# RabbitBio/RabbitKSSD

Measured on AMD Instinct MI355X. Metric: genome-pairs/sec alldist (10k bacteria, L3K10), higher is better.
Workload: dtype bit-sliced counters of 32 x 32 tiles in registers, 16 planes (exact), u32 counts after extraction / f64 jaccard + distance; 1 GPU; alldist over 10000 synthetic bacterial sketches (sketch-level clade generator, seed 20261003, L3K10: 28-bit hashes, ~1220 per genome, clades of 10), -D 0.05, distance kernel only from an HBM-resident index (BASELINE configs[2]: precomputed .sketch/.dict); genomes=10000, pairs=49995000, hits=45000, kernel=rk_tile_kernel<512u, true>

## Files before the change

rabbitkssd_amd/csrc/rk_core.hip:

```cpp
#include <algorithm>
#include <cstdlib>
#include <cstring>

#include "rk_internal.h"

int rk_fail(rk_ctx *ctx, int code, const char *fmt, ...)
{
    char buf[512];
    va_list ap;
    va_start(ap, fmt);
    vsnprintf(buf, sizeof(buf), fmt, ap);
    va_end(ap);
    if (ctx) ctx->err = buf;
    return code;
}

static size_t pool_round(size_t bytes)
{
    if (bytes <= (1u << 16)) return (bytes + 511) & ~(size_t)511;
    if (bytes <= (1u << 24)) return (bytes + 65535) & ~(size_t)65535;
    return (bytes + ((1u << 21) - 1)) & ~(size_t)((1u << 21) - 1);
}

static void pool_put_locked(rk_ctx *ctx, void *p)
// ... 113 lines not shown
    } else {
        RK_HIP(ctx, hipMemcpyAsync(dst, src_dev, bytes, hipMemcpyDeviceToHost, stream));
        RK_HIP(ctx, hipStreamSynchronize(stream));
    }
    return RK_OK;
}

int rk_occupancy(rk_ctx *ctx, const void *kernel, int threads, size_t lds_bytes)
{
    const auto key = std::make_tuple(kernel, threads, lds_bytes);
    {
        std::lock_guard<std::mutex> lk(ctx->mu);
        auto it = ctx->occupancy.find(key);
        if (it != ctx->occupancy.end()) return it->second;
    }
    int per_cu = 0;
    if (hipOccupancyMaxActiveBlocksPerMultiprocessor(&per_cu, kernel, threads, lds_bytes) != hipSuccess) {
        (void)hipGetLastError();
        per_cu = 1;
    }
    std::lock_guard<std::mutex> lk(ctx->mu);
    ctx->occupancy[key] = per_cu;
    return per_cu;
}

template <class V> __global__ void k_calib_read(const V *p, size_t n, unsigned long long *sink)
{
    unsigned long long acc = 0;
    for (size_t i = (size_t)blockIdx.x * blockDim.x + threadIdx.x; i < n; i += (size_t)gridDim.x * blockDim.x) {
        const V v = p[i];
        const unsigned char *b = reinterpret_cast<const unsigned char *>(&v);
        acc += b[0] + b[sizeof(V) - 1];
    }
    if (acc == 0x1234567ULL) *sink = acc;
}
extern "C" int rk_debug_calib_read(rk_ctx *ctx, uint64_t bytes, int width)
{
    if (!ctx || (width != 4 && width != 8 && width != 16)) return RK_ERR_ARG;
    RK_HIP(ctx, hipSetDevice(ctx->device));
    DevBuf<char> buf(ctx);
    DevBuf<unsigned long long> sink(ctx);
    RK_HIP(ctx, buf.alloc(bytes));
    RK_HIP(ctx, sink.alloc(1));
    RK_HIP(ctx, hipMemsetAsync(buf.p, 1, bytes, ctx->stream));
    const unsigned grid = (unsigned)ctx->num_cu * 8;
    if (width == 4) hipLaunchKernelGGL(k_calib_read<uint32_t>, dim3(grid), dim3(256), 0, ctx->stream, (const uint32_t *)buf.p, bytes / 4, sink.p);
    else if (width == 8) hipLaunchKernelGGL(k_calib_read<uint2>, dim3(grid), dim3(256), 0, ctx->stream, (const uint2 *)buf.p, bytes / 8, sink.p);
    else hipLaunchKernelGGL(k_calib_read<uint4>, dim3(grid), dim3(256), 0, ctx->stream, (const uint4 *)buf.p, bytes / 16, sink.p);
    RK_HIP(ctx, hipGetLastError());
    RK_HIP(ctx, hipStreamSynchronize(ctx->stream));
    return RK_OK;
}

extern "C" int rk_debug_stream_read_gbs(rk_ctx *ctx, uint64_t bytes, int reps, double *gbs)
{
    if (!ctx || !gbs || reps < 1 || bytes < (1u << 20)) return RK_ERR_ARG;
    *gbs = 0.0;
    RK_HIP(ctx, hipSetDevice(ctx->device));
    DevBuf<char> buf(ctx);
    DevBuf<unsigned long long> sink(ctx);
    RK_HIP(ctx, buf.alloc(bytes));
    RK_HIP(ctx, sink.alloc(1));
    RK_HIP(ctx, hipMemsetAsync(buf.p, 1, bytes, ctx->stream));
    const unsigned grid = (unsigned)ctx->num_cu * 8;
    hipEvent_t e0, e1;
    RK_HIP(ctx, hipEventCreate(&e0));
    RK_HIP(ctx, hipEventCreate(&e1));
    hipLaunchKernelGGL(k_calib_read<uint4>, dim3(grid), dim3(256), 0, ctx->stream, (const uint4 *)buf.p, bytes / 16, sink.p);
    (void)hipEventRecord(e0, ctx->stream);
    for (int r = 0; r < reps; r++)
        hipLaunchKernelGGL(k_calib_read<uint4>, dim3(grid), dim3(256), 0, ctx->stream, (const uint4 *)buf.p, bytes / 16, sink.p);
    (void)hipEventRecord(e1, ctx->stream);
    hipError_t e = hipStreamSynchronize(ctx->stream);
    float ms = 0.f;
    if (e == hipSuccess) e = hipEventElapsedTime(&ms, e0, e1);
    (void)hipEventDestroy(e0);
    (void)hipEventDestroy(e1);
    RK_HIP(ctx, e);
    if (ms > 0.f) *gbs = (double)bytes * reps / (ms * 1e-3) / 1e9;
    return RK_OK;
}

extern "C" {

const char *rk_version(void) { return "rabbitkssd-amd 0.1.0 (gfx950)"; }

int rk_device_count(void)
{
    int n = 0;
    if (hipGetDeviceCount(&n) != hipSuccess) return 0;
    return n;
}

static uint32_t env_u32(const char *name, uint32_t dflt)
{
    const char *v = getenv(name);
    return v && atoi(v) > 0 ? (uint32_t)atoi(v) : dflt;
}

int rk_ctx_create(int device, rk_ctx **out)
{
    if (!out) return RK_ERR_ARG;
    *out = nullptr;
    int n = 0;
    if (hipGetDeviceCount(&n) != hipSuccess || n <= 0) return RK_ERR_NO_DEVICE;
    if (device < 0 || device >= n) return RK_ERR_NO_DEVICE;
    if (hipSetDevice(device) != hipSuccess) return RK_ERR_HIP;
    rk_ctx *ctx = new (std::nothrow) rk_ctx;
    if (!ctx) return RK_ERR_NOMEM;
    ctx->device = device;
    int v = 0;
    if (hipDeviceGetAttribute(&v, hipDeviceAttributeMultiprocessorCount, device) != hipSuccess || v <= 0) {
        delete ctx;
        return RK_ERR_HIP;
    }
    ctx->num_cu = v;
    ctx->max_lds = 64 * 1024;
    if (hipDeviceGetAttribute(&v, hipDeviceAttributeMaxSharedMemoryPerBlock, device) == hipSuccess && v > 0)
        ctx->max_lds = (size_t)v;
    if (hipDeviceGetAttribute(&v, hipDeviceAttributeSharedMemPerBlockOptin, device) == hipSuccess &&
        (size_t)v > ctx->max_lds)
        ctx->max_lds = (size_t)v;
    if (hipStreamCreateWithFlags(&ctx->stream, hipStreamNonBlocking) != hipSuccess || !rk_pinned_scratch(ctx, kPinnedBytes)) {
        rk_ctx_destroy(ctx);
        return RK_ERR_HIP;
    }
    ctx->cache_limit = (size_t)env_u32("RK_POOL_LIMIT_MB", 32768) << 20;
    ctx->sw_dist_threads = env_u32("RK_DIST_THREADS", 0);
    ctx->sw_dist_rows = env_u32("RK_DIST_ROWS", 0);
    ctx->sw_dist_pair = env_u32("RK_DIST_PAIR", 1);
    ctx->sw_dist_pair_minwg = env_u32("RK_DIST_PAIR_MINWG", 3);
    ctx->sw_dist_persist = env_u32("RK_DIST_PERSIST", 1);
    ctx->sw_dist_cand_cap = env_u32("RK_DIST_CAND_CAP", 0);
    ctx->sw_dist_stage_hits = env_u32("RK_DIST_STAGE_HITS", 0);
    ctx->sw_dist_xcd_rows = env_u32("RK_DIST_XCD_ROWS", 0);
    ctx->sw_dist_bands = getenv("RK_DIST_BANDS") ? atoi(getenv("RK_DIST_BANDS")) != 0 : 1;
    if (getenv("RK_DIST_BAND_MIN_ROWS")) ctx->sw_dist_band_min_rows = std::max(1, atoi(getenv("RK_DIST_BAND_MIN_ROWS")));
    ctx->sw_dist_near = getenv("RK_DIST_NEAR") ? atoi(getenv("RK_DIST_NEAR")) != 0 : 1;
    if (getenv("RK_DIST_TILES")) ctx->sw_dist_tiles = atoi(getenv("RK_DIST_TILES"));
    if (getenv("RK_DIST_TILES_MIN_GENOMES")) ctx->sw_dist_tiles_min_genomes = atoi(getenv("RK_DIST_TILES_MIN_GENOMES"));
    if (getenv("RK_DIST_TILES_MIN_SHARD_ROWS")) ctx->sw_dist_tiles_min_shard_rows = atoi(getenv("RK_DIST_TILES_MIN_SHARD_ROWS"));
    if (getenv("RK_DIST_NEAR_UW")) ctx->sw_dist_near_uw = atoi(getenv("RK_DIST_NEAR_UW"));
    if (getenv("RK_DIST_NEAR_MIN")) ctx->sw_dist_near_min = std::max(1, atoi(getenv("RK_DIST_NEAR_MIN")));
    if (getenv("RK_DIST_FB_SKIP")) ctx->sw_dist_fb_skip = atoi(getenv("RK_DIST_FB_SKIP")) != 0;
    ctx->sw_dist_debug = getenv("RK_DIST_DEBUG") ? atoi(getenv("RK_DIST_DEBUG")) : 0;
    if (getenv("RK_DIST_LDS_KB")) ctx->sw_dist_lds_kb = std::max(0, atoi(getenv("RK_DIST_LDS_KB")));
    ctx->sw_sketch_img = getenv("RK_SKETCH_IMG") ? std::min(2, std::max(0, atoi(getenv("RK_SKETCH_IMG")))) : 2;
    ctx->sw_index_fast = getenv("RK_INDEX_FAST") ? atoi(getenv("RK_INDEX_FAST")) != 0 : 1;
    ctx->sw_index_relabel = getenv("RK_INDEX_RELABEL") ? atoi(getenv("RK_INDEX_RELABEL")) != 0 : 1;
    ctx->sw_index_no_self = getenv("RK_INDEX_NO_SELF") ? atoi(getenv("RK_INDEX_NO_SELF")) != 0 : 0;
    if (getenv("RK_INDEX_TILES")) ctx->sw_index_tiles = atoi(getenv("RK_INDEX_TILES"));
    if (getenv("RK_INDEX_NO_HEAVY")) ctx->sw_index_heavy = atoi(getenv("RK_INDEX_NO_HEAVY")) == 0;
    if (getenv("RK_TILE_REC_CAP")) ctx->sw_tile_rec_cap = strtoull(getenv("RK_TILE_REC_CAP"), nullptr, 10);
    ctx->sw_topn = getenv("RK_DIST_TOPN") ? atoi(getenv("RK_DIST_TOPN")) != 0 : 1;
    if (getenv("RK_TOPN_BATCH_BYTES")) ctx->sw_topn_batch_bytes = std::max(1ULL, strtoull(getenv("RK_TOPN_BATCH_BYTES"), nullptr, 10));
    if (getenv("RK_TOPN_CAND_CAP")) ctx->sw_topn_cand_cap = strtoull(getenv("RK_TOPN_CAND_CAP"), nullptr, 10);
    *out = ctx;
    return RK_OK;
}

void rk_ctx_set_single_shot(rk_ctx *ctx, int on)
{
    if (ctx) ctx->single_shot = on != 0;
}

void rk_ctx_set_timing(rk_ctx *ctx, int on)
{
    if (!ctx) return;
    (void)hipSetDevice(ctx->device);
    if (on && !ctx->ev[0] && (hipEventCreate(&ctx->ev[0]) != hipSuccess || hipEventCreate(&ctx->ev[1]) != hipSuccess)) return;
    ctx->timing = on != 0;
}

void rk_ctx_pool_stats(rk_ctx *ctx, uint64_t out[4])
{
    if (!ctx || !out) return;
    std::lock_guard<std::mutex> lk(ctx->mu);
    out[0] = ctx->pool_bytes;
    out[1] = ctx->cached_bytes;
    out[2] = ctx->driver_allocs;
    out[3] = ctx->driver_frees;
}

double rk_ctx_last_ms(const rk_ctx *ctx, int which) { return ctx && which >= 0 && which < 15 ? ctx->last_ms[which] : 0.0; }

void rk_ctx_trim(rk_ctx *ctx)
{
    if (!ctx) return;
    std::lock_guard<std::mutex> lk(ctx->mu);
    (void)hipSetDevice(ctx->device);
    if (!ctx->deferred.empty()) pool_collect_locked(ctx, true);
    for (auto &b : ctx->free_blocks) {
        ctx->live.erase(b.second);
        ctx->pool_bytes -= b.first;
        ctx->driver_frees++;
        (void)hipFree(b.second);
    }
    ctx->free_blocks.clear();
    ctx->cached_bytes = 0;
}

void rk_ctx_destroy(rk_ctx *ctx)
{
    if (!ctx) return;
    (void)hipSetDevice(ctx->device);
    if (ctx->stream) {
        (void)hipStreamSynchronize(ctx->stream);
        (void)hipStreamDestroy(ctx->stream);
        if (ctx->stream2) (void)hipStreamDestroy(ctx->stream2);
        if (ctx->ev_fork) (void)hipEventDestroy(ctx->ev_fork);
        if (ctx->ev_join) (void)hipEventDestroy(ctx->ev_join);
        if (ctx->ev_inv) (void)hipEventDestroy(ctx->ev_inv);
    }
    rk_ctx_trim(ctx);
    for (hipEvent_t e : ctx->spare_events) (void)hipEventDestroy(e);
    for (auto &b : ctx->live) (void)hipFree(b.first);
    if (ctx->pinned) (void)hipHostFree(ctx->pinned);
    for (hipEvent_t e : ctx->ev)
        if (e) (void)hipEventDestroy(e);
    delete ctx;
}

const char *rk_last_error(const rk_ctx *ctx) { return ctx ? ctx->err.c_str() : "no context"; }

void rk_free_host(void *p) { free(p); }

int rk_pinned_alloc(rk_ctx *ctx, uint64_t bytes, void **out)
{
    if (!ctx || !out) return RK_ERR_ARG;
    *out = nullptr;
    RK_HIP(ctx, hipSetDevice(ctx->device));
    if (hipHostMalloc(out, bytes ? bytes : 1, hipHostMallocDefault) != hipSuccess) {
        *out = nullptr;
        return rk_fail(ctx, RK_ERR_NOMEM, "cannot pin %llu bytes of host memory", (unsigned long long)bytes);
    }
    return RK_OK;
}
void rk_pinned_free(void *p) { if (p) (void)hipHostFree(p); }

int rk_dev_alloc(rk_ctx *ctx, uint64_t bytes, void **out)
{
    if (!ctx || !out) return RK_ERR_ARG;
    *out = nullptr;
    RK_HIP(ctx, hipSetDevice(ctx->device));
    if (hipMalloc(out, bytes ? bytes : 1) != hipSuccess) {
        *out = nullptr;
        return rk_fail(ctx, RK_ERR_NOMEM, "cannot allocate %llu bytes on the device", (unsigned long long)bytes);
    }
    return RK_OK;
}
void rk_dev_free(void *p) { if (p) (void)hipFree(p); }

int rk_stream_create(rk_ctx *ctx, void **out)
{
    if (!ctx || !out) return RK_ERR_ARG;
    *out = nullptr;
    RK_HIP(ctx, hipSetDevice(ctx->device));
    hipStream_t st = nullptr;
    RK_HIP(ctx, hipStreamCreateWithFlags(&st, hipStreamNonBlocking));
    *out = (void *)st;
    return RK_OK;
}
void rk_stream_destroy(void *stream) { if (stream) (void)hipStreamDestroy((hipStream_t)stream); }

int rk_stream_sync(rk_ctx *ctx, void *stream)
{
    if (!ctx) return RK_ERR_ARG;
    RK_HIP(ctx, hipSetDevice(ctx->device));
    RK_HIP(ctx, hipStreamSynchronize((hipStream_t)stream));
    return RK_OK;
}

int rk_upload_async(rk_ctx *ctx, void *dst_dev, const void *src_host, uint64_t bytes, void *stream)
{
    if (!ctx || (bytes && (!dst_dev || !src_host))) return RK_ERR_ARG;
    RK_HIP(ctx, hipSetDevice(ctx->device));
    if (bytes) RK_HIP(ctx, hipMemcpyAsync(dst_dev, src_host, bytes, hipMemcpyHostToDevice, (hipStream_t)stream));
    return RK_OK;
}

int rk_dev_copy_async(rk_ctx *ctx, void *dst_dev, const void *src_dev, uint64_t bytes, void *stream)
{
    if (!ctx || (bytes && (!dst_dev || !src_dev))) return RK_ERR_ARG;
    RK_HIP(ctx, hipSetDevice(ctx->device));
    if (bytes) RK_HIP(ctx, hipMemcpyAsync(dst_dev, src_dev, bytes, hipMemcpyDeviceToDevice, (hipStream_t)stream));
    return RK_OK;
}

int rk_params_init(int half_k, int half_subk, int drlevel, rk_params *p)
{
    if (!p) return RK_ERR_ARG;
    if (half_subk - drlevel < 3) return RK_ERR_ARG;
    if (half_k < half_subk || half_subk >= 8 || half_subk < 1) return RK_ERR_ARG;
    if (half_k > 16 || drlevel < 0) return RK_ERR_ARG;
    memset(p, 0, sizeof(*p));
    const int out = half_k - half_subk;
    p->half_k = half_k;
    p->half_subk = half_subk;
    p->drlevel = drlevel;
    p->half_outctx_len = out;
    p->rev_add_move = 4 * half_k - 2;
    p->kmer_size = 2u * (uint32_t)half_k;
    p->dim_start = 0;
    p->dim_end = 1 << (4 * (half_subk - drlevel));
    const uint64_t tupmask = ~0ULL >> (64 - 4 * half_k);
    const uint64_t domask = (tupmask >> (4 * out)) << (2 * out);
// ... 95 lines not shown
```

rabbitkssd_amd/csrc/rk_dist.hip:

```cpp
#include <algorithm>
#include <chrono>
#include <cmath>
#include <cstdio>
#include <cstdlib>
#include <cstring>
#include <thread>
#include <tuple>
#include <vector>


#include "rk_internal.h"
#include "rk_dist_common.h"
#include "rk_dist_plan.h"

namespace {

__global__ void k_hit_keys(const rk_hit *hits, unsigned long long n, unsigned long long *keys)
{
    const unsigned long long i = (unsigned long long)blockIdx.x * blockDim.x + threadIdx.x;
    if (i < n) keys[i] = ((unsigned long long)hits[i].row << 32) | hits[i].col;
}

constexpr int kGroup = 8;
constexpr uint32_t kRowsPerXcdChunk = 16;
// ... 928 lines not shown
    else if (idx->tiles_ready) {
        const uint32_t step = o->row_step > 1 ? o->row_step : 1;
        const bool small_shard = step > 2 && idx->n_ref / step < (uint32_t)ctx->sw_dist_tiles_min_shard_rows;
        tiles = !(small_shard && idx->d_selfrange);
    } else if (floor(sp->min_jorc * (double)idx->min_ref_size) < (double)ctx->sw_dist_near_min) {
        tiles = true;
    } else {
        int rc = near_window_too_narrow(ctx, idx, stream, &tiles);
        if (rc) return rc;
    }
    if (tiles) {
        sp->kind = SelfPlan::kTiles;
        sp->need_tiles = !idx->tiles_ready;
        if (!sp->need_tiles) sp->tile = tile_launch_shape(idx, o, sp->min_jorc);
        return RK_OK;
    }
    if (!idx->d_selfrange) {
        if (!can_rows)
            return rk_fail(ctx, RK_ERR_UNSUPPORTED, "this index has no slice records (2^31 postings or more): only sparse self joins (a threshold "
                                                    "below distance 1.0) over set sketches run on it%s", idx->tiles_unusable ? ", and its tile records "
                                                    "exceed the memory budget (lists scattered over thousands of genomes)" : "");
        sp->need_slices = true;
    }
    const bool slices_coming = sp->need_slices && idx->d_src_off && idx->wide == (idx->d_uhash64 != nullptr);
    sp->near = slices_coming || idx->d_self_split ? plan_near(ctx, idx, o, dense_mode, sp->min_jorc) : NearPlan();
    sp->kind = sp->near.use ? SelfPlan::kNear : SelfPlan::kBands;
    return sp->near.use ? RK_OK : plan_bands(ctx, idx, o, dense_mode, &sp->bands);
}

int ensure_fallback(rk_ctx *ctx, rk_index *idx, hipStream_t stream)
{
    std::lock_guard<std::mutex> lk(idx->lazy_mu);
    if (idx->d_fb) return RK_OK;
    DevBuf<uint32_t> fb(ctx);
    if (fb.alloc((size_t)idx->n_ref + 8) != hipSuccess) return rk_fail(ctx, RK_ERR_NOMEM, "cannot allocate the fallback list");
    RK_HIP(ctx, hipMemsetAsync(fb.p, 0, 16, stream));
    RK_HIP(ctx, hipStreamSynchronize(stream));
    if (hipHostMalloc((void **)&idx->h_fb_seen, 64, hipHostMallocCoherent) == hipSuccess) *idx->h_fb_seen = 0xFFFFFFFFu;
    else { (void)hipGetLastError(); idx->h_fb_seen = nullptr; }
    idx->d_fb = fb.release();
    return RK_OK;
}

int launch_near(rk_ctx *ctx, const rk_index *idx, const rk_dist_opts *o, const NearPlan &np, rk_hit *hits_dev, uint64_t cap,
                unsigned long long *n_hits_dev, hipStream_t stream)
{
    NearArgs a;
    a.ranges = idx->d_selfrange;
    a.range_off = idx->d_self_off;
    a.range_split = idx->d_self_split;
    a.size_off = idx->d_src_off;
    a.postings = idx->d_postings;
    a.ref_sizes = idx->d_sizes;
    a.orig = idx->relabeled ? idx->d_orig : nullptr;
    a.n_ref = idx->n_ref;
    a.row_first = np.rows.row_first;
    a.row_step = np.rows.row_step;
    a.row_block = np.rows.row_block;
    a.units_per_block = np.units_per_block;
    a.n_units = np.n_units;
    a.metric = o->metric != 0;
    a.kmer_size = o->kmer_size;
    a.max_dist = o->max_dist;
    a.min_jorc = np.min_jorc;
    a.min_ref_size = (uint32_t)std::min<uint64_t>(idx->min_ref_size, 0xFFFFFFFFu);
    a.hits = hits_dev;
    a.cap = cap;
    a.n_hits = n_hits_dev;
    a.fb_count = idx->d_fb;
    a.fb_rows = idx->d_fb + 4;
    a.stage_hits = kNearStage;
    a.debug = getenv("RK_NEAR_DEBUG") ? atoi(getenv("RK_NEAR_DEBUG")) : 0;
#define RK_NEAR(P, U) hipLaunchKernelGGL((rk_near_kernel<P, U>), dim3(np.grid), dim3(kNearThreads), 0, stream, a)
    if (np.pair) { if (np.uw == 1) RK_NEAR(true, 1); else if (np.uw == 2) RK_NEAR(true, 2); else RK_NEAR(true, 4); }
    else { if (np.uw == 1) RK_NEAR(false, 1); else if (np.uw == 2) RK_NEAR(false, 2); else RK_NEAR(false, 4); }
#undef RK_NEAR
    RK_HIP(ctx, hipGetLastError());
    return RK_OK;
}

struct FbGate { unsigned char key[sizeof(rk_index::fb_key)] = {0}; bool skip = false, arm = false; };
FbGate fb_gate_begin(rk_ctx *ctx, rk_index *mut, const rk_dist_opts *o, bool dense_mode)
{
    FbGate g;
    static_assert(sizeof(rk_dist_opts) + 1 <= sizeof g.key, "key holds the options and the report mode");
    memcpy(g.key, o, sizeof(rk_dist_opts));
    g.key[sizeof(rk_dist_opts)] = dense_mode ? 1 : 0;
    if (ctx->sw_dist_fb_skip && mut->h_fb_seen) {
        std::lock_guard<std::mutex> lk(mut->lazy_mu);
        if (memcmp(g.key, mut->fb_key, sizeof g.key) != 0) {
            memcpy(mut->fb_key, g.key, sizeof g.key);
            mut->fb_state = 0;
        }
        if (mut->fb_state == 1) {
            const hipError_t qe = hipEventQuery((hipEvent_t)mut->fb_event);
            if (qe == hipSuccess) mut->fb_state = *(volatile uint32_t *)mut->h_fb_seen == 0 ? 2 : 3;
            else (void)hipGetLastError();
        }
        g.skip = mut->fb_state == 2;
        if (mut->fb_state == 0) {
            if (!mut->fb_event) {
                hipEvent_t ev;
                if (hipEventCreateWithFlags(&ev, hipEventDisableTiming | hipEventReleaseToSystem) == hipSuccess) mut->fb_event = ev;
                else (void)hipGetLastError();
            }
            g.arm = mut->fb_event != nullptr;
        }
    }
    return g;
}
void fb_gate_armed(rk_index *mut, const FbGate &g, hipStream_t stream)
{
    std::lock_guard<std::mutex> lk(mut->lazy_mu);
    if (mut->fb_state == 0 && memcmp(g.key, mut->fb_key, sizeof g.key) == 0 &&
        hipEventRecord((hipEvent_t)mut->fb_event, stream) == hipSuccess) mut->fb_state = 1;
}

int launch_near_and_fallback(rk_ctx *ctx, rk_index *mut, const rk_dist_opts *o, bool dense_mode, const NearPlan &np, rk_hit *hits_dev,
                             uint64_t cap, unsigned long long *n_hits_dev, hipStream_t stream)
{
    int rc = ensure_fallback(ctx, mut, stream);
    if (!rc && np.n_units) rc = launch_near(ctx, mut, o, np, hits_dev, cap, n_hits_dev, stream);
    if (rc) return rc;
    const FbGate gate = fb_gate_begin(ctx, mut, o, dense_mode);
    if (gate.skip) return RK_OK;
    Plan fp;
    rk_dist_opts all = *o;
    all.row_first = 0;
    all.row_step = 1;
    rc = make_plan(ctx, mut, mut->n_ref, mut->max_src_size, &all, false, true, mut->n_ref, &fp, false);
    if (rc) return rc;
    rc = launch_dist(ctx, mut, mut->d_selfrange, mut->d_self_off, mut->d_src_off, mut->n_ref, o, fp, hits_dev, cap, n_hits_dev,
                     nullptr, stream, mut->d_fb);
    if (!rc && gate.arm) fb_gate_armed(mut, gate, stream);
    return rc;
}

int launch_self(rk_ctx *ctx, const rk_index *idx, const rk_dist_opts *o, bool dense_mode, rk_hit *hits_dev, uint64_t cap,
                unsigned long long *n_hits_dev, hipStream_t stream)
{
    rk_index *mut = const_cast<rk_index *>(idx);
    SelfPlan sp;
    int rc = plan_self(ctx, idx, o, dense_mode, stream, &sp);
    if (!rc && sp.need_tiles) {
        rc = rk_tiles_build(ctx, mut, stream);
        if (!rc && !idx->tiles_unusable) sp.tile = tile_launch_shape(idx, o, sp.min_jorc);
        else if (!rc) rc = plan_self(ctx, idx, o, dense_mode, stream, &sp);
    }
    if (!rc && sp.need_slices) {
        rc = rk_index_ensure_slices(ctx, mut, stream);
        if (!rc) rc = plan_self(ctx, idx, o, dense_mode, stream, &sp);
    }
    if (rc) return rc;
    if (sp.kind == SelfPlan::kTiles) return launch_tiles(ctx, idx, o, sp.min_jorc, sp.tile, hits_dev, cap, n_hits_dev, stream);
    if (sp.kind == SelfPlan::kNear) return launch_near_and_fallback(ctx, mut, o, dense_mode, sp.near, hits_dev, cap, n_hits_dev, stream);
    if (ctx->sw_dist_debug) print_bands(sp.bands);
    for (size_t b = 0; !rc && b < sp.bands.size(); b++)
        rc = launch_dist(ctx, idx, idx->d_selfrange, idx->d_self_off, idx->d_src_off, idx->n_ref, o, sp.bands[b], hits_dev, cap,
                         n_hits_dev, nullptr, stream);
    return rc;
}

uint64_t host_exact_distances(rk_hit *h, uint64_t n, const rk_dist_opts *o)
{
    const int metric = o->metric != 0;
    auto fix = [&](uint64_t lo, uint64_t hi) {
        for (uint64_t i = lo; i < hi; i++) {
            const JorcDist jd = rk_distance(h[i].common, h[i].size0, h[i].size1, metric, o->kmer_size);
            h[i].jorc = jd.jorc;
            h[i].dist = jd.dist;
        }
    };
    const uint64_t kChunk = 8192;
    if (n < 2 * kChunk) fix(0, n);
    else {
        const unsigned nt = (unsigned)std::min<uint64_t>(std::max(1u, std::thread::hardware_concurrency()), std::min<uint64_t>(16, n / kChunk));
        std::vector<std::thread> pool;
        for (unsigned t = 0; t < nt; t++) pool.emplace_back(fix, n * t / nt, n * (t + 1) / nt);
        for (auto &th : pool) th.join();
    }
    uint64_t w = 0;
    for (uint64_t i = 0; i < n; i++) {
        const bool keep = o->triangle ? (h[i].dist < o->max_dist) : (h[i].dist <= o->max_dist);
        if (keep) {
            if (w != i) h[w] = h[i];
            w++;
        }
    }
    return w;
}

int download_hits_in_order(rk_ctx *ctx, const rk_hit *hits_dev, unsigned long long n, uint32_t n_query, hipStream_t stream, rk_hit **out_p)
{
    rk_hit *out = (rk_hit *)malloc((n ? n : 1) * sizeof(rk_hit));
    if (!out) return rk_fail(ctx, RK_ERR_NOMEM, "host allocation of %llu hits failed", n);
    const rk_hit *src = hits_dev;
    DevBuf<rk_hit> ordered(ctx);
    bool on_device = false;
    if (n > (ctx->single_shot ? (1ULL << 18) : 2048ULL)) {
        DevBuf<unsigned long long> keys(ctx), keys_out(ctx);
        int bits = 33;
        while (bits < 64 && (1ULL << (bits - 32)) < n_query) bits++;
        if (keys.alloc(n) == hipSuccess && keys_out.alloc(n) == hipSuccess && ordered.alloc(n) == hipSuccess) {
            hipLaunchKernelGGL(k_hit_keys, dim3((unsigned)((n + 255) / 256)), dim3(256), 0, stream, hits_dev, n, keys.p);
            on_device = rk_prim_sort_hits(ctx, keys.p, keys_out.p, hits_dev, ordered.p, n, (unsigned)bits, stream) == RK_OK;
        }
        if (on_device) src = ordered.p;
        else (void)hipGetLastError();
    }
    if (n) {
        hipError_t e = hipMemcpyAsync(out, src, n * sizeof(rk_hit), hipMemcpyDeviceToHost, stream);
        if (e == hipSuccess) e = hipStreamSynchronize(stream);
        if (e != hipSuccess) {
            free(out);
            return rk_fail(ctx, RK_ERR_HIP, "hit download failed: %s", hipGetErrorString(e));
        }
    }
    if (!on_device)
        std::sort(out, out + n, [](const rk_hit &x, const rk_hit &y) {
            return x.row != y.row ? x.row < y.row : x.col < y.col;
        });
    *out_p = out;
    return RK_OK;
}

}

uint64_t rk_host_exact_distances(rk_hit *h, uint64_t n, const rk_dist_opts *o) { return host_exact_distances(h, n, o); }

#ifdef RK_DIST_PROFILE
extern "C" int rk_debug_dist_prof_raw(unsigned long long *out, unsigned long long n_waves)
{
    if (n_waves > (unsigned long long)kProfWaves) return -1;
    return hipMemcpyFromSymbol(out, HIP_SYMBOL(g_prof), n_waves * 16 * 8) == hipSuccess ? 0 : -1;
}
extern "C" int rk_debug_dist_prof(unsigned long long *out16, int reset)
{
    std::vector<unsigned long long> all((size_t)kProfWaves * 16);
    if (hipMemcpyFromSymbol(all.data(), HIP_SYMBOL(g_prof), sizeof(g_prof)) != hipSuccess) return -1;
    for (int i = 0; i < 16; i++) out16[i] = 0;
    for (size_t w = 0; w < (size_t)kProfWaves; w++)
        for (int i = 0; i < 16; i++) out16[i] += all[w * 16 + i];
    if (reset) {
        std::fill(all.begin(), all.end(), 0ULL);
        if (hipMemcpyToSymbol(HIP_SYMBOL(g_prof), all.data(), sizeof(g_prof)) != hipSuccess) return -1;
    }
    return 0;
}
#endif

extern "C" {

int rk_dist_kernel_name(rk_ctx *ctx, const rk_index *idx, const rk_sketches *queries, const rk_dist_opts *opts, char *buf,
                        size_t cap)
{
    if (!ctx || !idx || !opts || !buf || !cap) return RK_ERR_ARG;
    if (queries) return rk_distq_kernel_name(ctx, idx, queries, buf, cap);
    SelfPlan sp;
    int rc = plan_self(ctx, idx, opts, rk_dense_mode(opts), ctx->stream, &sp);
    if (rc) return rc;
    if (sp.kind == SelfPlan::kTiles && sp.need_tiles)
        snprintf(buf, cap, "rk_tile_kernel");
    else if (sp.kind == SelfPlan::kTiles)
        snprintf(buf, cap, "rk_tile_kernel<%du, %s>", sp.tile.threads, sp.tile.srow ? "true" : "false");
    else if (sp.kind == SelfPlan::kNear)
        snprintf(buf, cap, "rk_near_kernel<%s, %d>", sp.near.pair ? "true" : "false", sp.near.uw);
    else {
        if (ctx->sw_dist_debug) print_bands(sp.bands);
        const Plan &p = sp.bands[0];
        if (sp.bands.size() > 1)
            snprintf(buf, cap, "rk_dist_kernel<%s, %d, %u> [%u bands]", p.u16 ? "true" : "false", p.mode, p.threads, (unsigned)sp.bands.size());
        else
            snprintf(buf, cap, "rk_dist_kernel<%s, %d, %u>", p.u16 ? "true" : "false", p.mode, p.threads);
    }
    return RK_OK;
}

int rk_index_tile_stats(const rk_index *idx, const rk_dist_opts *opts, uint64_t out[4])
{
    if (!idx || !out) return RK_ERR_ARG;
    out[0] = out[1] = out[2] = out[3] = 0;
    if (!idx->tiles_ready) return RK_OK;
    out[0] = idx->n_tiles;
    out[2] = idx->n_tile_records;
    out[3] = idx->n_tile_slots;
    if (opts && opts->kmer_size > 0 && opts->max_dist > 0.0) out[1] = tile_launch_shape(idx, opts, rk_min_jorc(opts)).grid;
    return RK_OK;
}

int rk_dist_rows_dev(rk_ctx *ctx, const rk_index *idx, const rk_sketches *queries,
                     const rk_dist_opts *opts, rk_hit *hits_dev, uint64_t hits_cap,
                     uint64_t *n_hits_dev, void *stream)
{
    if (!ctx || !idx || !opts || !n_hits_dev || (!hits_dev && hits_cap)) return RK_ERR_ARG;
    RK_HIP(ctx, hipSetDevice(ctx->device));
    if (queries) {
        if (opts->triangle && queries->n != idx->n_ref)
            return rk_fail(ctx, RK_ERR_ARG, "triangle mode needs the indexed sketches as queries (%u vs %u)",
                           queries->n, idx->n_ref);
        return rk_distq_launch(ctx, idx, queries, opts, rk_dense_mode(opts), hits_dev, hits_cap, (unsigned long long *)n_hits_dev,
                               nullptr, (hipStream_t)stream);
    }
    if (int rc = rk_self_join_args(ctx, idx, opts)) return rc;
    return launch_self(ctx, idx, opts, rk_dense_mode(opts), hits_dev, hits_cap, (unsigned long long *)n_hits_dev, (hipStream_t)stream);
}

int rk_dist_rows(rk_ctx *ctx, const rk_index *idx, const rk_sketches *queries,
// ... 70 lines not shown
```

rabbitkssd_amd/csrc/rk_dist_tile.inc:

```

struct TileArgs {
    const unsigned long long *tile_key;
    const unsigned long long *tile_start;
    const uint32_t *blk_min;
    const uint64_t *size_off;
    const uint32_t *orig;
    const uint32_t *order;
    const uint4 *dir;
    unsigned long long n_tiles;
    uint32_t n_ref;
    uint32_t row_first, row_step, row_block;
    int metric, kmer_size;
    double max_dist, min_jorc;
    rk_hit *hits;
    unsigned long long cap;
    unsigned long long *n_hits;
    int debug;
};

constexpr unsigned long long kTileSrowPerTile = 2000ULL;
constexpr int kTilePlanes = 11;

__device__ inline uint32_t csa(uint32_t &a, uint32_t b, uint32_t c)
{
    const uint32_t carry = __builtin_amdgcn_bitop3_b32(a, b, c, 0xE8);
    a = __builtin_amdgcn_bitop3_b32(a, b, c, 0x96);
    return carry;
}
__device__ inline uint32_t ripple(uint32_t &p, uint32_t carry)
{
    const uint32_t c2 = p & carry;
    p ^= carry;
    return c2;
}

template <uint32_t kTileThreads, bool SROW>
__global__ __launch_bounds__(kTileThreads, kTileThreads == 256 ? 6 : 4) void rk_tile_kernel(TileArgs a, const uint2 *__restrict__ contrib, const uint32_t *__restrict__ rows, const uint32_t *__restrict__ cols)
{
    constexpr uint32_t kTileWaves = kTileThreads / 64;
    constexpr uint32_t kTileStage = (uint32_t)(8 * kTileThreads * sizeof(uint2) / sizeof(rk_hit));
    static_assert(kTileStage >= kTileThreads + 64, "a round of cells fits the stage");
    __shared__ uint32_t cnt[32 * 32];
    __shared__ __attribute__((aligned(16))) uint2 recs[8 * kTileThreads];
    rk_hit *stage = reinterpret_cast<rk_hit *>(recs);
    __shared__ uint32_t s_cursor;
    __shared__ unsigned long long s_base;
    __shared__ uint32_t rsize[32], csize[32];
    const uint32_t tid = threadIdx.x, lane = tid & 63, wave = tid >> 6;
    const uint32_t half = lane >> 5, row = lane & 31;

    const uint4 d0 = a.dir[2 * (size_t)blockIdx.x], d1 = a.dir[2 * (size_t)blockIdx.x + 1];
    const uint32_t b = d0.x, w = d0.y;
    const unsigned long long s0 = (unsigned long long)d0.z | ((unsigned long long)d0.w << 32), s1 = s0 + d1.x;
    {
        const uint32_t lb = d1.y;
        bool take = (double)(s1 - s0) >= a.min_jorc * (double)lb;
        if (take && a.row_step > 1) {
            bool mine = false;
            const uint32_t r0 = b * 32, r1 = min(a.n_ref, r0 + 32);
            for (uint32_t blk = r0 / a.row_block; blk <= (r1 - 1) / a.row_block; blk++) mine |= blk % a.row_step == a.row_first;
            take = mine;
        }
        if (!take || (a.debug & 4) || ((a.debug & 32) && blockIdx.x >= 512) || ((a.debug & 64) && blockIdx.x >= 256)) return;
    }
    for (uint32_t i = tid; i < 32 * 32; i += kTileThreads) cnt[i] = 0;
    if (tid == 0) s_cursor = 0;
    __syncthreads();

    auto flush_stage = [&]() {
        __syncthreads();
        const uint32_t n_st = min(s_cursor, kTileStage);
        if (n_st) {
            if (tid == 0) s_base = (a.debug & 4096) ? (unsigned long long)blockIdx.x * 128ULL : atomicAdd(a.n_hits, (unsigned long long)n_st);
            __syncthreads();
            const unsigned long long at0 = s_base;
            const unsigned long long *src = reinterpret_cast<const unsigned long long *>(stage);
            unsigned long long *dst = reinterpret_cast<unsigned long long *>(a.hits);
            constexpr uint32_t kW = sizeof(rk_hit) / 8;
            for (uint32_t i = tid; i < n_st * kW; i += kTileThreads)
                if (at0 + i / kW < a.cap) dst[at0 * kW + i] = src[i];
        }
        __syncthreads();
        if (tid == 0) s_cursor = 0;
        __syncthreads();
    };

    {
        if (tid < 64) {
            const uint32_t g = (tid < 32 ? b : w) * 32 + (tid & 31);
            const uint32_t sz = g < a.n_ref ? (uint32_t)(a.size_off[g + 1] - a.size_off[g]) : 0u;
            if (tid < 32) rsize[tid] = sz; else csize[tid - 32] = sz;
        }
        uint32_t p[kTilePlanes + 1];
#pragma unroll
        for (int k = 0; k <= kTilePlanes; k++) p[k] = 0;
        uint32_t steps = 0;
        auto to_lds = [&]() {
            uint32_t carry = 0;
#pragma unroll
            for (int k = 0; k < kTilePlanes; k++) {
                const uint32_t o = (uint32_t)__shfl_xor((int)p[k], 32);
                const uint32_t u = p[k] ^ o;
                const uint32_t c2 = (p[k] & o) | (u & carry);
                p[k] = u ^ carry;
                carry = c2;
            }
            p[kTilePlanes] = carry;
            uint32_t any = 0;
#pragma unroll
            for (int k = 0; k <= kTilePlanes; k++) any |= p[k];
            const uint32_t occupied = wave_or(any);
            uint32_t occ2 = (occupied | (occupied >> 16)) & 0xFFFFu;
            while (occ2) {
                const int c = __builtin_ctz(occ2) + 16 * (int)half;
                occ2 &= occ2 - 1;
                uint32_t v = 0;
#pragma unroll
                for (int k = 0; k <= kTilePlanes; k++) v |= ((p[k] >> c) & 1u) << k;
                if (v) atomicAdd(&cnt[c * 32 + row], v);
            }
#pragma unroll
            for (int k = 0; k <= kTilePlanes; k++) p[k] = 0;
            steps = 0;
        };
        auto add8 = [&](const uint32_t (&m)[8]) {
            const uint32_t t2a = csa(p[0], m[0], m[1]);
            const uint32_t t2b = csa(p[0], m[2], m[3]);
            const uint32_t t4a = csa(p[1], t2a, t2b);
            const uint32_t t2c = csa(p[0], m[4], m[5]);
            const uint32_t t2d = csa(p[0], m[6], m[7]);
            const uint32_t t4b = csa(p[1], t2c, t2d);
            uint32_t carry = csa(p[2], t4a, t4b);
#pragma unroll
            for (int k = 3; k < kTilePlanes; k++) carry = ripple(p[k], carry);
            steps += 8;
            if (steps >= 1984) to_lds();
        };
        auto carry16 = [&](const uint32_t (&ma)[8], const uint32_t (&mb)[8]) -> uint32_t {
            const uint32_t a2a = csa(p[0], ma[0], ma[1]);
            const uint32_t a2b = csa(p[0], ma[2], ma[3]);
            const uint32_t a4a = csa(p[1], a2a, a2b);
            const uint32_t a2c = csa(p[0], ma[4], ma[5]);
            const uint32_t a2d = csa(p[0], ma[6], ma[7]);
            const uint32_t a4b = csa(p[1], a2c, a2d);
            const uint32_t c8a = csa(p[2], a4a, a4b);
            const uint32_t b2a = csa(p[0], mb[0], mb[1]);
            const uint32_t b2b = csa(p[0], mb[2], mb[3]);
            const uint32_t b4a = csa(p[1], b2a, b2b);
            const uint32_t b2c = csa(p[0], mb[4], mb[5]);
            const uint32_t b2d = csa(p[0], mb[6], mb[7]);
            const uint32_t b4b = csa(p[1], b2c, b2d);
            const uint32_t c8b = csa(p[2], b4a, b4b);
            return csa(p[3], c8a, c8b);
        };
        auto add16 = [&](const uint32_t (&ma)[8], const uint32_t (&mb)[8]) {
            uint32_t carry = carry16(ma, mb);
#pragma unroll
            for (int k = 4; k < kTilePlanes; k++) carry = ripple(p[k], carry);
            steps += 16;
            if (steps >= 1984) to_lds();
        };
        if (!(a.debug & 1)) {
            if constexpr (SROW) {
                constexpr int kDepth = 3;
                const unsigned long long slot0 = (unsigned long long)d1.z | ((unsigned long long)d1.w << 32);
                const unsigned long long *__restrict__ tile_rows = reinterpret_cast<const unsigned long long *>(rows + slot0);
                const uint32_t n_rec = d1.x;
                const uint32_t wave_u = (uint32_t)__builtin_amdgcn_readfirstlane((int)wave);
                const uint32_t per = ((n_rec + kTileWaves - 1) / kTileWaves + 127u) & ~127u;
                const uint32_t w0 = min(n_rec, wave_u * per), w1 = min(n_rec, w0 + per);
                const uint32_t n_sub = (w1 - w0 + 127u) / 128u;
                const uint32_t *__restrict__ tile_cols = cols + slot0;
                uint32_t *mine = reinterpret_cast<uint32_t *>(recs + wave * 512);
                uint32_t in0[kDepth], in1[kDepth];
                auto request = [&](uint32_t sub, int slot) {
                    const uint32_t at = w0 + sub * 128u + lane;
                    in0[slot] = tile_cols[at];
                    in1[slot] = tile_cols[at + 64u];
                };
                const uint32_t put0 = (lane & 1u) * 64u + (lane >> 1), put1 = put0 + 32u;
    #pragma unroll
                for (int d = 0; d < kDepth; d++)
                    if ((uint32_t)d < n_sub) request((uint32_t)d, d);
                for (uint32_t sub0 = 0; sub0 < n_sub; sub0 += kDepth) {
    #pragma unroll
                    for (int d = 0; d < kDepth; d++) {
                        const uint32_t sub = sub0 + d;
                        if (sub >= n_sub) break;
                        const uint32_t at = w0 + sub * 128u + lane;
                        uint32_t *slot = mine + (sub & 3u) * 128;
                        slot[put0] = at < w1 ? in0[d] : 0u;
                        slot[put1] = at + 64u < w1 ? in1[d] : 0u;
                        if (sub + kDepth < n_sub) request(sub + kDepth, d);
                        __builtin_amdgcn_fence(__ATOMIC_RELEASE, "wavefront");
                        __builtin_amdgcn_wave_barrier();
                        const uint32_t n_here = min(128u, w1 - (w0 + sub * 128u));
                        const uint4 *rd = reinterpret_cast<const uint4 *>(slot + 64 * half);
                        const unsigned long long *pairs = tile_rows + ((w0 + sub * 128u) >> 1);
                        const uint32_t n_groups = min(8u, (n_here + 15) / 16);
                        auto masks_sel = [&](uint32_t g, const unsigned long long *sel, uint32_t (&m)[8]) {
                            const uint4 r0 = rd[2 * g], r1 = rd[2 * g + 1];
                            const uint32_t y[8] = {r0.x, r0.y, r0.z, r0.w, r1.x, r1.y, r1.z, r1.w};
    #pragma unroll
                            for (int j = 0; j < 8; j++)
                                asm("v_cndmask_b32_e64 %0, 0, %1, %2" : "=v"(m[j]) : "v"(y[j]), "s"(sel[j]));
                        };
                        auto masks = [&](uint32_t g, uint32_t (&m)[8]) {
                            unsigned long long sel[8];
    #pragma unroll
                            for (int j = 0; j < 8; j++) sel[j] = pairs[8 * g + j];
                            const uint4 r0 = rd[2 * g], r1 = rd[2 * g + 1];
                            const uint32_t y[8] = {r0.x, r0.y, r0.z, r0.w, r1.x, r1.y, r1.z, r1.w};
    #pragma unroll
                            for (int j = 0; j < 8; j++)
                                asm("v_cndmask_b32_e64 %0, 0, %1, %2" : "=v"(m[j]) : "v"(y[j]), "s"(sel[j]));
                        };
                        uint32_t g = 0;
                        auto carry32 = [&](uint32_t g0) -> uint32_t {
                            unsigned long long sel[32];
    #pragma unroll
                            for (int j = 0; j < 32; j++) sel[j] = pairs[8 * g0 + j];
                            uint32_t ma[8], mb[8];
                            masks_sel(g0, sel, ma);
                            masks_sel(g0 + 1, sel + 8, mb);
                            const uint32_t c16a = carry16(ma, mb);
                            masks_sel(g0 + 2, sel + 16, ma);
                            masks_sel(g0 + 3, sel + 24, mb);
                            const uint32_t c16b = carry16(ma, mb);
                            return csa(p[4], c16a, c16b);
                        };
                        if (n_groups == 8 && !(a.debug & (256 | 512 | 1024))) {
                            const uint32_t c32a = carry32(0);
                            const uint32_t c32b = carry32(4);
                            uint32_t carry = csa(p[5], c32a, c32b);
    #pragma unroll
                            for (int k = 6; k < kTilePlanes; k++) carry = ripple(p[k], carry);
                            steps += 64;
                            if (steps >= 1984) to_lds();
                            g = 8;
                        }
                        for (; g + 3 < n_groups && !(a.debug & (256 | 512)); g += 4) {
                            uint32_t carry = carry32(g);
    #pragma unroll
                            for (int k = 5; k < kTilePlanes; k++) carry = ripple(p[k], carry);
                            steps += 32;
                            if (steps >= 1984) to_lds();
                        }
                        for (; g + 1 < n_groups && !(a.debug & 256); g += 2) {
                            uint32_t ma[8], mb[8];
                            masks(g, ma);
                            masks(g + 1, mb);
                            if (a.debug & 8) { p[0] |= ma[0] | ma[1] | ma[2] | ma[3] | ma[4] | ma[5] | ma[6] | ma[7] | mb[0] | mb[7]; continue; }
                            add16(ma, mb);
                        }
                        for (; g < n_groups; g++) {
                            uint32_t m[8];
                            masks(g, m);
                            if (a.debug & 8) { p[0] |= m[0] | m[1] | m[2] | m[3] | m[4] | m[5] | m[6] | m[7]; continue; }
                            add8(m);
                        }
                        __builtin_amdgcn_wave_barrier();
                    }
                }
            } else {
                constexpr int kDepth = 3;
                const uint2 *__restrict__ tile = contrib + s0;
                const uint32_t n_rec = d1.x;
                const uint32_t per = ((n_rec + kTileWaves - 1) / kTileWaves + 127u) & ~127u;
                const uint32_t w0 = min(n_rec, wave * per), w1 = min(n_rec, w0 + per);
                const uint32_t n_sub = (w1 - w0 + 127u) / 128u;
                uint2 *mine = recs + wave * 512;
                uint2 in0[kDepth], in1[kDepth];
                auto request = [&](uint32_t sub, int slot) {
                    const uint32_t at = w0 + sub * 128u + lane;
                    in0[slot] = tile[min(at, n_rec - 1u)];
                    in1[slot] = tile[min(at + 64u, n_rec - 1u)];
                };
    #pragma unroll
                for (int d = 0; d < kDepth; d++)
                    if ((uint32_t)d < n_sub) request((uint32_t)d, d);
                for (uint32_t sub0 = 0; sub0 < n_sub; sub0 += kDepth) {
    #pragma unroll
                    for (int d = 0; d < kDepth; d++) {
                        const uint32_t sub = sub0 + d;
                        if (sub >= n_sub) break;
                        const uint32_t at = w0 + sub * 128u + lane;
                        uint2 *slot = mine + (sub & 3u) * 128;
                        slot[lane] = at < w1 ? in0[d] : make_uint2(0, 0);
                        slot[64 + lane] = at + 64u < w1 ? in1[d] : make_uint2(0, 0);
                        if (sub + kDepth < n_sub) request(sub + kDepth, d);
                        __builtin_amdgcn_fence(__ATOMIC_RELEASE, "wavefront");
                        __builtin_amdgcn_wave_barrier();
                        const uint32_t n_here = min(128u, w1 - (w0 + sub * 128u));
                        const uint4 *rd = reinterpret_cast<const uint4 *>(slot + 64 * half);
                        const uint32_t n_groups = min(8u, (n_here + 7) / 8);
                        auto masks = [&](uint32_t g, uint32_t (&m)[8]) {
    #pragma unroll
                            for (int j = 0; j < 4; j++) {
                                const uint4 r = rd[4 * g + j];
                                m[2 * j] = (uint32_t)__builtin_amdgcn_sbfe((int)r.x, row, 1) & r.y;
                                m[2 * j + 1] = (uint32_t)__builtin_amdgcn_sbfe((int)r.z, row, 1) & r.w;
                            }
                        };
                        uint32_t g = 0;
                        auto carry32 = [&](uint32_t g0) -> uint32_t {
                            uint32_t ma[8], mb[8];
                            masks(g0, ma);
                            masks(g0 + 1, mb);
                            const uint32_t c16a = carry16(ma, mb);
                            masks(g0 + 2, ma);
                            masks(g0 + 3, mb);
                            const uint32_t c16b = carry16(ma, mb);
                            return csa(p[4], c16a, c16b);
                        };
                        if (n_groups == 8 && !(a.debug & (256 | 512 | 1024))) {
                            const uint32_t c32a = carry32(0);
                            const uint32_t c32b = carry32(4);
                            uint32_t carry = csa(p[5], c32a, c32b);
    #pragma unroll
                            for (int k = 6; k < kTilePlanes; k++) carry = ripple(p[k], carry);
                            steps += 64;
                            if (steps >= 1984) to_lds();
                            g = 8;
                        }
                        for (; g + 3 < n_groups && !(a.debug & (256 | 512)); g += 4) {
                            uint32_t carry = carry32(g);
    #pragma unroll
                            for (int k = 5; k < kTilePlanes; k++) carry = ripple(p[k], carry);
                            steps += 32;
                            if (steps >= 1984) to_lds();
                        }
                        for (; g + 1 < n_groups && !(a.debug & 256); g += 2) {
                            uint32_t ma[8], mb[8];
                            masks(g, ma);
                            masks(g + 1, mb);
                            if (a.debug & 8) { p[0] |= ma[0] | ma[1] | ma[2] | ma[3] | ma[4] | ma[5] | ma[6] | ma[7] | mb[0] | mb[7]; continue; }
                            add16(ma, mb);
                        }
                        for (; g < n_groups; g++) {
                            uint32_t m[8];
                            masks(g, m);
                            if (a.debug & 8) { p[0] |= m[0] | m[1] | m[2] | m[3] | m[4] | m[5] | m[6] | m[7]; continue; }
                            add8(m);
                        }
                        __builtin_amdgcn_wave_barrier();
                    }
                }
            }
        }
        if (!(a.debug & 16)) {
            constexpr int kAll = 16;
            uint32_t q[kAll];
            {
                uint32_t carry = 0;
#pragma unroll
                for (int k = 0; k < kTilePlanes; k++) {
                    const uint32_t o = (uint32_t)__shfl_xor((int)p[k], 32);
                    const uint32_t u = p[k] ^ o;
                    q[k] = u ^ carry;
                    carry = (p[k] & o) | (u & carry);
                }
                q[kTilePlanes] = carry;
#pragma unroll
                for (int k = kTilePlanes + 1; k < kAll; k++) q[k] = 0;
            }
            uint32_t *all_planes = reinterpret_cast<uint32_t *>(recs);
            uint32_t *my_planes = all_planes + wave * 1024;
            auto publish = [&]() {
                if (lane < 32) {
#pragma unroll
                    for (int k = 0; k < kAll; k++) my_planes[k * 32 + row] = q[k];
                }
            };
            if (kTileWaves > 1) publish();
            __syncthreads();
#pragma unroll
            for (uint32_t stride = 1; stride < kTileWaves; stride <<= 1) {
                if ((wave & (2 * stride - 1)) == 0) {
                    const uint32_t *theirs = all_planes + (wave + stride) * 1024;
                    uint32_t carry = 0;
#pragma unroll
                    for (int k = 0; k < kAll; k++) {
                        const uint32_t o = theirs[k * 32 + row];
                        const uint32_t u = q[k] ^ o;
                        const uint32_t c2 = (q[k] & o) | (u & carry);
                        q[k] = u ^ carry;
                        carry = c2;
                    }
                    publish();
                }
                __syncthreads();
            }
            if (kTileWaves > 1) {
#pragma unroll
                for (int k = 0; k < kAll; k++) q[k] = all_planes[k * 32 + row];
            }
            constexpr uint32_t kColsPerHalf = 16 / kTileWaves;
#pragma unroll
            for (uint32_t i = 0; i < kColsPerHalf; i++) {
                const uint32_t c = wave * (32 / kTileWaves) + half * kColsPerHalf + i;
                uint32_t v = 0;
#pragma unroll
                for (int k = 0; k < kAll; k++) v |= ((q[k] >> c) & 1u) << k;
                if (v) cnt[c * 32 + row] += v;
            }
        }
        __syncthreads();
        for (uint32_t round = 0; round < 1024 / kTileThreads; round++) {
            if (s_cursor + kTileThreads > kTileStage) flush_stage();
            const uint32_t ci = round * kTileThreads + tid;
            const uint32_t col = ci >> 5, r = ci & 31;
            const uint32_t common = cnt[ci];
            cnt[ci] = 0;
            const uint32_t grow = b * 32 + r, gcol = w * 32 + col;
            bool ok = common != 0 && gcol > grow && gcol < a.n_ref && !(a.debug & 2);
            if (ok && a.row_step > 1) ok = (grow / a.row_block) % a.row_step == a.row_first;
            if (ok) {
                const int size0 = (int)rsize[r], size1 = (int)csize[col];
                const int denom = a.metric ? min(size0, size1) : size0 + size1 - (int)common;
                if ((double)common >= a.min_jorc * (double)denom) {
                    const JorcDist jd = rk_distance((int)common, size0, size1, a.metric, a.kmer_size);
                    if (jd.dist < a.max_dist) {
                        uint32_t out_row = grow, out_col = gcol;
                        if (a.orig) {
                            out_row = a.orig[grow];
                            out_col = a.orig[gcol];
                        }
                        const bool flip = out_row > out_col;
                        rk_hit hrec;
                        hrec.row = flip ? out_col : out_row;
                        hrec.col = flip ? out_row : out_col;
                        hrec.common = (int)common;
                        hrec.size0 = flip ? size1 : size0;
                        hrec.size1 = flip ? size0 : size1;
                        hrec.pad_ = 0;
                        hrec.jorc = jd.jorc;
                        hrec.dist = jd.dist;
                        stage[atomicAdd(&s_cursor, 1u)] = hrec;
                    }
                }
            }
            __syncthreads();
        }
        flush_stage();
    }
}

struct TileShape { unsigned long long grid = 0; int threads = 256; bool srow = false; };
TileShape tile_launch_shape(const rk_index *idx, const rk_dist_opts *o, double min_jorc)
{
    const int metric = o->metric != 0;
    unsigned long long grid = idx->n_tiles;
    if (min_jorc > 0.0) {
        const double kk = ceil(-8.0 * log2(min_jorc));
        if (kk < (double)kTileTable) grid = idx->tile_prefix[metric][kk < 0.0 ? 0 : (int)kk];
    }
    if (getenv("RK_TILE_ALL")) grid = idx->n_tiles;
    const uint32_t row_step = o->row_step ? o->row_step : 1;
    int threads = grid / row_step < 1500 ? 512 : 256;
    if (grid / row_step < 150) threads = 1024;
    if (getenv("RK_TILE_THREADS")) threads = atoi(getenv("RK_TILE_THREADS"));
    if (threads != 512 && threads != 1024) threads = 256;
    bool srow = threads >= 512 && grid && idx->n_tile_records >= kTileSrowPerTile * grid && idx->d_tile_rows;
    if (getenv("RK_TILE_SROW")) srow = atoi(getenv("RK_TILE_SROW")) != 0 && idx->d_tile_rows;
    return TileShape{grid, threads, srow};
}

int launch_tiles(rk_ctx *ctx, const rk_index *idx, const rk_dist_opts *o, double min_jorc, const TileShape &shape, rk_hit *hits_dev, uint64_t cap,
                 unsigned long long *n_hits_dev, hipStream_t stream)
{
    if (!idx->n_tiles) return RK_OK;
    TileArgs a;
    a.tile_key = idx->d_tile_key;
    a.tile_start = idx->d_tile_start;
    a.blk_min = idx->d_blk_min;
    a.size_off = idx->d_src_off;
    a.orig = idx->relabeled ? idx->d_orig : nullptr;
    a.n_tiles = idx->n_tiles;
    a.n_ref = idx->n_ref;
    a.order = idx->d_tile_order[o->metric != 0];
    a.dir = idx->d_tile_dir[o->metric != 0];
    const RowShard rows(o, idx->n_ref, 0);
    a.row_step = rows.row_step;
    a.row_first = rows.row_first;
    a.row_block = rows.row_block;
    a.metric = o->metric != 0;
    a.kmer_size = o->kmer_size;
    a.max_dist = o->max_dist;
    a.min_jorc = min_jorc;
    a.hits = hits_dev;
    a.cap = cap;
    a.n_hits = n_hits_dev;
    a.debug = getenv("RK_TILE_DEBUG") ? atoi(getenv("RK_TILE_DEBUG")) : 0;
    if (!shape.grid) return RK_OK;
    if (shape.grid > 0x7FFFFFFFULL) return rk_fail(ctx, RK_ERR_UNSUPPORTED, "too many tiles for one launch (%llu)", (unsigned long long)idx->n_tiles);
#define RK_TILE_LAUNCH(T)                                                                                                              \
    do {                                                                                                                               \
        if (shape.srow) hipLaunchKernelGGL((rk_tile_kernel<T, true>), dim3((unsigned)shape.grid), dim3(T), 0, stream, a, (const uint2 *)idx->d_tile_contrib, (const uint32_t *)idx->d_tile_rows, (const uint32_t *)idx->d_tile_cols); \
        else hipLaunchKernelGGL((rk_tile_kernel<T, false>), dim3((unsigned)shape.grid), dim3(T), 0, stream, a, (const uint2 *)idx->d_tile_contrib, (const uint32_t *)idx->d_tile_rows, (const uint32_t *)idx->d_tile_cols); \
    } while (0)
    if (shape.threads == 512)
        RK_TILE_LAUNCH(512);
    else if (shape.threads == 1024)
        RK_TILE_LAUNCH(1024);
    else
        RK_TILE_LAUNCH(256);
#undef RK_TILE_LAUNCH
    RK_HIP(ctx, hipGetLastError());
    return RK_OK;
}
```

rabbitkssd_amd/csrc/rk_index.hip:

```cpp
#include <cstring>

#include <algorithm>
#include <chrono>
#include <cstdlib>
#include <thread>

#include "rk_internal.h"

namespace {

struct BuildResult {
    unsigned long long U, n_self, dups, flags;
    unsigned long long flagged;
};

template <class Acc, class L, class W> __device__ inline Acc block_scan_sweeps(uint32_t n, L load, W store)
{
    __shared__ Acc scan_part[1024 / 64];
    constexpr uint32_t R = 16;
    const uint32_t tid = threadIdx.x, lane = tid & 63, wave = tid >> 6, nw = blockDim.x >> 6;
    const uint32_t rows = (n + 63) / 64;
    Acc carry = 0;
    for (uint32_t base = 0; base < rows; base += nw * R) {
        const uint32_t r0 = base + wave * R;
// ... 321 lines not shown
        uint32_t votes = 0;
#pragma unroll
        for (uint32_t j = 0; j < kMinK; j++) votes += r[j] == r[i];
        if (votes >= 2 && r[i] < best) best = r[i];
    }
    parent[g] = best;
}

__global__ void k_cluster_keys(const uint32_t *parent, uint32_t n_genomes, int id_bits, unsigned long long *keys)
{
    const uint32_t g = blockIdx.x * blockDim.x + threadIdx.x;
    if (g >= n_genomes) return;
    uint32_t p = parent[g];
    for (uint32_t hop = 0; hop < n_genomes; hop++) {
        const uint32_t q = parent[p];
        if (q == p) break;
        p = q;
    }
    keys[g] = ((unsigned long long)p << id_bits) | g;
}

__global__ void k_order_from_keys(const unsigned long long *keys, uint32_t n_genomes, int id_bits, const uint64_t *off,
                                  const uint32_t *sizes_in, uint32_t *orig, uint32_t *sizes)
{
    const uint32_t i = blockIdx.x * blockDim.x + threadIdx.x;
    if (i >= n_genomes) return;
    const uint32_t g = (uint32_t)(keys[i] & ((1ULL << id_bits) - 1ULL));
    orig[i] = g;
    sizes[i] = sizes_in ? sizes_in[g] : (uint32_t)(off[g + 1] - off[g]);
}

__global__ void k_offsets_scan(const uint32_t *sizes, uint32_t n_genomes, uint64_t *off_new)
{
    const unsigned long long all = block_scan_sweeps<unsigned long long>(
        n_genomes, [&](uint32_t g) { return (unsigned long long)sizes[g]; },
        [&](uint32_t g, unsigned long long before) { off_new[g] = before; });
    if (threadIdx.x == 0) off_new[n_genomes] = all;
}

constexpr uint32_t kRankThreads = 256, kRankPer = 4, kRankQ = kRankThreads * kRankPer, kRankStretch = 256, kRankMaxN = 32768;
__global__ void k_cluster_keys32(const uint32_t *parent, uint32_t n_genomes, int id_bits, uint32_t *keys, uint32_t *rank)
{
    const uint32_t g = blockIdx.x * blockDim.x + threadIdx.x;
    if (g >= n_genomes) return;
    rank[g] = 0;
    uint32_t p = parent[g];
    for (uint32_t hop = 0; hop < n_genomes; hop++) {
        const uint32_t q = parent[p];
        if (q == p) break;
        p = q;
    }
    keys[g] = (p << id_bits) | g;
}
__global__ __launch_bounds__(kRankThreads) void k_rank_keys(const uint32_t *__restrict__ keys, uint32_t n, uint32_t *rank)
{
    __shared__ __attribute__((aligned(16))) uint32_t others[kRankStretch];
    const uint32_t j0 = blockIdx.y * kRankStretch;
    for (uint32_t j = threadIdx.x; j < kRankStretch; j += kRankThreads) others[j] = j0 + j < n ? keys[j0 + j] : 0xFFFFFFFFu;
    uint32_t mine[kRankPer], below[kRankPer];
#pragma unroll
    for (uint32_t i = 0; i < kRankPer; i++) {
        const uint32_t q = blockIdx.x * kRankQ + i * kRankThreads + threadIdx.x;
        mine[i] = q < n ? keys[q] : 0u;
        below[i] = 0;
    }
    __syncthreads();
    const uint4 *o4 = reinterpret_cast<const uint4 *>(others);
#pragma unroll 4
    for (uint32_t j = 0; j < kRankStretch / 4; j++) {
        const uint4 v = o4[j];
#pragma unroll
        for (uint32_t i = 0; i < kRankPer; i++) below[i] += (v.x < mine[i]) + (v.y < mine[i]) + (v.z < mine[i]) + (v.w < mine[i]);
    }
#pragma unroll
    for (uint32_t i = 0; i < kRankPer; i++) {
        const uint32_t q = blockIdx.x * kRankQ + i * kRankThreads + threadIdx.x;
        if (q < n && below[i]) atomicAdd(&rank[q], below[i]);
    }
}
__global__ void k_order_from_rank(const uint32_t *rank, uint32_t n_genomes, const uint64_t *off, const uint32_t *sizes_in, uint32_t *orig, uint32_t *sizes)
{
    const uint32_t g = blockIdx.x * blockDim.x + threadIdx.x;
    if (g >= n_genomes) return;
    const uint32_t i = rank[g];
    orig[i] = g;
    sizes[i] = sizes_in ? sizes_in[g] : (uint32_t)(off[g + 1] - off[g]);
}

template <class K>
__global__ void k_gather_sketches(const K *hashes, const uint64_t *off, const uint32_t *orig, const uint64_t *off_new,
                                  uint32_t n_genomes, K *out)
{
    const uint32_t i = blockIdx.x * (blockDim.x >> 6) + (threadIdx.x >> 6);
    if (i >= n_genomes) return;
    const uint64_t src = off[orig[i]], dst = off_new[i], n = off_new[i + 1] - dst;
    for (uint64_t k = threadIdx.x & 63; k < n; k += 64) out[dst + k] = hashes[src + k];
}

__global__ void k_emit_table(const uint32_t *inv, const uint64_t *off_new, uint32_t n, uint2 *tab)
{
    const uint32_t g = blockIdx.x * blockDim.x + threadIdx.x;
    if (g < n) tab[g] = make_uint2(inv[g], (uint32_t)off_new[inv[g]]);
}

__global__ void k_invert_order(const uint32_t *orig, uint32_t n, uint32_t *inv)
{
    const uint32_t i = blockIdx.x * blockDim.x + threadIdx.x;
    if (i < n) inv[orig[i]] = i;
}

__global__ void k_iota(uint32_t n, uint32_t *out)
{
    const uint32_t i = blockIdx.x * blockDim.x + threadIdx.x;
    if (i < n) out[i] = i;
}

#include "rk_index_fast.inc"
#include "rk_index_tiles.inc"
#include "rk_index_keys.inc"

struct BuildSource {
    uint32_t n = 0;
    uint64_t total = 0;
    bool wide = false, is_set = false;
    uint64_t max_size = 0, min_size = 0;
    const uint64_t *d_off = nullptr;
    const uint32_t *d_sizes = nullptr;
    const uint32_t *d_sig = nullptr;
    const rk_sketches *s = nullptr;
    const unsigned long long *keys = nullptr;
    uint64_t n_keys = 0;
};
inline BuildSource source_of(const rk_sketches *s)
{
    BuildSource src;
    src.n = s->n;
    src.total = s->total;
    src.wide = s->wide;
    src.is_set = s->is_set;
    src.max_size = s->max_size;
    for (uint32_t g = 0; g < s->n; g++) {
        const uint64_t sz = s->h_off[g + 1] - s->h_off[g];
        if (sz && (!src.min_size || sz < src.min_size)) src.min_size = sz;
    }
    src.d_off = s->d_off;
    src.s = s;
    return src;
}

#include "rk_index_plan.h"

struct TileSortBufs {
    DevBuf<uint3> brec;
    DevBuf<uint32_t> tb, bins, t_rows, t_cols;
    DevBuf<uint4> proto, t_dir_j, t_dir_c;
    DevBuf<unsigned long long> level_start;
    DevBuf<uint2> t_contrib;
    explicit TileSortBufs(rk_ctx *c) : brec(c), tb(c), bins(c), t_rows(c), t_cols(c), proto(c), t_dir_j(c), t_dir_c(c), level_start(c), t_contrib(c) {}
    int alloc(rk_ctx *ctx, uint32_t n_blocks, uint64_t n_records, uint64_t tile_cap)
    {
        const uint64_t slot_cap = n_records + tile_cap;
        RK_HIP(ctx, brec.alloc(n_records));
        RK_HIP(ctx, tb.alloc(3 * (size_t)n_blocks));
        RK_HIP(ctx, bins.alloc((size_t)n_blocks + 1));
        RK_HIP(ctx, proto.alloc(2 * tile_cap));
        RK_HIP(ctx, level_start.alloc(2 * (kTileTable + 1)));
        RK_HIP(ctx, t_contrib.alloc(slot_cap + 256));
        if (rowsort_stage(n_blocks)) {
            RK_HIP(ctx, t_rows.alloc(slot_cap + 256));
            RK_HIP(ctx, t_cols.alloc(slot_cap + 256));
        }
        RK_HIP(ctx, t_dir_j.alloc(2 * tile_cap));
        RK_HIP(ctx, t_dir_c.alloc(2 * tile_cap));
        return RK_OK;
    }
    TileSortArgs args(const uint3 *rec, uint32_t region_cap, uint32_t n_blocks, const uint32_t *blk_min, const ZeroedLayout &z) const
    {
        TileSortArgs ta;
        memset(&ta, 0, sizeof ta);
        ta.rec = rec;
        ta.cur = z.tile_cursors();
        ta.region_cap = region_cap;
        ta.n_blocks = n_blocks;
        ta.bin_count = z.bin_count();
        ta.bin_cursor = z.bin_cursor();
        ta.bin_start = bins.p;
        ta.brec = brec.p;
        ta.blk_min = blk_min;
        ta.contrib = t_contrib.p;
        ta.rows = t_rows.p;
        ta.cols = t_cols.p;
        ta.tb_base = tb.p;
        ta.tb_cnt = tb.p + n_blocks;
        ta.order = tb.p + 2 * (size_t)n_blocks;
        ta.proto = proto.p;
        ta.level_start = level_start.p;
        ta.dir[0] = t_dir_j.p;
        ta.dir[1] = t_dir_c.p;
        ta.tres = z.tile_res();
        return ta;
    }
    void hand_over(rk_index *idx, const TileResult &tr)
    {
        idx->d_tile_contrib = t_contrib.release();
        idx->d_tile_rows = t_rows.release();
        idx->d_tile_cols = t_cols.release();
        idx->d_tile_dir[0] = t_dir_j.release();
        idx->d_tile_dir[1] = t_dir_c.release();
        idx->n_tile_slots = tr.n_slots;
        idx->n_tiles = tr.n_tiles;
        idx->n_tile_records = tr.n_records;
        idx->tile_max_records = tr.max_records;
        for (int m = 0; m < 2; m++)
            for (int k = 0; k < kTileTable; k++) idx->tile_prefix[m][k] = tr.level_count[m][k];
        idx->tiles_ready = true;
        idx->tiles_from_build = true;
    }
};

struct BuildCtx {
    rk_ctx *ctx;
    const BuildSource &src;
    const BuildPlan &p;
    const BuildKnobs &k;
    rk_index *idx;
    hipStream_t st;
};

int alloc_index_arrays(rk_ctx *ctx, rk_index *idx, const BuildPlan &p)
{
    RK_TRY(pool_array(ctx, &idx->d_sizes, (size_t)p.N + 1));
    RK_TRY(pool_array(ctx, &idx->d_src_off, (size_t)p.N + 1));
    RK_TRY(pool_array(ctx, &idx->d_postings, p.H_el + 8));
    if (idx->wide) RK_TRY(pool_array(ctx, &idx->d_uhash64, p.Ucap + 1));
    else RK_TRY(pool_array(ctx, &idx->d_uhash, p.Ucap + 1));
    RK_TRY(pool_array(ctx, &idx->d_upos, p.Ucap + 2));
    RK_TRY(pool_array(ctx, &idx->d_orig, (size_t)p.N + 1));
    if (p.tiles_mode) RK_TRY(pool_array(ctx, &idx->d_blk_min, (size_t)p.n_blocks));
    return RK_OK;
}
int alloc_slices(rk_ctx *ctx, rk_index *idx, const BuildPlan &p)
{
    if (p.no_self || idx->d_selfrange) return RK_OK;
    RK_TRY(pool_array(ctx, &idx->d_selfrange, p.H + 1));
    RK_TRY(pool_array(ctx, &idx->d_self_off, (size_t)p.N + 1));
    RK_TRY(pool_array(ctx, &idx->d_self_split, (size_t)p.N + 1));
    return RK_OK;
}
void drop_blk_min(rk_ctx *ctx, rk_index *idx)
{
    rk_pool_free(ctx, idx->d_blk_min);
    idx->d_blk_min = nullptr;
}

int ensure_stream2(rk_ctx *ctx, bool high_priority)
{
    if (ctx->stream2) return RK_OK;
    int prio_lo = 0, prio_hi = 0;
    if (high_priority && hipDeviceGetStreamPriorityRange(&prio_lo, &prio_hi) == hipSuccess && prio_hi != prio_lo)
        RK_HIP(ctx, hipStreamCreateWithPriority(&ctx->stream2, hipStreamNonBlocking, prio_hi));
    else
        RK_HIP(ctx, hipStreamCreateWithFlags(&ctx->stream2, hipStreamNonBlocking));
    RK_HIP(ctx, hipEventCreateWithFlags(&ctx->ev_fork, hipEventDisableTiming));
    RK_HIP(ctx, hipEventCreateWithFlags(&ctx->ev_join, hipEventDisableTiming));
    RK_HIP(ctx, hipEventCreateWithFlags(&ctx->ev_inv, hipEventDisableTiming));
    return RK_OK;
}

struct Renumbering {
    const BuildCtx &b;
    DevBuf<unsigned long long> rl_table, rl_keys, rl_keys_sorted;
    DevBuf<uint32_t> rl_parent, rl_keys32, rl_rank, rl_inv;
    DevBuf<uint2> rl_tab;
    DevBuf<char> rl_tmp;
    const uint32_t *inv = nullptr;
    bool forked = false, joined = true;
    bool inv_recorded = false;
    bool enqueued = false;
    explicit Renumbering(const BuildCtx &bc)
        : b(bc), rl_table(bc.ctx), rl_keys(bc.ctx), rl_keys_sorted(bc.ctx), rl_parent(bc.ctx), rl_keys32(bc.ctx), rl_rank(bc.ctx), rl_inv(bc.ctx),
          rl_tab(bc.ctx), rl_tmp(bc.ctx) {}

    int mark_fork()
    {
        if (!b.p.two_streams) return RK_OK;
        RK_TRY(ensure_stream2(b.ctx, b.k.stream2_high));
        RK_HIP(b.ctx, hipEventRecord(b.ctx->ev_fork, b.st));
        return RK_OK;
    }
    int join()
    {
        if (!joined) {
            RK_HIP(b.ctx, hipStreamWaitEvent(b.st, b.ctx->ev_join, 0));
            joined = true;
        }
        return RK_OK;
    }
    int wait_inv()
    {
        if (inv_recorded && !joined) RK_HIP(b.ctx, hipStreamWaitEvent(b.st, b.ctx->ev_inv, 0));
        else RK_TRY(join());
        return RK_OK;
    }
    int ensure_table()
    {
        if (!inv || rl_tab.p) return RK_OK;
        RK_HIP(b.ctx, rl_tab.alloc(b.p.N));
        hipLaunchKernelGGL(k_emit_table, dim3(blocks_for(b.p.N)), dim3(kThreads), 0, b.st, inv, b.idx->d_src_off, b.p.N, rl_tab.p);
        return RK_OK;
    }
    int branch_heads(hipStream_t *sh)
    {
        RK_HIP(b.ctx, hipEventRecord(b.ctx->ev_fork, b.st));
        RK_HIP(b.ctx, hipStreamWaitEvent(b.ctx->stream2, b.ctx->ev_fork, 0));
        *sh = b.ctx->stream2;
        return RK_OK;
    }
    int heads_branched()
    {
        RK_HIP(b.ctx, hipEventRecord(b.ctx->ev_join, b.ctx->stream2));
        joined = false;
        return RK_OK;
    }
    int enqueue(bool want_tab);
    int enqueue_identity();
};

int Renumbering::enqueue(bool want_tab)
{
    if (enqueued) return RK_OK;
    enqueued = true;
    if (!b.p.relabel) return enqueue_identity();
    rk_ctx *ctx = b.ctx;
    rk_index *idx = b.idx;
    const BuildSource &src = b.src;
    const uint32_t N = b.p.N;
    hipStream_t s2 = b.st;
    if (b.p.two_streams) {
        s2 = ctx->stream2;
        RK_HIP(ctx, hipStreamWaitEvent(s2, ctx->ev_fork, 0));
        forked = true;
    }
    const int id_bits = b.p.gb;
    uint32_t slots = 1024;
    const unsigned long long want_slots = b.k.table_x * N * kMinK;
    while (slots < want_slots && slots < (1u << 30)) slots <<= 1;
    RK_HIP(ctx, rl_table.alloc(slots));
    RK_HIP(ctx, rl_parent.alloc(N));
    RK_HIP(ctx, hipMemsetAsync(rl_table.p, 0xFF, (size_t)slots * 8, s2));
    const unsigned nb_ins = (unsigned)(((uint64_t)N * kMinK + kInsertThreads - 1) / kInsertThreads), nb_n = blocks_for(N);
    auto insert_and_vote = [&](auto rs) {
        using R = decltype(rs);
        hipLaunchKernelGGL(k_minhash_insert<R>, dim3(nb_ins), dim3(kInsertThreads), 0, s2, rs, N, rl_table.p, slots - 1);
        hipLaunchKernelGGL(k_minhash_vote<R>, dim3(nb_n), dim3(kThreads), 0, s2, rs, N, rl_table.p, slots - 1, rl_parent.p);
    };
    if (src.d_sig) insert_and_vote(SigMinK{src.d_sig});
    else if (idx->wide) insert_and_vote(CsrMinK<uint64_t>{src.s->d_hashes64, src.s->d_off});
    else insert_and_vote(CsrMinK<uint32_t>{src.s->d_hashes, src.s->d_off});
    if (N <= kRankMaxN) {
// ... 541 lines not shown
            break;
        case AttemptOutcome::FallBackToSlices:
            rs.tiles_mode = false;
            drop_blk_min(ctx, idx);
            rep[RK_REPORT_FELL_BACK] = 1;
            break;
        default: again = false;
        }
    }
    rep[RK_REPORT_FLAGS] = o.flags;
    rep[RK_REPORT_HEAVY] = o.heavy;
    rep[RK_REPORT_PASSES] = o.passes;
    const bool built = o.what == AttemptOutcome::Built;
    if (!built && p.from_keys && (o.flags & kFastBadHash))
        return rk_fail(ctx, RK_ERR_ARG, "rk_index_build_shard_keys: a key outside the wire format (hash bits beyond the shard's range, or a genome id >= %u)", p.N);
    if (!built && n_shards > 1)
        return rk_fail(ctx, RK_ERR_UNSUPPORTED, "rk_index_build_shard: the bucket sort refused this collection (flags %s: a bucket or a pass beyond its "
                                                "buffer, a hash outside the hash space, or tile records beyond their capacity)", o.tr.overflow ? "tile overflow" : "bucket / key overflow");
    if (!built) {
        if (idx->d_blk_min) drop_blk_min(ctx, idx);
        RK_TRY(alloc_slices(ctx, idx, p));
    }

    RK_TRY(rn.enqueue(false));
    RK_TRY(rn.join());
    BuildResult r = built ? o.r : BuildResult{0, 0, 0, 0, 0};
    if (!built && p.H) {
        RK_TRY(build_general(b, res.p, &r));
        rep[RK_REPORT_GENERAL] = 1;
    } else if (!p.H) RK_TRY(build_empty(b));
    idx->U = r.U;
    idx->n_self = r.n_self;
    idx->slices_refused = p.no_self;
    idx->ref_sets = src.is_set || r.dups == 0;
    idx->built_fast = built;
    if (built) {
        idx->spread = r.flagged * 8 > r.n_self;
        idx->spread_known = 1;
    }
    set_dir_shape(idx);
    guard.p = nullptr;
    *out = idx;
    return RK_OK;
}

}

__global__ void k_slices_from_lists(const uint32_t *postings, const uint32_t *upos, uint64_t U, uint2 *raw, uint32_t *pos)
{
    const uint64_t u = (uint64_t)blockIdx.x * blockDim.x + threadIdx.x;
    if (u >= U) return;
    const uint32_t s = upos[u], e = upos[u + 1];
    const uint32_t last = e > s ? postings[e - 1] : 0u;
    uint32_t prev = 0xFFFFFFFFu;
    for (uint32_t k = s; k < e; k++) {
        const uint32_t g = postings[k];
        uint2 rec = make_uint2(0, 0);
        if (k + 1 < e) {
            const uint32_t first = postings[k + 1];
            const bool covered = (g & 1u) && prev == g - 1;
            if (last - first <= 31u) {
                uint32_t mask = 0;
                for (uint32_t m = k + 1; m < e; m++) mask |= 1u << (postings[m] - first);
                rec = make_uint2(0x80000000u | first, covered ? mask & ~1u : mask);
            } else {
                rec = make_uint2((k + 1) | (covered ? 0x40000000u : 0u), e | (first - g <= 32u ? 0x80000000u : 0u));
            }
        }
        raw[k] = rec;
        pos[k] = k;
        prev = g;
    }
}
__global__ void k_gather_slices(const uint2 *raw, const uint32_t *sorted_pos, uint64_t H, uint2 *out)
{
    const uint64_t e = (uint64_t)blockIdx.x * blockDim.x + threadIdx.x;
    if (e < H) out[e] = raw[sorted_pos[e]];
}

int rk_index_ensure_slices(rk_ctx *ctx, rk_index *idx, hipStream_t st)
{
    std::lock_guard<std::mutex> lk(idx->lazy_mu);
    if (idx->d_selfrange) return RK_OK;
    if (idx->slices_refused || idx->H >= (1ULL << 30) || !idx->ref_sets || !idx->d_src_off || idx->wide != (idx->d_uhash64 != nullptr))
        return rk_fail(ctx, RK_ERR_UNSUPPORTED, "this index has no slice records (2^31 postings or more, or RK_INDEX_NO_SELF): only sparse self "
                                                "joins (a threshold below distance 1.0) run on it");
    const auto t_begin = std::chrono::steady_clock::now();
    const uint64_t H = idx->H, U = idx->U;
    const uint32_t N = idx->n_ref;
    DevBuf<uint2> raw(ctx), self_raw(ctx), out(ctx);
    DevBuf<uint32_t> pos(ctx), keys_sorted(ctx), pos_sorted(ctx), n_open(ctx), n_cov(ctx);
    DevBuf<uint64_t> self_off(ctx), self_split(ctx);
    DevBuf<BuildResult> res(ctx);
    RK_HIP(ctx, raw.alloc(H));
    RK_HIP(ctx, self_raw.alloc(H));
    RK_HIP(ctx, out.alloc(H + 1));
    RK_HIP(ctx, pos.alloc(H));
    RK_HIP(ctx, keys_sorted.alloc(H));
    RK_HIP(ctx, pos_sorted.alloc(H));
    RK_HIP(ctx, n_open.alloc((size_t)N + 1));
    RK_HIP(ctx, n_cov.alloc((size_t)N + 1));
    RK_HIP(ctx, self_off.alloc((size_t)N + 1));
    RK_HIP(ctx, self_split.alloc((size_t)N + 1));
    RK_HIP(ctx, res.alloc(1));
    RK_HIP(ctx, hipMemsetAsync(res.p, 0, sizeof(BuildResult), st));
    BuildResult r{0, 0, 0, 0, 0};
    if (H) {
        hipLaunchKernelGGL(k_slices_from_lists, dim3(blocks_for(U)), dim3(kThreads), 0, st, idx->d_postings, idx->d_upos, U, raw.p, pos.p);
        RK_HIP(ctx, hipGetLastError());
        int gbits = 1;
        while ((1ULL << gbits) < N) gbits++;
        RK_TRY(rk_prim_sort_pairs_u32_u32(ctx, idx->d_postings, keys_sorted.p, pos.p, pos_sorted.p, H, (unsigned)gbits, st));
        hipLaunchKernelGGL(k_gather_slices, dim3(blocks_for(H)), dim3(kThreads), 0, st, raw.p, pos_sorted.p, H, self_raw.p);
        const unsigned wave_blocks = (N + 3) / 4;
        hipLaunchKernelGGL(k_row_counts2, dim3(wave_blocks), dim3(kThreads), 0, st, idx->d_src_off, N, self_raw.p, n_open.p, n_cov.p);
        hipLaunchKernelGGL(k_row_scan, dim3(1), dim3(1024), 0, st, n_open.p, n_cov.p, N, self_off.p, self_split.p, res.p);
        hipLaunchKernelGGL(k_row_place2, dim3(wave_blocks), dim3(kThreads), 0, st, idx->d_src_off, N, self_raw.p, self_off.p, self_split.p, out.p);
        RK_HIP(ctx, hipGetLastError());
        RK_TRY(rk_read_back(ctx, &r, res.p, sizeof(r), st));
    } else {
        RK_HIP(ctx, hipMemsetAsync(self_off.p, 0, ((size_t)N + 1) * 8, st));
        RK_HIP(ctx, hipMemsetAsync(self_split.p, 0, ((size_t)N + 1) * 8, st));
        RK_HIP(ctx, hipStreamSynchronize(st));
    }
    idx->n_self = r.n_self;
    idx->d_self_off = self_off.release();
    idx->d_self_split = self_split.release();
    idx->d_selfrange = out.release();
    if (ctx->sw_dist_debug)
        fprintf(stderr, "[rk] slice records built on first use: %llu records in %.3f ms\n", (unsigned long long)r.n_self,
                std::chrono::duration<double, std::milli>(std::chrono::steady_clock::now() - t_begin).count());
    return RK_OK;
}

int rk_index_ensure_dir(rk_ctx *ctx, rk_index *idx, hipStream_t st)
{
    std::lock_guard<std::mutex> lk(idx->lazy_mu);
    if (idx->d_dir) return RK_OK;
    const uint32_t nb = 1u << idx->dir_bits;
    DevBuf<uint32_t> dir(ctx);
    RK_HIP(ctx, dir.alloc((size_t)nb + 1));
    if (idx->wide)
        hipLaunchKernelGGL(k_dir<uint64_t>, dim3(blocks_for((uint64_t)nb + 1)), dim3(kThreads), 0, st,
                           idx->d_uhash64, idx->U, idx->dir_shift, nb, dir.p);
    else
        hipLaunchKernelGGL(k_dir<uint32_t>, dim3(blocks_for((uint64_t)nb + 1)), dim3(kThreads), 0, st,
                           idx->d_uhash, idx->U, idx->dir_shift, nb, dir.p);
    RK_HIP(ctx, hipGetLastError());
    RK_HIP(ctx, hipStreamSynchronize(st));
    idx->d_dir = dir.release();
    return RK_OK;
}

extern "C" {

void rk_index_free(rk_index *idx)
{
    if (!idx) return;
    rk_ctx *ctx = idx->ctx;
    rk_pool_free(ctx, idx->d_postings);
    rk_pool_free(ctx, idx->d_uhash);
    rk_pool_free(ctx, idx->d_uhash64);
    rk_pool_free(ctx, idx->d_upos);
    rk_pool_free(ctx, idx->d_dir);
    rk_pool_free(ctx, idx->d_rankbm);
    rk_pool_free(ctx, idx->d_rankbase);
    rk_pool_free(ctx, idx->d_urec);
    rk_pool_free(ctx, idx->d_sizes);
    rk_pool_free(ctx, idx->d_selfrange);
    rk_pool_free(ctx, idx->d_shard_rec);
    rk_pool_free(ctx, idx->d_self_off);
    rk_pool_free(ctx, idx->d_self_split);
    rk_pool_free(ctx, idx->d_src_off);
    rk_pool_free(ctx, idx->d_orig);
    rk_pool_free(ctx, idx->d_fb);
    rk_pool_free(ctx, idx->d_tile_contrib);
    rk_pool_free(ctx, idx->d_tile_rows);
    rk_pool_free(ctx, idx->d_tile_cols);
    rk_pool_free(ctx, idx->d_tile_key);
    rk_pool_free(ctx, idx->d_tile_start);
    rk_pool_free(ctx, idx->d_blk_min);
    rk_pool_free(ctx, idx->d_tile_dir[0]);
    rk_pool_free(ctx, idx->d_tile_dir[1]);
    rk_pool_free(ctx, idx->d_tile_order[0]);
    rk_pool_free(ctx, idx->d_tile_order[1]);
    if (idx->h_fb_seen) (void)hipHostFree(idx->h_fb_seen);
    if (idx->fb_event) (void)hipEventDestroy((hipEvent_t)idx->fb_event);
    delete idx;
}

int rk_index_order(const rk_index *idx, uint32_t *orig_out)
{
    if (!idx || (!orig_out && idx->n_ref)) return RK_ERR_ARG;
    rk_ctx *ctx = idx->ctx;
    if (!idx->relabeled || !idx->d_orig) {
        for (uint32_t i = 0; i < idx->n_ref; i++) orig_out[i] = i;
        return RK_OK;
    }
    RK_HIP(ctx, hipSetDevice(ctx->device));
    RK_HIP(ctx, hipMemcpyAsync(orig_out, idx->d_orig, (size_t)idx->n_ref * 4, hipMemcpyDeviceToHost, ctx->stream));
    RK_HIP(ctx, hipStreamSynchronize(ctx->stream));
    return RK_OK;
}

uint64_t rk_index_total(const rk_index *idx) { return idx ? idx->H : 0; }
uint64_t rk_index_distinct(const rk_index *idx) { return idx ? idx->U : 0; }
uint32_t rk_index_genomes(const rk_index *idx) { return idx ? idx->n_ref : 0; }
int rk_index_hash_bits(const rk_index *idx) { return idx ? idx->hash_bits : 0; }
int rk_index_built_fast(const rk_index *idx) { return idx && idx->built_fast ? 1 : 0; }
int rk_index_build_report(const rk_index *idx, uint64_t out[8])
{
    if (!idx || !out) return RK_ERR_ARG;
    for (int i = 0; i < RK_REPORT_WORDS; i++) out[i] = idx->build_report[i];
    return RK_OK;
}
int rk_index_products(const rk_index *idx)
{
    if (!idx) return 0;
    return (idx->d_selfrange ? 1 : 0) | (idx->tiles_ready ? 2 : 0) | (idx->tiles_ready && idx->tiles_from_build ? 4 : 0);
}

uint64_t rk_index_sum_sq(const rk_index *cidx)
{
    if (!cidx) return 0;
    rk_index *idx = const_cast<rk_index *>(cidx);
    std::lock_guard<std::mutex> lk(idx->lazy_mu);
    if (idx->sum_sq_known) return idx->sum_sq;
    rk_ctx *ctx = idx->ctx;
    if (hipSetDevice(ctx->device) != hipSuccess) return 0;
    DevBuf<unsigned long long> acc(ctx);
    if (acc.alloc(1) != hipSuccess || hipMemsetAsync(acc.p, 0, 8, ctx->stream) != hipSuccess) return 0;
    if (idx->U)
        hipLaunchKernelGGL(k_sum_sq, dim3(blocks_for(idx->U)), dim3(kThreads), 0, ctx->stream, idx->d_upos, idx->U, acc.p);
    unsigned long long ss = 0;
    if (rk_read_back(ctx, &ss, acc.p, 8, ctx->stream) != RK_OK) return 0;
    idx->sum_sq = ss;
    idx->sum_sq_known = true;
    return ss;
}

int rk_index_self_stats(const rk_index *cidx, uint64_t out[4])
{
    if (!cidx || !out) return RK_ERR_ARG;
    rk_index *idx = const_cast<rk_index *>(cidx);
    std::lock_guard<std::mutex> lk(idx->lazy_mu);
    rk_ctx *ctx = idx->ctx;
    if (!idx->self_stats_known && idx->d_selfrange && idx->n_ref) {
        RK_HIP(ctx, hipSetDevice(ctx->device));
        DevBuf<unsigned long long> acc(ctx);
        RK_HIP(ctx, acc.alloc(2));
        RK_HIP(ctx, hipMemsetAsync(acc.p, 0, 16, ctx->stream));
        hipLaunchKernelGGL(k_self_stats, dim3((idx->n_ref + 3) / 4), dim3(kThreads), 0, ctx->stream, idx->d_selfrange, idx->d_self_off,
                           idx->d_self_split, idx->n_ref, acc.p);
        RK_HIP(ctx, hipGetLastError());
        unsigned long long v[2] = {0, 0};
        RK_TRY(rk_read_back(ctx, v, acc.p, 16, ctx->stream));
        idx->self_stats[0] = idx->n_self;
        idx->self_stats[1] = v[0];
        idx->self_stats[2] = v[1];
        idx->self_stats_known = true;
    }
    idx->self_stats[3] = idx->tiles_ready ? idx->n_tile_records : 0;
    for (int i = 0; i < 4; i++) out[i] = idx->self_stats[i];
    return RK_OK;
}


static int settle_streams(rk_ctx *ctx, int rc)
{
    if (rc && ctx) {
        if (ctx->stream2) (void)hipStreamSynchronize(ctx->stream2);
        if (ctx->stream) (void)hipStreamSynchronize(ctx->stream);
        (void)hipGetLastError();
    }
    return rc;
}

int rk_index_build(rk_ctx *ctx, const rk_sketches *s, int hash_bits, rk_index **out)
{
    if (!ctx || !s || !out) return RK_ERR_ARG;
    return settle_streams(ctx, index_build_impl(ctx, source_of(s), hash_bits, 0, 1, out));
}

int rk_index_build_plan(rk_ctx *ctx, const rk_sketches *s, int hash_bits, uint32_t shard, uint32_t n_shards, int64_t out[])
{
    if (!ctx) return RK_ERR_ARG;
    if (!n_shards || n_shards > kRecRegions || (n_shards & (n_shards - 1)) || shard >= n_shards)
        return rk_fail(ctx, RK_ERR_ARG, "rk_index_build_plan: %u shards (a power of two up to %u), shard %u", n_shards, kRecRegions, shard);
    if (!s || !out) return RK_ERR_ARG;
    const BuildKnobs k = read_knobs();
    BuildPlan p;
    RK_TRY(plan_build(ctx, source_of(s), hash_bits, shard, n_shards, k, &p));
    AttemptPlan a;
    RK_TRY(plan_attempt(ctx, p, k, RetryState{p.tiles_mode}, &a));
    out[RK_PLAN_FAST_OK] = p.fast_ok();
    out[RK_PLAN_TILES_MODE] = p.tiles_mode;
    out[RK_PLAN_SLICES_OK] = p.slices_ok;
    out[RK_PLAN_TILES_OK] = p.tiles_ok;
    out[RK_PLAN_B] = p.B;
    out[RK_PLAN_LOW_BITS] = p.low_bits;
    out[RK_PLAN_GB] = p.gb;
    out[RK_PLAN_RB] = p.rb;
    out[RK_PLAN_N_PASS] = p.n_pass;
    out[RK_PLAN_RANGE_BITS] = p.range_bits;
    out[RK_PLAN_PART2] = a.part2;
    out[RK_PLAN_USE_FILTER] = a.use_filter;
    out[RK_PLAN_SMALL_WGS] = a.small_wgs;
    out[RK_PLAN_NARROW] = a.narrow;
    out[RK_PLAN_BIG_OK] = a.big_ok;
    out[RK_PLAN_RELABEL] = p.relabel;
    out[RK_PLAN_TWO_STREAMS] = p.two_streams;
    out[RK_PLAN_EMIT_T] = with_emit_shape(k.emit_t, a.narrow, [](auto threads, auto) -> int { return decltype(threads)::value; });
    out[RK_PLAN_KEYS_CAP] = (int64_t)a.keys_cap;
    out[RK_PLAN_REC_CAP] = (int64_t)a.rec_cap;
    return RK_OK;
}

int rk_index_build_shard(rk_ctx *ctx, const rk_sketches *s, int hash_bits, uint32_t shard, uint32_t n_shards, rk_index **out)
{
    if (!ctx) return RK_ERR_ARG;
    if (!n_shards || n_shards > kRecRegions || (n_shards & (n_shards - 1)) || shard >= n_shards)
        return rk_fail(ctx, RK_ERR_ARG, "rk_index_build_shard: %u shards (a power of two up to %u), shard %u", n_shards, kRecRegions, shard);
    if (!s || !out) return RK_ERR_ARG;
    return settle_streams(ctx, index_build_impl(ctx, source_of(s), hash_bits, shard, n_shards, out));
}


namespace {
struct PackArgs {
    unsigned long long dst[kRecRegions];
    unsigned long long cnt[kRecRegions];
// ... 361 lines not shown
```

rabbitkssd_amd/csrc/rk_index_tiles.inc:

```

constexpr uint32_t kRecRegions = 64;
constexpr uint32_t kRecParts = 8;
constexpr uint32_t kCrowdedSub = 768;
constexpr uint32_t kTileMaxBlocks = 16384;

struct TileResult {
    unsigned long long overflow;
    unsigned long long n_records, n_slots, n_tiles, max_records;
    unsigned long long level_count[2][kTileTable + 1];
    unsigned long long rec_count[kRecRegions];
};
struct TileCursors {
    unsigned long long final_at, tile_at;
    unsigned long long ticket;
    unsigned long long level_at[2][kTileTable + 1];
};

struct TileEmitArgs {
    const unsigned long long *keys;
    const uint32_t *bstart;
    const uint32_t *inv;
    int low_bits, gb, rb;
    uint32_t nb;
    uint32_t *postings;
    uint32_t *tmp_uhash, *tmp_upos;
    unsigned long long *tmp_uhash64;
    uint32_t *ucount;
    uint3 *rec;
    uint32_t region_cap;
    const unsigned long long *pass_base;
    unsigned long long hash_base;
    uint32_t n_dest;
    const BuildResult *stop;
    int big_ok;
    BuildResult *stop_rw;
    uint32_t *big_list, *n_big;
    TileResult *tres;
    int xcd_map;
    int debug;
};

__device__ inline uint32_t tile_level(uint32_t n, uint32_t lb)
{
    const float ratio = (float)n / (float)lb;
    if (!(ratio > 0.0f)) return kTileTable;
    auto theta = [](int k) { return exp2f(-(float)k / 8.0f) * (1.0f - 1e-4f); };
    const float kf = ceilf(-8.0f * log2f(ratio));
    int k = kf < 0.0f ? 0 : (kf > (float)kTileTable ? kTileTable : (int)kf);
    while (k > 0 && ratio >= theta(k - 1)) k--;
    while (k < kTileTable && !(ratio >= theta(k))) k++;
    return (uint32_t)k;
}

template <int T, class K>
__device__ inline uint32_t emit_sorted_bucket(const TileEmitArgs &a, const K *S, uint16_t *hd, uint16_t *rpos, uint32_t *wave_part, uint32_t *s_cnt,
                                              uint32_t *s_cur, unsigned long long *s_dbase, uint32_t n, uint32_t b, uint32_t post_base, uint32_t head_base,
                                              unsigned long long hash_hi, bool write_ucount, uint32_t *rmask)
{
    constexpr uint32_t NW = T / 64, EPT = kBucketCap / T;
    const uint32_t tid = threadIdx.x, lane = tid & 63, wave = tid >> 6;
    const uint32_t gmask = (1u << a.gb) - 1u;
    const uint32_t per = (n + T - 1) / T;
    const uint32_t k0 = min(n, tid * per), k1 = min(n, k0 + per);
    auto genome = [&](uint32_t k) { return (uint32_t)S[k] & gmask; };
    uint32_t head_bits = 0, run_bits = 0;
    {
        K prev = k0 ? S[k0 - 1] : (K)0;
#pragma unroll
        for (uint32_t i = 0; i < EPT; i++) {
            const uint32_t k = k0 + i;
            if (i < per && k < k1) {
                const K cur = S[k];
                const bool head = k == 0 || (cur >> a.gb) != (prev >> a.gb);
                const bool run = head || (((uint32_t)cur & gmask) >> 5) != (((uint32_t)prev & gmask) >> 5);
                head_bits |= (head ? 1u : 0u) << i;
                run_bits |= (run ? 1u : 0u) << i;
                prev = cur;
            }
        }
    }
    const uint32_t mine = (uint32_t)__popc(head_bits) + ((uint32_t)__popc(run_bits) << 16);
    uint32_t incl = mine;
    for (int o = 1; o < 64; o <<= 1) {
        const uint32_t t = __shfl_up(incl, o);
        if ((int)lane >= o) incl += t;
    }
    if (lane == 63) wave_part[wave] = incl;
    __syncthreads();
    uint32_t before = incl - mine, all = 0;
    for (uint32_t w = 0; w < NW; w++) {
        if (w < wave) before += wave_part[w];
        all += wave_part[w];
    }
    const uint32_t U = all & 0xFFFFu, R = all >> 16;
    {
        uint32_t at_h = before & 0xFFFFu, at_r = before >> 16;
#pragma unroll
        for (uint32_t i = 0; i < EPT; i++) {
            if (i >= per) break;
            const uint32_t k = k0 + i;
            const bool head = (head_bits >> i) & 1u;
            if (head) hd[at_h++] = (uint16_t)k;
            if ((run_bits >> i) & 1u) rpos[at_r++] = (uint16_t)(k | (head ? 0x8000u : 0u));
        }
        if (tid == 0) {
            hd[U] = (uint16_t)n;
            rpos[R] = (uint16_t)(n | 0x8000u);
        }
    }
    __syncthreads();
    if (tid == 0 && write_ucount) a.ucount[b] = U;
    if (a.debug & 4) return U;

    auto run_at = [&](uint32_t r) { return (uint32_t)rpos[r] & 0x7FFFu; };
    auto walk_mask = [&](uint32_t r) {
        uint32_t m = 0;
        for (uint32_t k = run_at(r), e = run_at(r + 1); k < e; k++) m |= 1u << (genome(k) & 31u);
        return m;
    };
    if (rmask) {
        for (uint32_t r = tid; r < R; r += T) rmask[r] = walk_mask(r);
        __syncthreads();
    }
    auto run_mask = [&](uint32_t r) { return rmask ? rmask[r] : walk_mask(r); };
    const uint32_t n_dest = a.n_dest, n_sub_regions = kRecRegions / n_dest;
    auto dest_of = [&](uint32_t row_block) { return n_dest > 1 ? row_block % n_dest : 0u; };
    bool outputs_done = false;
    auto outputs = [&]() {
        if (a.debug & 2) return;
        for (uint32_t k = tid; k < n; k += T) a.postings[post_base + k] = genome(k);
        for (uint32_t gi = tid; gi < U; gi += T) {
            const uint32_t k = hd[gi];
            const unsigned long long hh = hash_hi | (unsigned long long)(S[k] >> a.gb);
            if (a.tmp_uhash64) a.tmp_uhash64[head_base + gi] = hh;
            else a.tmp_uhash[head_base + gi] = (uint32_t)hh;
            a.tmp_upos[head_base + gi] = post_base + k;
        }
    };
    auto count_run = [&](uint32_t j, bool add, uint32_t &earlier, bool &self) {
        earlier = 0;
        for (uint32_t i = j; !(rpos[i] & 0x8000u); i--) {
            earlier++;
            if (add) atomicAdd(&s_cnt[dest_of(genome(run_at(i - 1)) >> 5)], 1u);
        }
        self = run_at(j + 1) - run_at(j) >= 2;
        if (self && add) atomicAdd(&s_cnt[dest_of(genome(run_at(j)) >> 5)], 1u);
    };
    auto place_run = [&](uint32_t j, uint32_t earlier, bool self) {
        const uint32_t mask_j = run_mask(j), wj = genome(run_at(j)) >> 5;
        for (uint32_t i = j; i > j - earlier; i--) {
            const uint32_t bi = genome(run_at(i - 1)) >> 5, d = dest_of(bi);
            const unsigned long long base = s_dbase[d];
            const uint32_t at = atomicAdd(&s_cur[d], 1u);
            if (base != ~0ULL) a.rec[base + at] = make_uint3((bi << 16) | wj, run_mask(i - 1), mask_j);
        }
        if (self) {
            const uint32_t d = dest_of(wj);
            const unsigned long long base = s_dbase[d];
            const uint32_t at = atomicAdd(&s_cur[d], 1u);
            if (base != ~0ULL) a.rec[base + at] = make_uint3((wj << 16) | wj, mask_j, mask_j);
        }
    };
    auto reserve = [&]() {
        uint32_t want = 0;
        unsigned long long got = 0;
        uint32_t region = 0;
        if (tid < n_dest) {
// ... 294 lines not shown
                const bool take = k < n && hl >= hl_lo && hl < hl_hi;
                const unsigned long long m = __ballot(take);
                if (!m) continue;
                uint32_t at = 0;
                if (lane == 0) at = atomicAdd(&s_fill, (uint32_t)__popcll(m));
                at = (uint32_t)__shfl((int)at, 0);
                if (take) S[at + (uint32_t)__popcll(m & ((1ULL << lane) - 1ULL))] = (hl << a.gb) | gi_of(full);
            }
            __syncthreads();
            if (!(a.debug & 64)) bitonic_sort_lds<T>(S, p2);
            const uint32_t U = emit_sorted_bucket<T, K>(a, S, hd, rpos, wave_part, s_cnt, s_cur, s_dbase, tot, b, pb + s0 + post_off, pb + s0 + heads_done,
                                                        hash_hi, false, bitmap);
            __syncthreads();
            heads_done += U;
        };
        auto heavy_list = [&](uint32_t hl, uint32_t post_off) {
            for (uint32_t w = tid; w < h.n_blocks; w += T) bitmap[w] = 0;
            __syncthreads();
            for (uint32_t k = tid; k < n; k += T) {
                const unsigned long long full = keys[k];
                if (hl_of(full) == hl) {
                    const uint32_t g = gi_of(full);
                    atomicOr(&bitmap[g >> 5], 1u << (g & 31u));
                }
            }
            __syncthreads();
            const uint32_t wpt = (h.n_blocks + T - 1) / T, w0 = min(h.n_blocks, tid * wpt), w1 = min(h.n_blocks, w0 + wpt);
            unsigned long long mine = 0;
            for (uint32_t w = w0; w < w1; w++) {
                const uint32_t m = bitmap[w];
                mine += (unsigned long long)__popc(m) + (m ? (1ULL << 32) : 0ULL);
            }
            unsigned long long incl = mine;
            for (int o = 1; o < 64; o <<= 1) {
                const unsigned long long t = (unsigned long long)__shfl_up((long long)incl, o);
                if ((int)lane >= o) incl += t;
            }
            if (lane == 63) wave_part64[wave] = incl;
            __syncthreads();
            unsigned long long before = incl - mine, all = 0;
            for (uint32_t w = 0; w < NW; w++) {
                if (w < wave) before += wave_part64[w];
                all += wave_part64[w];
            }
            const uint32_t R = (uint32_t)(all >> 32);
            {
                uint32_t at_p = (uint32_t)before, at_r = (uint32_t)(before >> 32);
                for (uint32_t w = w0; w < w1; w++) {
                    uint32_t m = bitmap[w];
                    if (m) nz[at_r++] = (uint16_t)w;
                    while (m) {
                        const int bit = __builtin_ctz(m);
                        m &= m - 1;
                        a.postings[pb + s0 + post_off + at_p++] = (w << 5) + (uint32_t)bit;
                    }
                }
            }
            if (tid == 0) {
                const unsigned long long hh = hash_hi | hl;
                if (a.tmp_uhash64) a.tmp_uhash64[pb + s0 + heads_done] = hh;
                else a.tmp_uhash[pb + s0 + heads_done] = (uint32_t)hh;
                a.tmp_upos[pb + s0 + heads_done] = pb + s0 + post_off;
            }
            __syncthreads();
            for (uint32_t i = tid; i < R; i += T) {
                const uint32_t w = nz[i];
                atomicAdd(&s_cnt[dest_of(w)], (R - 1 - i) + (__popc(bitmap[w]) >= 2 ? 1u : 0u));
            }
            __syncthreads();
            if (tid < n_dest) {
                const uint32_t want = s_cnt[tid];
                s_cnt[tid] = 0;
                s_cur[tid] = 0;
                const uint32_t region = tid * n_sub_regions + b % n_sub_regions;
                unsigned long long base = ~0ULL;
                if (want) {
                    const unsigned long long got = atomicAdd(&a.tres->rec_count[region], (unsigned long long)want);
                    if (got + want <= a.region_cap) base = (unsigned long long)region * a.region_cap + got;
                    else a.tres->overflow = 1;
                }
                s_dbase[tid] = base;
            }
            __syncthreads();
            for (uint32_t i = wave; i < R && !(a.debug & 1); i += NW) {
                const uint32_t wi = nz[i], mi = bitmap[wi], d = dest_of(wi);
                const bool self = __popc(mi) >= 2;
                const uint32_t cnt = (R - 1 - i) + (self ? 1u : 0u);
                uint32_t at = 0;
                if (lane == 0 && cnt) at = atomicAdd(&s_cur[d], cnt);
                at = (uint32_t)__shfl((int)at, 0);
                const unsigned long long base = s_dbase[d];
                if (base == ~0ULL) continue;
                for (uint32_t j = i + 1 + lane; j < R; j += 64) {
                    const uint32_t wj = nz[j];
                    a.rec[base + at + (j - i - 1)] = make_uint3((wi << 16) | wj, mi, bitmap[wj]);
                }
                if (self && lane == 0) a.rec[base + at + (R - 1 - i)] = make_uint3((wi << 16) | wi, mi, mi);
            }
            __syncthreads();
            heads_done += 1;
        };

        uint32_t sidx = 0;
        while (sidx < n_sub) {
            const uint32_t base = sbo[sidx];
            uint32_t lo = sidx, hi = n_sub;
            while (lo < hi) {
                const uint32_t mid = (lo + hi + 1) >> 1;
                if (sbo[mid] - base <= kBucketCap) lo = mid; else hi = mid - 1;
            }
            if (lo > sidx) {
                const uint32_t tot = sbo[lo] - base;
                if (tot) light_slab(sidx << rest_bits, lo << rest_bits, tot, base);
                sidx = lo;
                continue;
            }
            if (rest_bits == 0) {
                heavy_list(sidx, sbo[sidx]);
            } else if (rest_bits > 6) {
                if (tid == 0) atomicOr((unsigned long long *)&a.stop_rw->flags, (unsigned long long)kFastOverflow);
            } else {
                const uint32_t n_val = 1u << rest_bits;
                if (tid < 64) hist2[tid] = 0;
                __syncthreads();
                for (uint32_t k = tid; k < n; k += T) {
                    const uint32_t hl = hl_of(keys[k]);
                    if ((hl >> rest_bits) == sidx) atomicAdd(&hist2[hl & (n_val - 1u)], 1u);
                }
                __syncthreads();
                uint32_t off2 = sbo[sidx], v = 0;
                while (v < n_val) {
                    const uint32_t c2 = hist2[v];
                    if (!c2) { v++; continue; }
                    if (c2 <= kBucketCap) {
                        uint32_t e2 = v, tot = 0;
                        while (e2 < n_val && tot + hist2[e2] <= kBucketCap) tot += hist2[e2++];
                        light_slab((sidx << rest_bits) + v, (sidx << rest_bits) + e2, tot, off2);
                        off2 += tot;
                        v = e2;
                    } else {
                        heavy_list((sidx << rest_bits) + v, off2);
                        off2 += c2;
                        v++;
                    }
                }
            }
            sidx++;
        }
        if (tid == 0) a.ucount[b] = heads_done;
        __syncthreads();
    }
}

struct TileSortArgs {
    const uint3 *rec;
    TileCursors *cur;
    uint32_t region_cap;
    uint32_t n_blocks;
    uint32_t *bin_count;
    uint32_t *bin_start;
    uint32_t *bin_cursor;
    uint3 *brec;
    const uint32_t *blk_min;
    uint2 *contrib;
    uint32_t *rows, *cols;
    uint32_t *tb_base, *tb_cnt;
    uint32_t *order;
    uint4 *proto;
    unsigned long long *level_start;
    uint4 *dir[2];
    TileResult *tres;
    uint32_t stage_slots;
    int debug;
};

__device__ inline void trec_share(const TileSortArgs &a, unsigned long long *lo, unsigned long long *hi)
{
    const unsigned long long cnt = min(a.tres->rec_count[blockIdx.x], (unsigned long long)a.region_cap);
    const unsigned long long share = (cnt + gridDim.y - 1) / gridDim.y;
    const unsigned long long base = (unsigned long long)blockIdx.x * a.region_cap;
    *lo = base + min(cnt, (unsigned long long)blockIdx.y * share);
    *hi = base + min(cnt, ((unsigned long long)blockIdx.y + 1) * share);
}

__device__ inline void trec_histogram(const TileSortArgs &a, unsigned long long lo, unsigned long long hi, uint32_t *h)
{
    constexpr int D = 8;
    for (unsigned long long i0 = lo + threadIdx.x; i0 < hi; i0 += (unsigned long long)D * blockDim.x) {
        uint32_t k[D];
#pragma unroll
        for (int d = 0; d < D; d++) {
            const unsigned long long i = i0 + (unsigned long long)d * blockDim.x;
            k[d] = i < hi ? a.rec[i].x : 0xFFFFFFFFu;
        }
#pragma unroll
        for (int d = 0; d < D; d++)
            if (k[d] != 0xFFFFFFFFu) atomicAdd(&h[k[d] >> 16], 1u);
    }
}

__global__ __launch_bounds__(512) void k_trec_count(TileSortArgs a)
{
    extern __shared__ uint32_t trec_lds[];
    if (a.tres->overflow) return;
    for (uint32_t i = threadIdx.x; i < a.n_blocks; i += blockDim.x) trec_lds[i] = 0;
    __syncthreads();
    unsigned long long lo, hi;
    trec_share(a, &lo, &hi);
    trec_histogram(a, lo, hi, trec_lds);
    __syncthreads();
    for (uint32_t i = threadIdx.x; i < a.n_blocks; i += blockDim.x)
        if (trec_lds[i]) atomicAdd(&a.bin_count[i], trec_lds[i]);
}

__global__ void k_trec_starts(TileSortArgs a)
{
    if (a.tres->overflow) return;
    const uint32_t all = block_scan_sweeps<uint32_t>(a.n_blocks, [&](uint32_t i) { return a.bin_count[i]; },
                                                     [&](uint32_t i, uint32_t before) { a.bin_start[i] = before; });
    if (threadIdx.x == 0) {
        a.bin_start[a.n_blocks] = all;
        a.tres->n_records = all;
    }
    __shared__ uint32_t n_first, n_rest;
    if (threadIdx.x == 0) n_first = n_rest = 0;
    __syncthreads();
    const uint32_t big = max(16384u, 8u * (all / a.n_blocks));
    const uint32_t lane = threadIdx.x & 63;
    for (int round = 0; round < 2; round++) {
        for (uint32_t i0 = threadIdx.x - lane; i0 < a.n_blocks; i0 += blockDim.x) {
            const uint32_t i = i0 + lane;
            const bool mine = i < a.n_blocks && (a.bin_count[i] > big) == (round == 0);
            const unsigned long long m = __ballot(mine);
            if (!m) continue;
            uint32_t at = 0;
            if (lane == 0) at = atomicAdd(round ? &n_rest : &n_first, (uint32_t)__popcll(m));
            at = (uint32_t)__shfl((int)at, 0) + (round ? n_first : 0u);
            if (mine) a.order[at + (uint32_t)__popcll(m & ((1ULL << lane) - 1ULL))] = i;
        }
        __syncthreads();
    }
}

__global__ __launch_bounds__(512) void k_trec_scatter(TileSortArgs a)
{
    extern __shared__ uint32_t trec_lds[];
    if (a.tres->overflow) return;
    for (uint32_t i = threadIdx.x; i < a.n_blocks; i += blockDim.x) trec_lds[i] = 0;
    __syncthreads();
    unsigned long long lo, hi;
    trec_share(a, &lo, &hi);
    trec_histogram(a, lo, hi, trec_lds);
    __syncthreads();
    for (uint32_t i = threadIdx.x; i < a.n_blocks; i += blockDim.x) {
        const uint32_t c = trec_lds[i];
        if (c) trec_lds[i] = a.bin_start[i] + atomicAdd(&a.bin_cursor[i], c);
    }
    __syncthreads();
    constexpr int D = 8;
    for (unsigned long long i0 = lo + threadIdx.x; i0 < hi; i0 += (unsigned long long)D * blockDim.x) {
        uint3 r[D];
#pragma unroll
        for (int d = 0; d < D; d++) {
            const unsigned long long i = i0 + (unsigned long long)d * blockDim.x;
            r[d] = i < hi ? a.rec[i] : make_uint3(0xFFFFFFFFu, 0, 0);
        }
#pragma unroll
        for (int d = 0; d < D; d++)
            if (r[d].x != 0xFFFFFFFFu) a.brec[atomicAdd(&trec_lds[r[d].x >> 16], 1u)] = r[d];
    }
}

constexpr uint32_t kRowStage = 6144;
inline uint32_t rowsort_stage(uint32_t n_blocks) { return n_blocks <= 8192 ? kRowStage : 0; }
inline size_t rowsort_lds(uint32_t n_blocks) { return (size_t)n_blocks * 4 + 8 + (size_t)rowsort_stage(n_blocks) * 8; }
template <uint32_t T> __global__ __launch_bounds__(T) void k_trec_rowsort(TileSortArgs a)
{
    extern __shared__ __attribute__((aligned(16))) uint32_t trec_lds[];
    __shared__ unsigned long long scan_part[T / 64];
    __shared__ unsigned long long s_slot0, s_tile0;
    __shared__ uint32_t lv[2][kTileTable + 1];
    __shared__ uint32_t s_ticket;
    if (a.tres->overflow) return;
    const uint32_t tid = threadIdx.x, lane = tid & 63, wave = tid >> 6, nb = a.n_blocks;
    uint32_t *cur = trec_lds;
    uint2 *stage = reinterpret_cast<uint2 *>(trec_lds + ((nb + 1) & ~1u));
    constexpr int D = T >= 1024 ? 16 : 8;
    for (;;) {
        __syncthreads();
        if (tid == 0) s_ticket = (uint32_t)atomicAdd(&a.cur->ticket, 1ULL);
        __syncthreads();
        const uint32_t it = s_ticket;
        if (it >= nb) break;
        const uint32_t b = a.order[it];
        const uint32_t r0 = a.bin_start[b], r1 = a.bin_start[b + 1];
        if (r0 == r1) {
            if (tid == 0) a.tb_cnt[it] = 0;
            continue;
        }
        for (uint32_t i = tid; i < nb; i += T) cur[i] = 0;
        for (uint32_t i = tid; i < 2 * (kTileTable + 1); i += T) (&lv[0][0])[i] = 0;
        __syncthreads();
        for (uint32_t i0 = r0 + tid; i0 < r1; i0 += D * T) {
            uint32_t k[D];
#pragma unroll
            for (int d = 0; d < D; d++) k[d] = i0 + d * T < r1 ? a.brec[i0 + d * T].x : 0xFFFFFFFFu;
#pragma unroll
            for (int d = 0; d < D; d++)
                if (k[d] != 0xFFFFFFFFu && !(a.debug & 4)) atomicAdd(&cur[k[d] & 0xFFFFu], 1u);
        }
        __syncthreads();
        const uint32_t per = ((nb + T - 1) / T) | 1u;
        const uint32_t w0 = min(nb, tid * per), w1 = min(nb, w0 + per);
        unsigned long long mine = 0;
        uint32_t biggest = 0;
        for (uint32_t w = w0; w < w1; w++) {
            const uint32_t c = cur[w];
            mine += (unsigned long long)((c + 1u) & ~1u) + (c ? (1ULL << 40) : 0ULL);
            biggest = max(biggest, c);
        }
        unsigned long long incl = mine;
        for (int o = 1; o < 64; o <<= 1) {
            const unsigned long long t = (unsigned long long)__shfl_up((long long)incl, o);
            if ((int)lane >= o) incl += t;
        }
        for (int o = 32; o > 0; o >>= 1) biggest = max(biggest, (uint32_t)__shfl_xor((int)biggest, o));
        if (lane == 63) scan_part[wave] = incl;
        __syncthreads();
        unsigned long long before = incl - mine, all = 0;
        for (uint32_t w = 0; w < T / 64; w++) {
            if (w < wave) before += scan_part[w];
            all += scan_part[w];
        }
        const unsigned long long n_slots = all & ((1ULL << 40) - 1ULL), n_tiles = all >> 40;
        const bool staged = n_slots <= a.stage_slots;
        if (tid == 0) {
            s_slot0 = atomicAdd(&a.cur->final_at, n_slots);
            s_tile0 = atomicAdd(&a.cur->tile_at, n_tiles);
            a.tb_base[it] = (uint32_t)s_tile0;
            a.tb_cnt[it] = (uint32_t)n_tiles;
        }
        if (lane == 0 && biggest) atomicMax(&a.tres->max_records, (unsigned long long)biggest);
        if (staged)
            for (uint32_t i = tid; i < (uint32_t)n_slots; i += T) stage[i] = make_uint2(0, 0);
        __syncthreads();
        const unsigned long long slot0 = s_slot0, tile0 = s_tile0;
        {
            uint32_t at = (uint32_t)(before & ((1ULL << 40) - 1ULL));
            unsigned long long t = tile0 + (before >> 40);
            const uint32_t mb = a.blk_min[b];
            for (uint32_t w = w0; w < w1; w++) {
                const uint32_t c = cur[w];
                cur[w] = at;
                if (c) {
                    const unsigned long long first = slot0 + at;
                    const uint32_t mw = a.blk_min[w];
                    const uint32_t lb_j = max(mb, mw), lb_c = min(mb, mw);
                    const uint32_t lj = tile_level(c, lb_j), lc = tile_level(c, lb_c);
                    a.proto[2 * t] = make_uint4(b, w, (uint32_t)first, (uint32_t)(first >> 32));
                    a.proto[2 * t + 1] = make_uint4(c, lb_j, lb_c, lj | (lc << 16));
                    atomicAdd(&lv[0][lj], 1u);
                    atomicAdd(&lv[1][lc], 1u);
                    t++;
                }
                at += (c + 1u) & ~1u;
            }
        }
        __syncthreads();
        if (staged) {
            for (uint32_t i0 = r0 + tid; i0 < r1; i0 += D * T) {
                uint3 r[D];
#pragma unroll
                for (int d = 0; d < D; d++) r[d] = i0 + d * T < r1 ? a.brec[i0 + d * T] : make_uint3(0xFFFFFFFFu, 0, 0);
#pragma unroll
                for (int d = 0; d < D; d++)
                    if (r[d].x != 0xFFFFFFFFu) stage[atomicAdd(&cur[r[d].x & 0xFFFFu], 1u)] = make_uint2(r[d].y, r[d].z);
            }
            __syncthreads();
            for (uint32_t i = tid; i < (uint32_t)n_slots; i += T) {
                const uint2 v = stage[i];
                a.contrib[slot0 + i] = v;
                a.rows[slot0 + i] = v.x;
                a.cols[slot0 + i] = v.y;
            }
        } else {
            for (uint32_t i0 = r0 + tid; i0 < r1; i0 += D * T) {
                uint3 r[D];
#pragma unroll
                for (int d = 0; d < D; d++) r[d] = i0 + d * T < r1 ? a.brec[i0 + d * T] : make_uint3(0xFFFFFFFFu, 0, 0);
#pragma unroll
                for (int d = 0; d < D; d++)
                    if (r[d].x != 0xFFFFFFFFu && !(a.debug & 1)) a.contrib[slot0 + atomicAdd(&cur[r[d].x & 0xFFFFu], 1u)] = make_uint2(r[d].y, r[d].z);
            }
            __syncthreads();
            for (unsigned long long i0 = tid; i0 < n_slots && a.rows && !(a.debug & 2); i0 += (unsigned long long)D * T) {
                uint2 v[D];
#pragma unroll
                for (int d = 0; d < D; d++) v[d] = i0 + (unsigned long long)d * T < n_slots ? a.contrib[slot0 + i0 + (unsigned long long)d * T] : make_uint2(0, 0);
#pragma unroll
                for (int d = 0; d < D; d++)
                    if (i0 + (unsigned long long)d * T < n_slots) {
                        a.rows[slot0 + i0 + (unsigned long long)d * T] = v[d].x;
                        a.cols[slot0 + i0 + (unsigned long long)d * T] = v[d].y;
                    }
            }
        }
        __syncthreads();
        for (uint32_t i = tid; i < 2 * (kTileTable + 1); i += T) {
            const uint32_t c = (&lv[0][0])[i];
            if (c) atomicAdd(&a.tres->level_count[0][0] + i, (unsigned long long)c);
        }
    }
}

__global__ void k_tdir_scan(TileSortArgs a)
{
    if (a.tres->overflow) return;
    const uint32_t m = threadIdx.x >> 9, l = threadIdx.x & 511;
    __shared__ unsigned long long part[2][512 / 64];
    const unsigned long long c = l <= (uint32_t)kTileTable ? a.tres->level_count[m][l] : 0ULL;
    unsigned long long incl = c;
    const uint32_t lane = threadIdx.x & 63, wv = l >> 6;
    for (int o = 1; o < 64; o <<= 1) {
        const unsigned long long t = (unsigned long long)__shfl_up((long long)incl, o);
        if ((int)lane >= o) incl += t;
    }
    if (lane == 63) part[m][wv] = incl;
    __syncthreads();
    for (uint32_t w = 0; w < wv; w++) incl += part[m][w];
    if (l <= (uint32_t)kTileTable) {
        a.level_start[m * (kTileTable + 1) + l] = incl - c;
        a.tres->level_count[m][l] = incl;
    }
    if (threadIdx.x == 0) {
        a.tres->n_tiles = a.cur->tile_at;
        a.tres->n_slots = a.cur->final_at;
    }
}

constexpr uint32_t kDirItems = 8;
__global__ __launch_bounds__(256) void k_tdir_place(TileSortArgs a)
{
    constexpr uint32_t T = 256;
    __shared__ unsigned long long at[2][kTileTable + 1];
    __shared__ uint32_t cnt[2][kTileTable + 1];
    if (a.tres->overflow) return;
    const uint32_t n_items = a.n_blocks, tid = threadIdx.x;
    const uint32_t it0 = blockIdx.x * kDirItems, it1 = min(n_items, it0 + kDirItems);
    if (it0 >= it1) return;
    for (uint32_t i = tid; i < 2 * (kTileTable + 1); i += T) (&cnt[0][0])[i] = 0;
    __syncthreads();
    for (uint32_t it = it0; it < it1; it++) {
        const uint32_t n = a.tb_cnt[it];
        const uint4 *mine = a.proto + 2 * (size_t)a.tb_base[it];
        for (uint32_t t = tid; t < n; t += T) {
            const uint32_t lv = mine[2 * t + 1].w;
            atomicAdd(&cnt[0][lv & 0xFFFFu], 1u);
            atomicAdd(&cnt[1][lv >> 16], 1u);
        }
    }
    __syncthreads();
    for (uint32_t i = tid; i < 2 * (kTileTable + 1); i += T) {
        const uint32_t c = (&cnt[0][0])[i];
        if (c) (&at[0][0])[i] = a.level_start[i] + atomicAdd(&a.cur->level_at[0][0] + i, (unsigned long long)c);
    }
    __syncthreads();
    for (uint32_t it = it0; it < it1; it++) {
        const uint32_t n = a.tb_cnt[it];
        const uint4 *mine = a.proto + 2 * (size_t)a.tb_base[it];
        for (uint32_t t = tid; t < n; t += T) {
            const uint4 e0 = mine[2 * t], e1 = mine[2 * t + 1];
#pragma unroll
            for (int m = 0; m < 2; m++) {
                const uint32_t lv = m ? (e1.w >> 16) : (e1.w & 0xFFFFu);
                const unsigned long long p = atomicAdd(&at[m][lv], 1ULL);
                a.dir[m][2 * p] = e0;
                a.dir[m][2 * p + 1] = make_uint4(e1.x, m ? e1.z : e1.y, e0.z, e0.w);
            }
        }
    }
}

__global__ void k_blk_min_sizes(const uint32_t *sizes, uint32_t n_ref, uint32_t n_blocks, uint32_t *blk_min)
{
    const uint32_t b = blockIdx.x * blockDim.x + threadIdx.x;
    if (b >= n_blocks) return;
    uint32_t m = 0xFFFFFFFFu;
    for (uint32_t g = b * 32; g < min(n_ref, b * 32 + 32); g++) {
        const uint32_t s = sizes[g];
        if (s && s < m) m = s;
    }
    blk_min[b] = m;
}

template <class F> int launch_tile_sort(rk_ctx *ctx, TileSortArgs ta, hipStream_t st, F before_rowsort)
{
    const size_t hist_lds = (size_t)ta.n_blocks * 4;
    ta.stage_slots = rowsort_stage(ta.n_blocks);
    ta.debug = getenv("RK_ROWSORT_DEBUG") ? atoi(getenv("RK_ROWSORT_DEBUG")) : 0;
    if (hist_lds > 48 * 1024) {
        RK_HIP(ctx, hipFuncSetAttribute((const void *)k_trec_count, hipFuncAttributeMaxDynamicSharedMemorySize, (int)hist_lds));
        RK_HIP(ctx, hipFuncSetAttribute((const void *)k_trec_scatter, hipFuncAttributeMaxDynamicSharedMemorySize, (int)hist_lds));
    }
    hipLaunchKernelGGL(k_trec_count, dim3(kRecRegions, kRecParts), dim3(512), hist_lds, st, ta);
    hipLaunchKernelGGL(k_trec_starts, dim3(1), dim3(1024), 0, st, ta);
    hipLaunchKernelGGL(k_trec_scatter, dim3(kRecRegions, kRecParts), dim3(512), hist_lds, st, ta);
    int rc = before_rowsort();
    if (rc) return rc;
    if (ta.stage_slots) {
        RK_HIP(ctx, hipFuncSetAttribute((const void *)k_trec_rowsort<512>, hipFuncAttributeMaxDynamicSharedMemorySize, (int)rowsort_lds(ta.n_blocks)));
        hipLaunchKernelGGL(k_trec_rowsort<512>, dim3(std::min(ta.n_blocks, 4096u)), dim3(512), rowsort_lds(ta.n_blocks), st, ta);
    } else {
        RK_HIP(ctx, hipFuncSetAttribute((const void *)k_trec_rowsort<1024>, hipFuncAttributeMaxDynamicSharedMemorySize, (int)rowsort_lds(ta.n_blocks)));
        hipLaunchKernelGGL(k_trec_rowsort<1024>, dim3(std::min(ta.n_blocks, 1024u)), dim3(1024), rowsort_lds(ta.n_blocks), st, ta);
    }
    hipLaunchKernelGGL(k_tdir_scan, dim3(1), dim3(1024), 0, st, ta);
    hipLaunchKernelGGL(k_tdir_place, dim3((ta.n_blocks + kDirItems - 1) / kDirItems), dim3(256), 0, st, ta);
    RK_HIP(ctx, hipGetLastError());
    return RK_OK;
}
```

rabbitkssd_amd/csrc/rk_internal.h:

```cpp
#pragma once
#include <hip/hip_runtime.h>

#include <cstdarg>
#include <cstdint>
#include <cstdio>
#include <cstdlib>
#include <map>
#include <mutex>
#include <string>
#include <tuple>
#include <unordered_map>
#include <vector>

#include "rabbitkssd.h"

struct rk_ctx {
    int device = 0;
    int num_cu = 0;
    size_t max_lds = 0;
    std::string err;
    hipStream_t stream = nullptr;
    hipStream_t stream2 = nullptr;
    hipEvent_t ev_fork = nullptr, ev_join = nullptr, ev_inv = nullptr;
    void *pinned = nullptr;
    size_t pinned_bytes = 0;
    std::mutex mu;
    std::multimap<size_t, void *> free_blocks;
    std::unordered_map<void *, size_t> live;
    size_t pool_bytes = 0;
    size_t cached_bytes = 0;
    uint64_t driver_allocs = 0, driver_frees = 0;
    std::vector<std::pair<void *, hipEvent_t>> deferred;
    std::vector<hipEvent_t> spare_events;
    size_t cache_limit = 0;
    std::map<std::tuple<const void *, int, size_t>, int> occupancy;
    bool single_shot = false;
    bool timing = false;
    hipEvent_t ev[2] = {nullptr, nullptr};
    double last_ms[15] = {0, 0, 0, 0, 0, 0, 0, 0, 0, 0, 0, 0, 0, 0, 0};
    rk_sketch_plan sketch_plan = {};
    bool sketch_plan_set = false;
    uint32_t sw_dist_threads = 0, sw_dist_rows = 0, sw_dist_pair = 1, sw_dist_pair_minwg = 3, sw_dist_persist = 1;
    uint32_t sw_dist_cand_cap = 0, sw_dist_stage_hits = 0, sw_dist_xcd_rows = 0;
    int sw_dist_bands = 1;
    int sw_dist_band_min_rows = 3072;
    int sw_dist_near = 1;
    int sw_dist_near_uw = 0;
    int sw_dist_fb_skip = 1;
    int sw_dist_tiles = 2;
    int sw_dist_tiles_min_genomes = 4000, sw_dist_tiles_min_shard_rows = 12000;
    int sw_dist_near_min = 16;
    int sw_dist_debug = 0;
    int sw_dist_lds_kb = 0;
    int sw_sketch_img = 2;
    int sw_index_fast = 1;
    int sw_index_relabel = 1;
    int sw_index_no_self = 0;
    int sw_index_heavy = 1;
    int sw_index_tiles = 2;
    unsigned long long sw_tile_rec_cap = 0;
    int sw_topn = 1;
    unsigned long long sw_topn_batch_bytes = 1ULL << 30;
    unsigned long long sw_topn_cand_cap = 0;
};
constexpr size_t kPinnedBytes = 1 << 16;

int rk_fail(rk_ctx *ctx, int code, const char *fmt, ...);
void *rk_pool_alloc(rk_ctx *ctx, size_t bytes);
void rk_pool_free(rk_ctx *ctx, void *p);
void rk_pool_free_after(rk_ctx *ctx, void *p, hipStream_t st);
int rk_read_back(rk_ctx *ctx, void *dst, const void *src_dev, size_t bytes, hipStream_t stream);
int rk_occupancy(rk_ctx *ctx, const void *kernel, int threads, size_t lds_bytes);
void *rk_pinned_scratch(rk_ctx *ctx, size_t bytes);

#define RK_HIP(ctx, call)                                                                   \
    do {                                                                                    \
        hipError_t e__ = (call);                                                            \
        if (e__ != hipSuccess)                                                              \
            return rk_fail((ctx), RK_ERR_HIP, "%s failed: %s (%s:%d)", #call,               \
                           hipGetErrorString(e__), __FILE__, __LINE__);                     \
    } while (0)
#define RK_TRY(call) do { int rc__ = (call); if (rc__) return rc__; } while (0)

constexpr int kThreads = 256;
inline unsigned blocks_for(uint64_t n, int t = kThreads) { return (unsigned)((n + t - 1) / t); }

struct TimedSpan {
    rk_ctx *ctx;
    int which;
    void clear() const { if (ctx->timing) ctx->last_ms[which] = 0.0; }
    hipError_t begin() const { return ctx->timing ? hipEventRecord(ctx->ev[0], ctx->stream) : hipSuccess; }
    hipError_t end() const { return ctx->timing ? hipEventRecord(ctx->ev[1], ctx->stream) : hipSuccess; }
    void read() const
    {
        float ms = 0.f;
        if (ctx->timing && hipEventElapsedTime(&ms, ctx->ev[0], ctx->ev[1]) == hipSuccess) ctx->last_ms[which] = ms;
    }
};

inline bool rk_switched_off(const char *name)
{
    const char *sw = getenv(name);
    return sw && atoi(sw) == 0;
}

template <class T> struct DevBuf {
    rk_ctx *ctx;
    T *p = nullptr;
    explicit DevBuf(rk_ctx *c) : ctx(c) {}
    DevBuf(const DevBuf &) = delete;
    DevBuf &operator=(const DevBuf &) = delete;
    ~DevBuf() { reset(); }
    hipError_t alloc(size_t n) {
        reset();
        p = static_cast<T *>(rk_pool_alloc(ctx, (n ? n : 1) * sizeof(T)));
        return p ? hipSuccess : hipErrorOutOfMemory;
    }
    void reset() {
        if (p) rk_pool_free(ctx, p);
        p = nullptr;
    }
    T *release() {
        T *q = p;
        p = nullptr;
        return q;
    }
    operator T *() const { return p; }
};

template <class T> inline int pool_array(rk_ctx *ctx, T **out, size_t n)
{
    *out = static_cast<T *>(rk_pool_alloc(ctx, (n ? n : 1) * sizeof(T)));
    return *out ? RK_OK : rk_fail(ctx, RK_ERR_NOMEM, "cannot allocate %llu bytes on the device", (unsigned long long)(n * sizeof(T)));
}

template <class T, void (*Free)(T *)> struct Owned {
    T *p;
    ~Owned() { if (p) Free(p); }
};

struct rk_filter {
    rk_ctx *ctx = nullptr;
    rk_params params{};
    int32_t *d_table = nullptr;
    uint32_t *d_bitmap = nullptr;
    int bitmap_bits = 0;
    bool exact = false;
    int img = 0;
    uint32_t n_keys = 0;
};

struct rk_sketches {
    rk_ctx *ctx = nullptr;
    uint32_t n = 0;
    uint64_t total = 0;
    uint64_t windows = 0;
    bool wide = false;
    uint32_t *d_hashes = nullptr;
    uint64_t *d_hashes64 = nullptr;
    uint64_t *d_off = nullptr;
    std::vector<uint64_t> h_off;
    bool is_set = false;
    uint64_t max_size = 0;
    std::mutex lazy_mu;
    uint32_t *d_member_rec = nullptr;
    uint32_t *d_member_seg = nullptr;
};

template <class F> int with_hash_type(bool wide, F f) { return wide ? f(uint64_t()) : f(uint32_t()); }
inline uint32_t *&hashes_of(rk_sketches *s, uint32_t) { return s->d_hashes; }
inline uint64_t *&hashes_of(rk_sketches *s, uint64_t) { return s->d_hashes64; }

struct rk_index {
    rk_ctx *ctx = nullptr;
    uint32_t n_ref = 0;
    uint64_t H = 0;
    uint64_t U = 0;
    int hash_bits = 0;
    int dir_bits = 0, dir_shift = 0;
    uint64_t sum_sq = 0;
    bool sum_sq_known = false;
    uint64_t self_stats[4] = {0, 0, 0, 0};
    bool self_stats_known = false;
    uint64_t max_src_size = 0;
    uint64_t max_ref_size = 0;
    uint64_t min_ref_size = 0;
    bool ref_sets = false;
    uint2 *d_rankbm = nullptr;
    uint32_t *d_rankbase = nullptr;
    uint2 *d_urec = nullptr;
    uint32_t *d_postings = nullptr;
    bool wide = false;
    uint32_t *d_uhash = nullptr;
    uint64_t *d_uhash64 = nullptr;
    uint32_t *d_upos = nullptr;
    uint32_t *d_dir = nullptr;
    uint32_t *d_sizes = nullptr;
    uint2 *d_selfrange = nullptr;
    uint64_t *d_self_off = nullptr;
    uint64_t *d_self_split = nullptr;
    uint64_t n_self = 0;
    uint64_t *d_src_off = nullptr;
    uint32_t *d_orig = nullptr;
    bool relabeled = false;
    bool built_fast = false;
    uint64_t build_report[8] = {0, 0, 0, 0, 0, 0, 0, 0};
    uint32_t *d_fb = nullptr;
    uint32_t *h_fb_seen = nullptr;
    unsigned char fb_key[40] = {0};
    int fb_state = 0;
    void *fb_event = nullptr;
    uint2 *d_tile_contrib = nullptr;
    uint32_t *d_tile_rows = nullptr, *d_tile_cols = nullptr;
    uint64_t n_tile_slots = 0, tile_max_records = 0;
    unsigned long long *d_tile_key = nullptr;
    unsigned long long *d_tile_start = nullptr;
    uint32_t *d_blk_min = nullptr;
    uint4 *d_tile_dir[2] = {nullptr, nullptr};
    uint32_t *d_tile_order[2] = {nullptr, nullptr};
    unsigned long long tile_prefix[2][256] = {};
    uint64_t n_tiles = 0, n_tile_records = 0;
    bool tiles_ready = false;
    bool tiles_from_build = false;
    uint3 *d_shard_rec = nullptr;
    uint32_t shard_region_cap = 0, n_shards = 0, shard_id = 0;
    unsigned long long shard_rec_count[64] = {};
    bool slices_refused = false;
    bool tiles_unusable = false;
    int spread_known = 0;
    bool spread = false;
    std::mutex lazy_mu;
};

using IndexGuard = Owned<rk_index, rk_index_free>;
using SketchesGuard = Owned<rk_sketches, rk_sketches_free>;

inline void set_dir_shape(rk_index *idx)
{
    int dbits = 10;
    while (dbits < 24 && (1ULL << dbits) < 2 * idx->U) dbits++;
    if (dbits > idx->hash_bits) dbits = idx->hash_bits;
    idx->dir_bits = dbits;
    idx->dir_shift = idx->hash_bits - dbits;
}

int rk_prim_sort_keys_u64(rk_ctx *ctx, const unsigned long long *in, unsigned long long *out, uint64_t n, unsigned begin_bit, unsigned end_bit,
                          hipStream_t st, void **tmp_keep = nullptr);
int rk_prim_sort_pairs_u32_u32(rk_ctx *ctx, const uint32_t *kin, uint32_t *kout, const uint32_t *vin, uint32_t *vout, uint64_t n, unsigned end_bit,
                               hipStream_t st);
int rk_prim_sort_pairs_u64_u32(rk_ctx *ctx, const uint64_t *kin, uint64_t *kout, const uint32_t *vin, uint32_t *vout, uint64_t n, unsigned end_bit,
                               hipStream_t st);
int rk_prim_inclusive_scan_u32(rk_ctx *ctx, const uint32_t *in, uint32_t *out, uint64_t n, hipStream_t st);
int rk_prim_exclusive_scan_u32(rk_ctx *ctx, const uint32_t *in, uint32_t *out, uint64_t n, hipStream_t st);
int rk_prim_unique_u64(rk_ctx *ctx, const unsigned long long *in, unsigned long long *out, unsigned long long *n_out_dev, uint64_t n, hipStream_t st);
int rk_prim_rle_u64(rk_ctx *ctx, const unsigned long long *in, uint64_t n, unsigned long long *runs, unsigned int *counts, unsigned long long *n_runs_dev,
                    hipStream_t st);
int rk_prim_select_u64(rk_ctx *ctx, const unsigned long long *in, const unsigned char *flags, unsigned long long *out, unsigned long long *n_out_dev,
                       uint64_t n, hipStream_t st);
int rk_prim_segmented_sort_u32(rk_ctx *ctx, const uint32_t *in, uint32_t *out, unsigned n, unsigned segments, const uint64_t *off, hipStream_t st);
int rk_prim_segmented_sort_u64(rk_ctx *ctx, const uint64_t *in, uint64_t *out, unsigned n, unsigned segments, const uint64_t *off, hipStream_t st);
int rk_prim_sort_hits(rk_ctx *ctx, const unsigned long long *keys, unsigned long long *keys_out, const rk_hit *hits, rk_hit *hits_out, uint64_t n,
                      unsigned end_bit, hipStream_t st);
constexpr int kTileTable = 256;
int rk_tiles_build(rk_ctx *ctx, rk_index *idx, hipStream_t stream);
int rk_index_ensure_slices(rk_ctx *ctx, rk_index *idx, hipStream_t stream);
int rk_index_ensure_dir(rk_ctx *ctx, rk_index *idx, hipStream_t stream);
int rk_distq_launch(rk_ctx *ctx, const rk_index *idx, const rk_sketches *queries, const rk_dist_opts *opts, bool dense_mode,
                    rk_hit *hits_dev, uint64_t cap, unsigned long long *n_hits_dev, int32_t *dense_dev,
                    hipStream_t stream);
int rk_distq_counts(rk_ctx *ctx, const rk_index *idx, const rk_sketches *queries, const rk_dist_opts *opts, uint32_t slot_base,
                    uint32_t n_slots, int32_t *counts_dev, hipStream_t stream);
uint64_t rk_host_exact_distances(rk_hit *h, uint64_t n, const rk_dist_opts *opts);
int rk_distq_kernel_name(rk_ctx *ctx, const rk_index *idx, const rk_sketches *queries, char *buf, size_t cap);
inline bool rk_dense_mode(const rk_dist_opts *o) { return o->triangle ? (1.0 < o->max_dist) : (1.0 <= o->max_dist); }
inline int rk_self_join_args(rk_ctx *ctx, const rk_index *idx, const rk_dist_opts *opts)
{
    if (!opts->triangle || !idx->d_src_off) return rk_fail(ctx, RK_ERR_ARG, "queries == NULL needs triangle=1 and an index built by rk_index_build");
    if (idx->n_shards > 1) return rk_fail(ctx, RK_ERR_ARG, "a shard of a sharded build holds the lists of one hash range: join through rk_index_join_shard");
    return RK_OK;
}
int rk_sketches_classify(rk_ctx *ctx, rk_sketches *s);
```

rabbitkssd_amd/csrc/rk_tiles.hip:

```cpp
#include <algorithm>
#include <chrono>
#include <cstdio>
#include <cstdlib>
#include <cstring>
#include <mutex>

#include <rocprim/rocprim.hpp>

#include "rk_internal.h"

namespace {


__global__ void k_list_starts(const uint32_t *upos, uint64_t U, uint8_t *starts)
{
    const uint64_t u = (uint64_t)blockIdx.x * blockDim.x + threadIdx.x;
    if (u >= U) return;
    const uint32_t p = upos[u];
    if (upos[u + 1] > p) starts[p] = 1;
}

__global__ void k_run_flags(const uint32_t *postings, const uint8_t *starts, uint64_t H, uint32_t *flags, uint32_t *bm)
{
    const uint64_t p = (uint64_t)blockIdx.x * blockDim.x + threadIdx.x;
    const bool in = p < H;
    const bool ls = in && starts[p];
    const bool run = in && (ls || (postings[p] >> 5) != (postings[p - (p ? 1 : 0)] >> 5));
    if (p <= H) flags[p] = run ? 1u : 0u;
    const unsigned long long m = __ballot(ls);
    if ((threadIdx.x & 31) == 0 && (p >> 5) <= (H >> 5)) bm[p >> 5] = (uint32_t)(m >> (threadIdx.x & 32));
}

__global__ void k_run_emit(const uint32_t *postings, const uint32_t *bm, const uint32_t *rank, uint64_t H, uint32_t *run_block,
                           uint32_t *run_mask, uint32_t *run_first, uint32_t *run_records)
{
    const uint64_t p = (uint64_t)blockIdx.x * blockDim.x + threadIdx.x;
    if (p >= H) return;
    const uint32_t j = rank[p];
    if (rank[p + 1] == j) return;
    const uint32_t blk = postings[p] >> 5;
    uint32_t mask = 1u << (postings[p] & 31);
    for (uint64_t q = p + 1; q < H && rank[q + 1] == rank[q]; q++) mask |= 1u << (postings[q] & 31);
    uint64_t wd = p >> 5;
    uint32_t bits = bm[wd] & (0xFFFFFFFFu >> (31 - (p & 31)));
    while (!bits) bits = bm[--wd];
    const uint64_t ls = (wd << 5) + (31 - __builtin_clz(bits));
    const uint32_t first = rank[ls];
    run_block[j] = blk;
    run_mask[j] = mask;
    run_first[j] = first;
    run_records[j] = (j - first) + (__popc(mask) >= 2 ? 1u : 0u);
}

__global__ void k_contrib_emit(const uint32_t *run_block, const uint32_t *run_mask, const uint32_t *run_first, const unsigned long long *run_at,
                               uint64_t n_runs, int kbits, unsigned long long *keys, uint2 *vals)
{
    const uint64_t j = (uint64_t)blockIdx.x * blockDim.x + threadIdx.x;
    if (j >= n_runs) return;
    const uint32_t wj = run_block[j], mj = run_mask[j];
    unsigned long long at = run_at[j];
    for (uint32_t i = run_first[j]; i < j; i++) {
        keys[at] = ((unsigned long long)run_block[i] << kbits) | wj;
        vals[at] = make_uint2(run_mask[i], mj);
        at++;
    }
    if (__popc(mj) >= 2) {
        keys[at] = ((unsigned long long)wj << kbits) | wj;
        vals[at] = make_uint2(mj, mj);
    }
}

__global__ void k_blk_min(const uint32_t *sizes, uint32_t n_ref, uint32_t n_blocks, uint32_t *blk_min)
{
    const uint32_t b = blockIdx.x * blockDim.x + threadIdx.x;
    if (b >= n_blocks) return;
    uint32_t m = 0xFFFFFFFFu;
    for (uint32_t g = b * 32; g < min(n_ref, b * 32 + 32); g++) {
        const uint32_t s = sizes[g];
        if (s && s < m) m = s;
    }
    blk_min[b] = m;
}

__global__ void k_tile_key_expand(const unsigned long long *packed, unsigned long long n, int kbits, unsigned long long *out)
{
    const unsigned long long i = (unsigned long long)blockIdx.x * blockDim.x + threadIdx.x;
    if (i < n) out[i] = ((packed[i] >> kbits) << 32) | (packed[i] & ((1ULL << kbits) - 1ULL));
}

__global__ void k_widen_u32(const uint32_t *in, uint64_t n, unsigned long long *out)
{
    const uint64_t i = (uint64_t)blockIdx.x * blockDim.x + threadIdx.x;
    if (i < n) out[i] = in[i];
}

__global__ void k_tile_ratio_keys(const unsigned long long *tile_key, const unsigned long long *tile_start, const uint32_t *blk_min,
                                  unsigned long long n_tiles, uint32_t *key_j, uint32_t *key_c, uint32_t *ids)
{
    const unsigned long long t = (unsigned long long)blockIdx.x * blockDim.x + threadIdx.x;
    if (t >= n_tiles) return;
    const unsigned long long key = tile_key[t];
    const uint32_t mb = blk_min[(uint32_t)(key >> 32)], mw = blk_min[(uint32_t)key];
    const float n = (float)(tile_start[t + 1] - tile_start[t]);
    key_j[t] = ~__float_as_uint(n / (float)max(mb, mw));
    key_c[t] = ~__float_as_uint(n / (float)min(mb, mw));
    ids[t] = (uint32_t)t;
}

__global__ void k_tile_prefix_table(const uint32_t *keys, unsigned long long n_tiles, unsigned long long *table)
{
    const int k = threadIdx.x;
    if (k >= kTileTable) return;
    const float theta = exp2f(-(float)k / 8.0f) * (1.0f - 1e-4f);
    const uint32_t limit = ~__float_as_uint(theta);
    unsigned long long lo = 0, hi = n_tiles;
    while (lo < hi) {
        const unsigned long long mid = (lo + hi) >> 1;
        if (keys[mid] <= limit) lo = mid + 1; else hi = mid;
    }
    table[k] = lo;
}

__global__ void k_tile_dir(const uint32_t *order, const unsigned long long *tile_key, const unsigned long long *tile_start,
                           const unsigned long long *slot_start, const uint32_t *blk_min, unsigned long long n_tiles, int metric, uint4 *out)
{
    const unsigned long long i = (unsigned long long)blockIdx.x * blockDim.x + threadIdx.x;
    if (i >= n_tiles) return;
    const uint32_t t = order[i];
    const unsigned long long key = tile_key[t], s0 = tile_start[t], n = tile_start[t + 1] - s0, d0 = slot_start[t];
    const uint32_t b = (uint32_t)(key >> 32), w = (uint32_t)key;
    const uint32_t mb = blk_min[b], mw = blk_min[w];
    out[2 * i] = make_uint4(b, w, (uint32_t)s0, (uint32_t)(s0 >> 32));
    out[2 * i + 1] = make_uint4((uint32_t)min(n, 0xFFFFFFFFULL), metric ? min(mb, mw) : max(mb, mw), (uint32_t)d0, (uint32_t)(d0 >> 32));
}

__global__ void k_tile_max(const unsigned long long *tile_start, unsigned long long n_tiles, unsigned long long *out)
{
    const unsigned long long t = (unsigned long long)blockIdx.x * blockDim.x + threadIdx.x;
    unsigned long long v = t < n_tiles ? tile_start[t + 1] - tile_start[t] : 0ULL;
    for (int o = 32; o > 0; o >>= 1) v = max(v, (unsigned long long)__shfl_xor((long long)v, o));
    if ((threadIdx.x & 63) == 0 && v) atomicMax(out, v);
}
__global__ void k_tile_padded_counts(const unsigned long long *tile_start, unsigned long long n_tiles, unsigned long long *padded)
{
    const unsigned long long t = (unsigned long long)blockIdx.x * blockDim.x + threadIdx.x;
    if (t < n_tiles) padded[t] = (tile_start[t + 1] - tile_start[t] + 1ULL) & ~1ULL;
}
__global__ void k_tile_split(const uint2 *recs, const unsigned long long *tile_start, const unsigned long long *slot_start, unsigned long long n_tiles,
                             uint32_t *rows, uint32_t *cols)
{
    const unsigned long long t = (unsigned long long)blockIdx.x * (blockDim.x >> 6) + (threadIdx.x >> 6);
    if (t >= n_tiles) return;
    const uint32_t lane = threadIdx.x & 63;
    const unsigned long long s0 = tile_start[t], n = tile_start[t + 1] - s0, d0 = slot_start[t];
    for (unsigned long long i = lane; i < n; i += 64) {
        const uint2 r = recs[s0 + i];
        rows[d0 + i] = r.x;
        cols[d0 + i] = r.y;
    }
}

#define RK_TILE_TRY(call) do { int rc__ = (call); if (rc__) return rc__; } while (0)

int tile_scan_u64(rk_ctx *ctx, unsigned long long *v, uint64_t n, unsigned long long *total, hipStream_t st)
{
    *total = 0;
    if (!n) return RK_OK;
    unsigned long long last_in = 0, last_out = 0;
    RK_TILE_TRY(rk_read_back(ctx, &last_in, v + (n - 1), 8, st));
    size_t tb = 0;
    RK_HIP(ctx, rocprim::exclusive_scan(nullptr, tb, v, v, 0ULL, n, rocprim::plus<unsigned long long>(), st));
    DevBuf<char> tmp(ctx);
    RK_HIP(ctx, tmp.alloc(tb));
    RK_HIP(ctx, rocprim::exclusive_scan(tmp.p, tb, v, v, 0ULL, n, rocprim::plus<unsigned long long>(), st));
    RK_TILE_TRY(rk_read_back(ctx, &last_out, v + (n - 1), 8, st));
    *total = last_in + last_out;
    return RK_OK;
}

}

static int tiles_build_body(rk_ctx *ctx, rk_index *idx, hipStream_t st);
int rk_tiles_build(rk_ctx *ctx, rk_index *idx, hipStream_t st)
{
    const int rc = tiles_build_body(ctx, idx, st);
    if (rc) {
        (void)hipStreamSynchronize(st);
        (void)hipGetLastError();
    }
    return rc;
}
static int tiles_build_body(rk_ctx *ctx, rk_index *idx, hipStream_t st)
{
    std::lock_guard<std::mutex> lk(idx->lazy_mu);
    if (idx->tiles_ready || idx->tiles_unusable) return RK_OK;
    const auto t_begin = std::chrono::steady_clock::now();
    const uint64_t H = idx->H, U = idx->U;
    const uint32_t n_blocks = (idx->n_ref + 31) / 32;
    const unsigned tpb = 256;
    auto nb = [&](uint64_t n) { return dim3((unsigned)((n + tpb - 1) / tpb)); };
    DevBuf<uint32_t> blk_min(ctx);
    RK_HIP(ctx, blk_min.alloc(n_blocks));
    hipLaunchKernelGGL(k_blk_min, nb(n_blocks), dim3(tpb), 0, st, idx->d_sizes, idx->n_ref, n_blocks, blk_min.p);
    DevBuf<unsigned long long> keys_out(ctx), tile_key(ctx), tile_start(ctx);
    DevBuf<uint2> vals_out(ctx);
    DevBuf<uint32_t> order_j(ctx), order_c(ctx);
    DevBuf<uint4> dir_j(ctx), dir_c(ctx);
    DevBuf<uint32_t> t_rows(ctx), t_cols(ctx);
    unsigned long long n_slots = 0;
    unsigned long long n_c = 0, n_t = 0;
    if (H && U) {
        DevBuf<uint32_t> bm(ctx), rank(ctx);
        DevBuf<uint8_t> starts(ctx);
        RK_HIP(ctx, bm.alloc(H / 32 + 2));
        RK_HIP(ctx, rank.alloc(H + 1));
        RK_HIP(ctx, starts.alloc(H + 1));
        RK_HIP(ctx, hipMemsetAsync(starts.p, 0, H + 1, st));
        hipLaunchKernelGGL(k_list_starts, nb(U), dim3(tpb), 0, st, idx->d_upos, U, starts.p);
        hipLaunchKernelGGL(k_run_flags, nb(H + 1), dim3(tpb), 0, st, idx->d_postings, starts.p, H, rank.p, bm.p);
        RK_HIP(ctx, hipGetLastError());
        uint32_t n_runs32 = 0;
        {
            size_t tb = 0;
            RK_HIP(ctx, rocprim::exclusive_scan(nullptr, tb, rank.p, rank.p, 0u, H + 1, rocprim::plus<uint32_t>(), st));
            DevBuf<char> tmp(ctx);
            RK_HIP(ctx, tmp.alloc(tb));
            RK_HIP(ctx, rocprim::exclusive_scan(tmp.p, tb, rank.p, rank.p, 0u, H + 1, rocprim::plus<uint32_t>(), st));
            RK_TILE_TRY(rk_read_back(ctx, &n_runs32, rank.p + H, 4, st));
        }
        const uint64_t n_runs = n_runs32;
        DevBuf<uint32_t> run_block(ctx), run_mask(ctx), run_first(ctx), run_records(ctx);
        DevBuf<unsigned long long> run_at(ctx);
        RK_HIP(ctx, run_block.alloc(n_runs));
        RK_HIP(ctx, run_mask.alloc(n_runs));
        RK_HIP(ctx, run_first.alloc(n_runs));
        RK_HIP(ctx, run_records.alloc(n_runs));
        RK_HIP(ctx, run_at.alloc(n_runs));
        hipLaunchKernelGGL(k_run_emit, nb(H), dim3(tpb), 0, st, idx->d_postings, bm.p, rank.p, H, run_block.p, run_mask.p, run_first.p,
                           run_records.p);
        hipLaunchKernelGGL(k_widen_u32, nb(n_runs), dim3(tpb), 0, st, run_records.p, n_runs, run_at.p);
        RK_HIP(ctx, hipGetLastError());
        RK_TILE_TRY(tile_scan_u64(ctx, run_at.p, n_runs, &n_c, st));
        {
            const char *env = getenv("RK_TILE_BUDGET");
            const unsigned long long budget = env ? strtoull(env, nullptr, 10) : 4ULL * H + (1ULL << 22);
            if (n_c > budget) {
                idx->tiles_unusable = true;
                if (ctx->sw_dist_debug) fprintf(stderr, "[rk] tiles: %llu records for %llu postings exceed the budget of %llu: not built\n", n_c, (unsigned long long)H, budget);
                RK_HIP(ctx, hipStreamSynchronize(st));
                return RK_OK;
            }
        }
        if (n_c) {
            DevBuf<unsigned long long> keys(ctx);
            DevBuf<uint2> vals(ctx);
            if (keys.alloc(n_c) != hipSuccess || vals.alloc(n_c) != hipSuccess || keys_out.alloc(n_c) != hipSuccess || vals_out.alloc(n_c + 256) != hipSuccess)
                return rk_fail(ctx, RK_ERR_NOMEM, "cannot allocate %llu tile records", n_c);
            int kbits = 1;
            while (kbits < 32 && (1u << kbits) < n_blocks) kbits++;
            hipLaunchKernelGGL(k_contrib_emit, nb(n_runs), dim3(tpb), 0, st, run_block.p, run_mask.p, run_first.p, run_at.p, n_runs, kbits, keys.p, vals.p);
            RK_HIP(ctx, hipGetLastError());
            int bbits = 1;
            while (bbits < 32 && (1u << bbits) < n_blocks) bbits++;
            size_t tb = 0;
            RK_HIP(ctx, rocprim::radix_sort_pairs(nullptr, tb, keys.p, keys_out.p, vals.p, vals_out.p, (size_t)n_c, 0, 2 * bbits, st));
            DevBuf<char> tmp(ctx);
            RK_HIP(ctx, tmp.alloc(tb));
            RK_HIP(ctx, rocprim::radix_sort_pairs(tmp.p, tb, keys.p, keys_out.p, vals.p, vals_out.p, (size_t)n_c, 0, 2 * bbits, st));
            DevBuf<unsigned long long> n_runs_out(ctx);
            DevBuf<uint32_t> counts(ctx);
            RK_HIP(ctx, n_runs_out.alloc(1));
            RK_HIP(ctx, counts.alloc(n_c));
            size_t tb2 = 0;
            RK_HIP(ctx, rocprim::run_length_encode(nullptr, tb2, keys_out.p, (size_t)n_c, keys.p, counts.p, n_runs_out.p, st));
            DevBuf<char> tmp2(ctx);
            RK_HIP(ctx, tmp2.alloc(tb2));
            RK_HIP(ctx, rocprim::run_length_encode(tmp2.p, tb2, keys_out.p, (size_t)n_c, keys.p, counts.p, n_runs_out.p, st));
            RK_TILE_TRY(rk_read_back(ctx, &n_t, n_runs_out.p, 8, st));
            RK_HIP(ctx, tile_key.alloc(n_t));
            RK_HIP(ctx, tile_start.alloc(n_t + 1));
            hipLaunchKernelGGL(k_tile_key_expand, nb(n_t), dim3(tpb), 0, st, keys.p, n_t, bbits, tile_key.p);
            hipLaunchKernelGGL(k_widen_u32, nb(n_t), dim3(tpb), 0, st, counts.p, n_t, tile_start.p);
            RK_HIP(ctx, hipGetLastError());
            unsigned long long tot = 0;
            RK_TILE_TRY(tile_scan_u64(ctx, tile_start.p, n_t, &tot, st));
            RK_HIP(ctx, hipMemcpyAsync(tile_start.p + n_t, &n_c, 8, hipMemcpyHostToDevice, st));
            RK_HIP(ctx, hipStreamSynchronize(st));
            if (tot != n_c) return rk_fail(ctx, RK_ERR_HIP, "tile directory does not add up (%llu vs %llu records)", tot, n_c);
            if (n_t >= 0xFFFFFFFFULL) return rk_fail(ctx, RK_ERR_UNSUPPORTED, "more than 2^32-1 tiles");
            DevBuf<uint32_t> key_j(ctx), key_c(ctx), ids(ctx), key_out(ctx);
            DevBuf<unsigned long long> table(ctx);
            RK_HIP(ctx, key_j.alloc(n_t));
            RK_HIP(ctx, key_c.alloc(n_t));
            RK_HIP(ctx, ids.alloc(n_t));
            RK_HIP(ctx, key_out.alloc(n_t));
            RK_HIP(ctx, order_j.alloc(n_t));
            RK_HIP(ctx, order_c.alloc(n_t));
            RK_HIP(ctx, table.alloc(2 * kTileTable + 1));
            RK_HIP(ctx, hipMemsetAsync(table.p + 2 * kTileTable, 0, 8, st));
            hipLaunchKernelGGL(k_tile_max, nb(n_t), dim3(tpb), 0, st, tile_start.p, n_t, table.p + 2 * kTileTable);
            hipLaunchKernelGGL(k_tile_ratio_keys, nb(n_t), dim3(tpb), 0, st, tile_key.p, tile_start.p, blk_min.p, n_t, key_j.p, key_c.p, ids.p);
            RK_HIP(ctx, hipGetLastError());
            size_t tb3 = 0;
            RK_HIP(ctx, rocprim::radix_sort_pairs(nullptr, tb3, key_j.p, key_out.p, ids.p, order_j.p, (size_t)n_t, 0, 32, st));
            DevBuf<char> tmp3(ctx);
            RK_HIP(ctx, tmp3.alloc(tb3));
            RK_HIP(ctx, rocprim::radix_sort_pairs(tmp3.p, tb3, key_j.p, key_out.p, ids.p, order_j.p, (size_t)n_t, 0, 32, st));
            hipLaunchKernelGGL(k_tile_prefix_table, dim3(1), dim3(kTileTable), 0, st, key_out.p, n_t, table.p);
            RK_HIP(ctx, hipStreamSynchronize(st));
            RK_HIP(ctx, rocprim::radix_sort_pairs(tmp3.p, tb3, key_c.p, key_out.p, ids.p, order_c.p, (size_t)n_t, 0, 32, st));
            hipLaunchKernelGGL(k_tile_prefix_table, dim3(1), dim3(kTileTable), 0, st, key_out.p, n_t, table.p + kTileTable);
            DevBuf<unsigned long long> slot_start(ctx);
            RK_HIP(ctx, slot_start.alloc(n_t + 1));
            hipLaunchKernelGGL(k_tile_padded_counts, nb(n_t), dim3(tpb), 0, st, tile_start.p, n_t, slot_start.p);
            RK_HIP(ctx, hipGetLastError());
            RK_TILE_TRY(tile_scan_u64(ctx, slot_start.p, n_t, &n_slots, st));
            RK_HIP(ctx, t_rows.alloc(n_slots + 256));
            RK_HIP(ctx, t_cols.alloc(n_slots + 256));
            RK_HIP(ctx, hipMemsetAsync(t_rows.p, 0, (n_slots + 256) * 4, st));
            RK_HIP(ctx, hipMemsetAsync(t_cols.p, 0, (n_slots + 256) * 4, st));
            hipLaunchKernelGGL(k_tile_split, dim3((unsigned)((n_t + 3) / 4)), dim3(256), 0, st, vals_out.p, tile_start.p, slot_start.p, n_t, t_rows.p, t_cols.p);
            RK_HIP(ctx, dir_j.alloc(2 * n_t));
            RK_HIP(ctx, dir_c.alloc(2 * n_t));
            hipLaunchKernelGGL(k_tile_dir, nb(n_t), dim3(tpb), 0, st, order_j.p, tile_key.p, tile_start.p, slot_start.p, blk_min.p, n_t, 0, dir_j.p);
            hipLaunchKernelGGL(k_tile_dir, nb(n_t), dim3(tpb), 0, st, order_c.p, tile_key.p, tile_start.p, slot_start.p, blk_min.p, n_t, 1, dir_c.p);
            RK_HIP(ctx, hipGetLastError());
            RK_HIP(ctx, hipStreamSynchronize(st));
            RK_HIP(ctx, hipGetLastError());
            RK_HIP(ctx, hipMemcpyAsync(idx->tile_prefix, table.p, sizeof(idx->tile_prefix), hipMemcpyDeviceToHost, st));
            RK_HIP(ctx, hipMemcpyAsync(&idx->tile_max_records, table.p + 2 * kTileTable, 8, hipMemcpyDeviceToHost, st));
            RK_HIP(ctx, hipStreamSynchronize(st));
        }
    }
    RK_HIP(ctx, hipStreamSynchronize(st));
    idx->d_tile_contrib = vals_out.release();
    idx->d_tile_rows = t_rows.release();
    idx->d_tile_cols = t_cols.release();
    idx->n_tile_slots = n_slots;
    idx->d_tile_key = tile_key.release();
    idx->d_tile_start = tile_start.release();
    idx->d_blk_min = blk_min.release();
    idx->d_tile_dir[0] = dir_j.release();
    idx->d_tile_dir[1] = dir_c.release();
    idx->d_tile_order[0] = order_j.release();
    idx->d_tile_order[1] = order_c.release();
    idx->n_tiles = n_t;
    idx->n_tile_records = n_c;
    idx->tiles_ready = true;
    if (ctx->sw_dist_debug)
        fprintf(stderr, "[rk] tiles: %llu tiles, %llu records, biggest tile %llu (%u genomes), built in %.3f ms\n", n_t, n_c, (unsigned long long)idx->tile_max_records, idx->n_ref,
                std::chrono::duration<double, std::milli>(std::chrono::steady_clock::now() - t_begin).count());
    return RK_OK;
}
```

Baseline: 2938 billion genome-pairs/s.

## Replace bit-sliced counter path with popcount accumulation over transposed tile copy

Replaces the bit-sliced carry-save counter kernel path with a per-lane popcount accumulation. Each wave reads 64-record steps of row bitmasks and column words, plus a per-step occupancy mask that lets it skip empty quarters, and then atomically adds the 32 per-lane counters into shared memory. A new tile copy kernel histogram-sorts records and writes 64-padded transposed rows/cols arrays with occupancy words. The copy can be deferred and built lazily after repeated asks. Occupancy bounds are raised to 7 for the popcount variant, which adds register pressure and LDS atomics.

```diff
diff --git a/rabbitkssd_amd/csrc/rk_core.hip b/rabbitkssd_amd/csrc/rk_core.hip
--- a/rabbitkssd_amd/csrc/rk_core.hip
+++ b/rabbitkssd_amd/csrc/rk_core.hip
@@ -289,6 +289,7 @@
     if (getenv("RK_INDEX_TILES")) ctx->sw_index_tiles = atoi(getenv("RK_INDEX_TILES"));
     if (getenv("RK_INDEX_NO_HEAVY")) ctx->sw_index_heavy = atoi(getenv("RK_INDEX_NO_HEAVY")) == 0;
     if (getenv("RK_TILE_REC_CAP")) ctx->sw_tile_rec_cap = strtoull(getenv("RK_TILE_REC_CAP"), nullptr, 10);
+    if (getenv("RK_TILE_COPY_BLOCKS")) ctx->sw_tile_copy_blocks = (unsigned)strtoul(getenv("RK_TILE_COPY_BLOCKS"), nullptr, 10);
     ctx->sw_topn = getenv("RK_DIST_TOPN") ? atoi(getenv("RK_DIST_TOPN")) != 0 : 1;
     if (getenv("RK_TOPN_BATCH_BYTES")) ctx->sw_topn_batch_bytes = std::max(1ULL, strtoull(getenv("RK_TOPN_BATCH_BYTES"), nullptr, 10));
     if (getenv("RK_TOPN_CAND_CAP")) ctx->sw_topn_cand_cap = strtoull(getenv("RK_TOPN_CAND_CAP"), nullptr, 10);
diff --git a/rabbitkssd_amd/csrc/rk_dist.hip b/rabbitkssd_amd/csrc/rk_dist.hip
--- a/rabbitkssd_amd/csrc/rk_dist.hip
+++ b/rabbitkssd_amd/csrc/rk_dist.hip
@@ -1104,7 +1104,10 @@
         if (!rc) rc = plan_self(ctx, idx, o, dense_mode, stream, &sp);
     }
     if (rc) return rc;
-    if (sp.kind == SelfPlan::kTiles) return launch_tiles(ctx, idx, o, sp.min_jorc, sp.tile, hits_dev, cap, n_hits_dev, stream);
+    if (sp.kind == SelfPlan::kTiles) {
+        rc = tile_copy_for_launch(ctx, mut, &sp.tile, stream);
+        return rc ? rc : launch_tiles(ctx, idx, o, sp.min_jorc, sp.tile, hits_dev, cap, n_hits_dev, stream);
+    }
     if (sp.kind == SelfPlan::kNear) return launch_near_and_fallback(ctx, mut, o, dense_mode, sp.near, hits_dev, cap, n_hits_dev, stream);
     if (ctx->sw_dist_debug) print_bands(sp.bands);
     for (size_t b = 0; !rc && b < sp.bands.size(); b++)
diff --git a/rabbitkssd_amd/csrc/rk_dist_tile.inc b/rabbitkssd_amd/csrc/rk_dist_tile.inc
--- a/rabbitkssd_amd/csrc/rk_dist_tile.inc
+++ b/rabbitkssd_amd/csrc/rk_dist_tile.inc
@@ -34,8 +34,8 @@
     return c2;
 }
 
-template <uint32_t kTileThreads, bool SROW>
-__global__ __launch_bounds__(kTileThreads, kTileThreads == 256 ? 6 : 4) void rk_tile_kernel(TileArgs a, const uint2 *__restrict__ contrib, const uint32_t *__restrict__ rows, const uint32_t *__restrict__ cols)
+template <uint32_t kTileThreads, bool POPC>
+__global__ __launch_bounds__(kTileThreads, kTileThreads == 256 ? 6 : POPC ? 7 : 4) void rk_tile_kernel(TileArgs a, const uint2 *__restrict__ contrib, const uint32_t *__restrict__ rows, const uint32_t *__restrict__ cols, const uint32_t *__restrict__ occ)
 {
     constexpr uint32_t kTileWaves = kTileThreads / 64;
     constexpr uint32_t kTileStage = (uint32_t)(8 * kTileThreads * sizeof(uint2) / sizeof(rk_hit));
@@ -161,24 +161,28 @@
             if (steps >= 1984) to_lds();
         };
         if (!(a.debug & 1)) {
-            if constexpr (SROW) {
+            if constexpr (POPC) {
                 constexpr int kDepth = 3;
                 const unsigned long long slot0 = (unsigned long long)d1.z | ((unsigned long long)d1.w << 32);
-                const unsigned long long *__restrict__ tile_rows = reinterpret_cast<const unsigned long long *>(rows + slot0);
-                const uint32_t n_rec = d1.x;
+                const uint32_t n_steps = (d1.x + 63u) >> 6;
                 const uint32_t wave_u = (uint32_t)__builtin_amdgcn_readfirstlane((int)wave);
-                const uint32_t per = ((n_rec + kTileWaves - 1) / kTileWaves + 127u) & ~127u;
-                const uint32_t w0 = min(n_rec, wave_u * per), w1 = min(n_rec, w0 + per);
-                const uint32_t n_sub = (w1 - w0 + 127u) / 128u;
-                const uint32_t *__restrict__ tile_cols = cols + slot0;
+                const uint32_t per = (n_steps + kTileWaves - 1) / kTileWaves;
+                const uint32_t st0 = min(n_steps, wave_u * per), st1 = min(n_steps, st0 + per);
+                const uint32_t n_sub = st1 - st0;
+                const uint32_t *__restrict__ tile_rows = rows + slot0 + (unsigned long long)st0 * 64ULL;
+                const uint32_t *__restrict__ tile_cols = cols + slot0 + (unsigned long long)st0 * 64ULL;
+                const uint32_t *__restrict__ tile_occ = occ + (slot0 >> 6) + st0;
                 uint32_t *mine = reinterpret_cast<uint32_t *>(recs + wave * 512);
-                uint32_t in0[kDepth], in1[kDepth];
-                auto request = [&](uint32_t sub, int slot) {
-                    const uint32_t at = w0 + sub * 128u + lane;
-                    in0[slot] = tile_cols[at];
-                    in1[slot] = tile_cols[at + 64u];
+                uint32_t in_r[kDepth], in_c[kDepth], in_o[kDepth];
+                auto request = [&](uint32_t sub, int d) {
+                    in_r[d] = tile_rows[sub * 64u + lane];
+                    in_c[d] = tile_cols[sub * 64u + lane];
+                    in_o[d] = tile_occ[sub];
                 };
-                const uint32_t put0 = (lane & 1u) * 64u + (lane >> 1), put1 = put0 + 32u;
+                uint32_t acc[32];
+    #pragma unroll
+                for (int r = 0; r < 32; r++) acc[r] = 0;
+                uint32_t used = 0;
     #pragma unroll
                 for (int d = 0; d < kDepth; d++)
                     if ((uint32_t)d < n_sub) request((uint32_t)d, d);
@@ -187,79 +191,38 @@
                     for (int d = 0; d < kDepth; d++) {
                         const uint32_t sub = sub0 + d;
                         if (sub >= n_sub) break;
-                        const uint32_t at = w0 + sub * 128u + lane;
-                        uint32_t *slot = mine + (sub & 3u) * 128;
-                        slot[put0] = at < w1 ? in0[d] : 0u;
-                        slot[put1] = at + 64u < w1 ? in1[d] : 0u;
+                        uint32_t *slot = mine + (sub & 3u) * 64;
+                        slot[lane] = in_r[d];
+                        const uint32_t wcol = in_c[d];
+                        const uint32_t oc = (a.debug & 8192) ? 15u : (uint32_t)__builtin_amdgcn_readfirstlane((int)in_o[d]);
                         if (sub + kDepth < n_sub) request(sub + kDepth, d);
                         __builtin_amdgcn_fence(__ATOMIC_RELEASE, "wavefront");
                         __builtin_amdgcn_wave_barrier();
-                        const uint32_t n_here = min(128u, w1 - (w0 + sub * 128u));
-                        const uint4 *rd = reinterpret_cast<const uint4 *>(slot + 64 * half);
-                        const unsigned long long *pairs = tile_rows + ((w0 + sub * 128u) >> 1);
-                        const uint32_t n_groups = min(8u, (n_here + 15) / 16);
-                        auto masks_sel = [&](uint32_t g, const unsigned long long *sel, uint32_t (&m)[8]) {
-                            const uint4 r0 = rd[2 * g], r1 = rd[2 * g + 1];
-                            const uint32_t y[8] = {r0.x, r0.y, r0.z, r0.w, r1.x, r1.y, r1.z, r1.w};
-    #pragma unroll
-                            for (int j = 0; j < 8; j++)
-                                asm("v_cndmask_b32_e64 %0, 0, %1, %2" : "=v"(m[j]) : "v"(y[j]), "s"(sel[j]));
-                        };
-                        auto masks = [&](uint32_t g, uint32_t (&m)[8]) {
-                            unsigned long long sel[8];
-    #pragma unroll
-                            for (int j = 0; j < 8; j++) sel[j] = pairs[8 * g + j];
-                            const uint4 r0 = rd[2 * g], r1 = rd[2 * g + 1];
-                            const uint32_t y[8] = {r0.x, r0.y, r0.z, r0.w, r1.x, r1.y, r1.z, r1.w};
-    #pragma unroll
-                            for (int j = 0; j < 8; j++)
-                                asm("v_cndmask_b32_e64 %0, 0, %1, %2" : "=v"(m[j]) : "v"(y[j]), "s"(sel[j]));
-                        };
-                        uint32_t g = 0;
-                        auto carry32 = [&](uint32_t g0) -> uint32_t {
-                            unsigned long long sel[32];
-    #pragma unroll
-                            for (int j = 0; j < 32; j++) sel[j] = pairs[8 * g0 + j];
-                            uint32_t ma[8], mb[8];
-                            masks_sel(g0, sel, ma);
-                            masks_sel(g0 + 1, sel + 8, mb);
-                            const uint32_t c16a = carry16(ma, mb);
-                            masks_sel(g0 + 2, sel + 16, ma);
-                            masks_sel(g0 + 3, sel + 24, mb);
-                            const uint32_t c16b = carry16(ma, mb);
-                            return csa(p[4], c16a, c16b);
-                        };
-                        if (n_groups == 8 && !(a.debug & (256 | 512 | 1024))) {
-                            const uint32_t c32a = carry32(0);
-                            const uint32_t c32b = carry32(4);
-                            uint32_t carry = csa(p[5], c32a, c32b);
-    #pragma unroll
-                            for (int k = 6; k < kTilePlanes; k++) carry = ripple(p[k], carry);
-                            steps += 64;
-                            if (steps >= 1984) to_lds();
-                            g = 8;
-                        }
-                        for (; g + 3 < n_groups && !(a.debug & (256 | 512)); g += 4) {
-                            uint32_t carry = carry32(g);
-    #pragma unroll
-                            for (int k = 5; k < kTilePlanes; k++) carry = ripple(p[k], carry);
-                            steps += 32;
-                            if (steps >= 1984) to_lds();
-                        }
-                        for (; g + 1 < n_groups && !(a.debug & 256); g += 2) {
-                            uint32_t ma[8], mb[8];
-                            masks(g, ma);
-                            masks(g + 1, mb);
-                            if (a.debug & 8) { p[0] |= ma[0] | ma[1] | ma[2] | ma[3] | ma[4] | ma[5] | ma[6] | ma[7] | mb[0] | mb[7]; continue; }
-                            add16(ma, mb);
-                        }
-                        for (; g < n_groups; g++) {
-                            uint32_t m[8];
-                            masks(g, m);
-                            if (a.debug & 8) { p[0] |= m[0] | m[1] | m[2] | m[3] | m[4] | m[5] | m[6] | m[7]; continue; }
-                            add8(m);
+                        const uint4 *rd = reinterpret_cast<const uint4 *>(slot + 32 * half);
+                        used |= oc;
+    #pragma unroll
+                        for (int q = 0; q < 4; q++) {
+                            if (!(oc & (1u << q))) continue;
+                            const uint4 r0 = rd[2 * q], r1 = rd[2 * q + 1];
+                            acc[8 * q + 0] += (uint32_t)__builtin_popcount(r0.x & wcol);
+                            acc[8 * q + 1] += (uint32_t)__builtin_popcount(r0.y & wcol);
+                            acc[8 * q + 2] += (uint32_t)__builtin_popcount(r0.z & wcol);
+                            acc[8 * q + 3] += (uint32_t)__builtin_popcount(r0.w & wcol);
+                            acc[8 * q + 4] += (uint32_t)__builtin_popcount(r1.x & wcol);
+                            acc[8 * q + 5] += (uint32_t)__builtin_popcount(r1.y & wcol);
+                            acc[8 * q + 6] += (uint32_t)__builtin_popcount(r1.z & wcol);
+                            acc[8 * q + 7] += (uint32_t)__builtin_popcount(r1.w & wcol);
                         }
                         __builtin_amdgcn_wave_barrier();
+                    }
+                }
+                if (!(a.debug & 16)) {
+    #pragma unroll
+                    for (int q = 0; q < 4; q++) {
+                        if (!(used & (1u << q))) continue;
+    #pragma unroll
+                        for (int j = 0; j < 8; j++)
+                            if (acc[8 * q + j]) atomicAdd(&cnt[(8 * q + j) * 32 + (int)row], acc[8 * q + j]);
                     }
                 }
             } else {
@@ -348,7 +311,7 @@
                 }
             }
         }
-        if (!(a.debug & 16)) {
+        if (!POPC && !(a.debug & 16)) {
             constexpr int kAll = 16;
             uint32_t q[kAll];
             {
@@ -409,7 +372,7 @@
         for (uint32_t round = 0; round < 1024 / kTileThreads; round++) {
             if (s_cursor + kTileThreads > kTileStage) flush_stage();
             const uint32_t ci = round * kTileThreads + tid;
-            const uint32_t col = ci >> 5, r = ci & 31;
+            const uint32_t col = POPC ? ci & 31 : ci >> 5, r = POPC ? ci >> 5 : ci & 31;
             const uint32_t common = cnt[ci];
             cnt[ci] = 0;
             const uint32_t grow = b * 32 + r, gcol = w * 32 + col;
@@ -446,7 +409,7 @@
     }
 }
 
-struct TileShape { unsigned long long grid = 0; int threads = 256; bool srow = false; };
+struct TileShape { unsigned long long grid = 0; int threads = 256; bool srow = false; bool asks = false; };
 TileShape tile_launch_shape(const rk_index *idx, const rk_dist_opts *o, double min_jorc)
 {
     const int metric = o->metric != 0;
@@ -461,9 +424,21 @@
     if (grid / row_step < 150) threads = 1024;
     if (getenv("RK_TILE_THREADS")) threads = atoi(getenv("RK_TILE_THREADS"));
     if (threads != 512 && threads != 1024) threads = 256;
-    bool srow = threads >= 512 && grid && idx->n_tile_records >= kTileSrowPerTile * grid && idx->d_tile_rows;
-    if (getenv("RK_TILE_SROW")) srow = atoi(getenv("RK_TILE_SROW")) != 0 && idx->d_tile_rows;
-    return TileShape{grid, threads, srow};
+    const bool have = idx->d_tile_rows != nullptr, can = have || idx->tile_copy_deferred;
+    const bool rule = threads >= 512 && grid && idx->n_tile_records >= kTileSrowPerTile * grid;
+    const bool asks = rule && !have && idx->tile_copy_deferred;
+    bool srow = rule && (have || (asks && idx->tile_copy_asks + 1 >= kTileCopyAfter));
+    if (getenv("RK_TILE_SROW")) srow = atoi(getenv("RK_TILE_SROW")) != 0 && can;
+    return TileShape{grid, threads, srow, asks};
+}
+
+int tile_copy_for_launch(rk_ctx *ctx, rk_index *idx, TileShape *shape, hipStream_t stream)
+{
+    if (shape->asks) idx->tile_copy_asks++;
+    if (!shape->srow || idx->d_tile_rows) return RK_OK;
+    const int rc = rk_index_tile_copy(ctx, idx, stream);
+    if (!idx->d_tile_rows) shape->srow = false;
+    return rc;
 }
 
 int launch_tiles(rk_ctx *ctx, const rk_index *idx, const rk_dist_opts *o, double min_jorc, const TileShape &shape, rk_hit *hits_dev, uint64_t cap,
@@ -496,8 +471,8 @@
     if (shape.grid > 0x7FFFFFFFULL) return rk_fail(ctx, RK_ERR_UNSUPPORTED, "too many tiles for one launch (%llu)", (unsigned long long)idx->n_tiles);
 #define RK_TILE_LAUNCH(T)                                                                                                              \
     do {                                                                                                                               \
-        if (shape.srow) hipLaunchKernelGGL((rk_tile_kernel<T, true>), dim3((unsigned)shape.grid), dim3(T), 0, stream, a, (const uint2 *)idx->d_tile_contrib, (const uint32_t *)idx->d_tile_rows, (const uint32_t *)idx->d_tile_cols); \
-        else hipLaunchKernelGGL((rk_tile_kernel<T, false>), dim3((unsigned)shape.grid), dim3(T), 0, stream, a, (const uint2 *)idx->d_tile_contrib, (const uint32_t *)idx->d_tile_rows, (const uint32_t *)idx->d_tile_cols); \
+        if (shape.srow) hipLaunchKernelGGL((rk_tile_kernel<T, true>), dim3((unsigned)shape.grid), dim3(T), 0, stream, a, (const uint2 *)idx->d_tile_contrib, (const uint32_t *)idx->d_tile_rows, (const uint32_t *)idx->d_tile_cols, (const uint32_t *)idx->d_tile_occ); \
+        else hipLaunchKernelGGL((rk_tile_kernel<T, false>), dim3((unsigned)shape.grid), dim3(T), 0, stream, a, (const uint2 *)idx->d_tile_contrib, (const uint32_t *)idx->d_tile_rows, (const uint32_t *)idx->d_tile_cols, (const uint32_t *)idx->d_tile_occ); \
     } while (0)
     if (shape.threads == 512)
         RK_TILE_LAUNCH(512);
diff --git a/rabbitkssd_amd/csrc/rk_index.hip b/rabbitkssd_amd/csrc/rk_index.hip
--- a/rabbitkssd_amd/csrc/rk_index.hip
+++ b/rabbitkssd_amd/csrc/rk_index.hip
@@ -497,11 +497,13 @@
 
 struct TileSortBufs {
     DevBuf<uint3> brec;
-    DevBuf<uint32_t> tb, bins, t_rows, t_cols;
+    DevBuf<uint32_t> tb, bins;
+    DevBuf<unsigned long long> copy_slot;
+    uint64_t copy_cap = 0;
     DevBuf<uint4> proto, t_dir_j, t_dir_c;
     DevBuf<unsigned long long> level_start;
     DevBuf<uint2> t_contrib;
-    explicit TileSortBufs(rk_ctx *c) : brec(c), tb(c), bins(c), t_rows(c), t_cols(c), proto(c), t_dir_j(c), t_dir_c(c), level_start(c), t_contrib(c) {}
+    explicit TileSortBufs(rk_ctx *c) : brec(c), tb(c), bins(c), copy_slot(c), proto(c), t_dir_j(c), t_dir_c(c), level_start(c), t_contrib(c) {}
     int alloc(rk_ctx *ctx, uint32_t n_blocks, uint64_t n_records, uint64_t tile_cap)
     {
         const uint64_t slot_cap = n_records + tile_cap;
@@ -511,9 +513,9 @@
         RK_HIP(ctx, proto.alloc(2 * tile_cap));
         RK_HIP(ctx, level_start.alloc(2 * (kTileTable + 1)));
         RK_HIP(ctx, t_contrib.alloc(slot_cap + 256));
-        if (rowsort_stage(n_blocks)) {
-            RK_HIP(ctx, t_rows.alloc(slot_cap + 256));
-            RK_HIP(ctx, t_cols.alloc(slot_cap + 256));
+        if (n_blocks <= ctx->sw_tile_copy_blocks) {
+            copy_cap = ((n_records + 63) & ~(uint64_t)63) + 64 * tile_cap;
+            RK_HIP(ctx, copy_slot.alloc(tile_cap));
         }
         RK_HIP(ctx, t_dir_j.alloc(2 * tile_cap));
         RK_HIP(ctx, t_dir_c.alloc(2 * tile_cap));
@@ -533,8 +535,9 @@
         ta.brec = brec.p;
         ta.blk_min = blk_min;
         ta.contrib = t_contrib.p;
-        ta.rows = t_rows.p;
-        ta.cols = t_cols.p;
+        if (copy_cap) {
+            ta.copy_slot = copy_slot.p;
+        }
         ta.tb_base = tb.p;
         ta.tb_cnt = tb.p + n_blocks;
         ta.order = tb.p + 2 * (size_t)n_blocks;
@@ -548,8 +551,12 @@
     void hand_over(rk_index *idx, const TileResult &tr)
     {
         idx->d_tile_contrib = t_contrib.release();
-        idx->d_tile_rows = t_rows.release();
-        idx->d_tile_cols = t_cols.release();
+        if (copy_cap && tr.n_copy_slots && tr.n_copy_slots <= copy_cap) {
+            idx->d_tile_proto = proto.release();
+            idx->d_tile_copy_slot = copy_slot.release();
+            idx->n_tile_copy_slots = tr.n_copy_slots;
+            idx->tile_copy_deferred = true;
+        }
         idx->d_tile_dir[0] = t_dir_j.release();
         idx->d_tile_dir[1] = t_dir_c.release();
         idx->n_tile_slots = tr.n_slots;
@@ -1397,7 +1404,47 @@
     return RK_OK;
 }
 
+int rk_index_tile_copy(rk_ctx *ctx, rk_index *idx, hipStream_t st)
+{
+    std::lock_guard<std::mutex> lock(idx->lazy_mu);
+    if (!idx->tile_copy_deferred) return RK_OK;
+    idx->tile_copy_deferred = false;
+    DevBuf<uint4> proto(ctx);
+    DevBuf<unsigned long long> copy_slot(ctx);
+    proto.p = idx->d_tile_proto;
+    copy_slot.p = idx->d_tile_copy_slot;
+    idx->d_tile_proto = nullptr;
+    idx->d_tile_copy_slot = nullptr;
+    const uint64_t n = idx->n_tile_copy_slots;
+    DevBuf<uint32_t> rows(ctx), cols(ctx), occ(ctx);
+    DevBuf<uint2> scratch(ctx);
+    if (rows.alloc(n) != hipSuccess || cols.alloc(n) != hipSuccess || occ.alloc(n / 64) != hipSuccess || scratch.alloc(idx->n_tile_slots + 256) != hipSuccess) {
+        (void)hipGetLastError();
+        idx->n_tile_copy_slots = 0;
+        return RK_OK;
+    }
+    TileCopyArgs a;
+    memset(&a, 0, sizeof a);
+    a.recs = idx->d_tile_contrib;
+    a.proto = proto.p;
+    a.copy_slot = copy_slot.p;
+    a.n_tiles = idx->n_tiles;
+    a.cap = n;
+    a.sorted = scratch.p;
+    a.rows = rows.p;
+    a.cols = cols.p;
+    a.occ = occ.p;
+    launch_tile_copy(a, idx->n_tiles, st);
+    RK_HIP(ctx, hipGetLastError());
+    RK_HIP(ctx, hipStreamSynchronize(st));
+    idx->d_tile_rows = rows.release();
+    idx->d_tile_cols = cols.release();
+    idx->d_tile_occ = occ.release();
+    return RK_OK;
+}
+
 extern "C" {
+
 
 void rk_index_free(rk_index *idx)
 {
@@ -1422,6 +1469,9 @@
     rk_pool_free(ctx, idx->d_tile_contrib);
     rk_pool_free(ctx, idx->d_tile_rows);
     rk_pool_free(ctx, idx->d_tile_cols);
+    rk_pool_free(ctx, idx->d_tile_occ);
+    rk_pool_free(ctx, idx->d_tile_proto);
+    rk_pool_free(ctx, idx->d_tile_copy_slot);
     rk_pool_free(ctx, idx->d_tile_key);
     rk_pool_free(ctx, idx->d_tile_start);
     rk_pool_free(ctx, idx->d_blk_min);
diff --git a/rabbitkssd_amd/csrc/rk_index_tiles.inc b/rabbitkssd_amd/csrc/rk_index_tiles.inc
--- a/rabbitkssd_amd/csrc/rk_index_tiles.inc
+++ b/rabbitkssd_amd/csrc/rk_index_tiles.inc
@@ -7,12 +7,14 @@
 struct TileResult {
     unsigned long long overflow;
     unsigned long long n_records, n_slots, n_tiles, max_records;
+    unsigned long long n_copy_slots;
     unsigned long long level_count[2][kTileTable + 1];
     unsigned long long rec_count[kRecRegions];
 };
 struct TileCursors {
     unsigned long long final_at, tile_at;
     unsigned long long ticket;
+    unsigned long long copy_at;
     unsigned long long level_at[2][kTileTable + 1];
 };
 
@@ -613,6 +615,8 @@
     }
 }
 
+#include "rk_tile_copy.h"
+
 struct TileSortArgs {
     const uint3 *rec;
     TileCursors *cur;
@@ -624,7 +628,7 @@
     uint3 *brec;
     const uint32_t *blk_min;
     uint2 *contrib;
-    uint32_t *rows, *cols;
+    unsigned long long *copy_slot;
     uint32_t *tb_base, *tb_cnt;
     uint32_t *order;
     uint4 *proto;
@@ -738,8 +742,8 @@
 template <uint32_t T> __global__ __launch_bounds__(T) void k_trec_rowsort(TileSortArgs a)
 {
     extern __shared__ __attribute__((aligned(16))) uint32_t trec_lds[];
-    __shared__ unsigned long long scan_part[T / 64];
-    __shared__ unsigned long long s_slot0, s_tile0;
+    __shared__ unsigned long long scan_part[T / 64], scan_part2[T / 64];
+    __shared__ unsigned long long s_slot0, s_tile0, s_copy0;
     __shared__ uint32_t lv[2][kTileTable + 1];
     __shared__ uint32_t s_ticket;
     if (a.tres->overflow) return;
@@ -773,31 +777,44 @@
         __syncthreads();
         const uint32_t per = ((nb + T - 1) / T) | 1u;
         const uint32_t w0 = min(nb, tid * per), w1 = min(nb, w0 + per);
-        unsigned long long mine = 0;
+        unsigned long long mine = 0, mine2 = 0;
         uint32_t biggest = 0;
         for (uint32_t w = w0; w < w1; w++) {
             const uint32_t c = cur[w];
             mine += (unsigned long long)((c + 1u) & ~1u) + (c ? (1ULL << 40) : 0ULL);
+            mine2 += ((unsigned long long)c + 63ULL) & ~63ULL;
             biggest = max(biggest, c);
         }
-        unsigned long long incl = mine;
+        unsigned long long incl = mine, incl2 = mine2;
         for (int o = 1; o < 64; o <<= 1) {
             const unsigned long long t = (unsigned long long)__shfl_up((long long)incl, o);
-            if ((int)lane >= o) incl += t;
+            const unsigned long long t2 = (unsigned long long)__shfl_up((long long)incl2, o);
+            if ((int)lane >= o) {
+                incl += t;
+                incl2 += t2;
+            }
         }
         for (int o = 32; o > 0; o >>= 1) biggest = max(biggest, (uint32_t)__shfl_xor((int)biggest, o));
-        if (lane == 63) scan_part[wave] = incl;
-        __syncthreads();
-        unsigned long long before = incl - mine, all = 0;
+        if (lane == 63) {
+            scan_part[wave] = incl;
+            scan_part2[wave] = incl2;
+        }
+        __syncthreads();
+        unsigned long long before = incl - mine, all = 0, before2 = incl2 - mine2, all2 = 0;
         for (uint32_t w = 0; w < T / 64; w++) {
-            if (w < wave) before += scan_part[w];
+            if (w < wave) {
+                before += scan_part[w];
+                before2 += scan_part2[w];
+            }
             all += scan_part[w];
+            all2 += scan_part2[w];
         }
         const unsigned long long n_slots = all & ((1ULL << 40) - 1ULL), n_tiles = all >> 40;
         const bool staged = n_slots <= a.stage_slots;
         if (tid == 0) {
             s_slot0 = atomicAdd(&a.cur->final_at, n_slots);
             s_tile0 = atomicAdd(&a.cur->tile_at, n_tiles);
+            s_copy0 = a.copy_slot ? atomicAdd(&a.cur->copy_at, all2) : 0ULL;
             a.tb_base[it] = (uint32_t)s_tile0;
             a.tb_cnt[it] = (uint32_t)n_tiles;
         }
@@ -805,10 +822,10 @@
         if (staged)
             for (uint32_t i = tid; i < (uint32_t)n_slots; i += T) stage[i] = make_uint2(0, 0);
         __syncthreads();
-        const unsigned long long slot0 = s_slot0, tile0 = s_tile0;
+        const unsigned long long slot0 = s_slot0, tile0 = s_tile0, copy0 = s_copy0;
         {
             uint32_t at = (uint32_t)(before & ((1ULL << 40) - 1ULL));
-            unsigned long long t = tile0 + (before >> 40);
+            unsigned long long t = tile0 + (before >> 40), at2 = copy0 + before2;
             const uint32_t mb = a.blk_min[b];
             for (uint32_t w = w0; w < w1; w++) {
                 const uint32_t c = cur[w];
@@ -820,11 +837,13 @@
                     const uint32_t lj = tile_level(c, lb_j), lc = tile_level(c, lb_c);
                     a.proto[2 * t] = make_uint4(b, w, (uint32_t)first, (uint32_t)(first >> 32));
                     a.proto[2 * t + 1] = make_uint4(c, lb_j, lb_c, lj | (lc << 16));
+                    if (a.copy_slot) a.copy_slot[t] = at2;
                     atomicAdd(&lv[0][lj], 1u);
                     atomicAdd(&lv[1][lc], 1u);
                     t++;
                 }
                 at += (c + 1u) & ~1u;
+                at2 += ((unsigned long long)c + 63ULL) & ~63ULL;
             }
         }
         __syncthreads();
@@ -838,12 +857,7 @@
                     if (r[d].x != 0xFFFFFFFFu) stage[atomicAdd(&cur[r[d].x & 0xFFFFu], 1u)] = make_uint2(r[d].y, r[d].z);
             }
             __syncthreads();
-            for (uint32_t i = tid; i < (uint32_t)n_slots; i += T) {
-                const uint2 v = stage[i];
-                a.contrib[slot0 + i] = v;
-                a.rows[slot0 + i] = v.x;
-                a.cols[slot0 + i] = v.y;
-            }
+            for (uint32_t i = tid; i < (uint32_t)n_slots; i += T) a.contrib[slot0 + i] = stage[i];
         } else {
             for (uint32_t i0 = r0 + tid; i0 < r1; i0 += D * T) {
                 uint3 r[D];
@@ -852,18 +866,6 @@
 #pragma unroll
                 for (int d = 0; d < D; d++)
                     if (r[d].x != 0xFFFFFFFFu && !(a.debug & 1)) a.contrib[slot0 + atomicAdd(&cur[r[d].x & 0xFFFFu], 1u)] = make_uint2(r[d].y, r[d].z);
-            }
-            __syncthreads();
-            for (unsigned long long i0 = tid; i0 < n_slots && a.rows && !(a.debug & 2); i0 += (unsigned long long)D * T) {
-                uint2 v[D];
-#pragma unroll
-                for (int d = 0; d < D; d++) v[d] = i0 + (unsigned long long)d * T < n_slots ? a.contrib[slot0 + i0 + (unsigned long long)d * T] : make_uint2(0, 0);
-#pragma unroll
-                for (int d = 0; d < D; d++)
-                    if (i0 + (unsigned long long)d * T < n_slots) {
-                        a.rows[slot0 + i0 + (unsigned long long)d * T] = v[d].x;
-                        a.cols[slot0 + i0 + (unsigned long long)d * T] = v[d].y;
-                    }
             }
         }
         __syncthreads();
@@ -896,6 +898,7 @@
     if (threadIdx.x == 0) {
         a.tres->n_tiles = a.cur->tile_at;
         a.tres->n_slots = a.cur->final_at;
+        a.tres->n_copy_slots = a.cur->copy_at;
     }
 }
 
@@ -931,12 +934,13 @@
         const uint4 *mine = a.proto + 2 * (size_t)a.tb_base[it];
         for (uint32_t t = tid; t < n; t += T) {
             const uint4 e0 = mine[2 * t], e1 = mine[2 * t + 1];
+            const unsigned long long cs = a.copy_slot ? a.copy_slot[(size_t)a.tb_base[it] + t] : 0ULL;
 #pragma unroll
             for (int m = 0; m < 2; m++) {
                 const uint32_t lv = m ? (e1.w >> 16) : (e1.w & 0xFFFFu);
                 const unsigned long long p = atomicAdd(&at[m][lv], 1ULL);
                 a.dir[m][2 * p] = e0;
-                a.dir[m][2 * p + 1] = make_uint4(e1.x, m ? e1.z : e1.y, e0.z, e0.w);
+                a.dir[m][2 * p + 1] = make_uint4(e1.x, m ? e1.z : e1.y, (uint32_t)cs, (uint32_t)(cs >> 32));
             }
         }
     }
diff --git a/rabbitkssd_amd/csrc/rk_internal.h b/rabbitkssd_amd/csrc/rk_internal.h
--- a/rabbitkssd_amd/csrc/rk_internal.h
+++ b/rabbitkssd_amd/csrc/rk_internal.h
@@ -13,6 +13,8 @@
 #include <vector>
 
 #include "rabbitkssd.h"
+
+constexpr unsigned kTileCopyMaxBlocks = 1024;
 
 struct rk_ctx {
     int device = 0;
@@ -59,6 +61,7 @@
     int sw_index_heavy = 1;
     int sw_index_tiles = 2;
     unsigned long long sw_tile_rec_cap = 0;
+    unsigned sw_tile_copy_blocks = kTileCopyMaxBlocks;
     int sw_topn = 1;
     unsigned long long sw_topn_batch_bytes = 1ULL << 30;
     unsigned long long sw_topn_cand_cap = 0;
@@ -211,7 +214,12 @@
     int fb_state = 0;
     void *fb_event = nullptr;
     uint2 *d_tile_contrib = nullptr;
-    uint32_t *d_tile_rows = nullptr, *d_tile_cols = nullptr;
+    uint32_t *d_tile_rows = nullptr, *d_tile_cols = nullptr, *d_tile_occ = nullptr;
+    uint64_t n_tile_copy_slots = 0;
+    uint4 *d_tile_proto = nullptr;
+    unsigned long long *d_tile_copy_slot = nullptr;
+    bool tile_copy_deferred = false;
+    uint32_t tile_copy_asks = 0;
     uint64_t n_tile_slots = 0, tile_max_records = 0;
     unsigned long long *d_tile_key = nullptr;
     unsigned long long *d_tile_start = nullptr;
@@ -263,6 +271,8 @@
                       unsigned end_bit, hipStream_t st);
 constexpr int kTileTable = 256;
 int rk_tiles_build(rk_ctx *ctx, rk_index *idx, hipStream_t stream);
+int rk_index_tile_copy(rk_ctx *ctx, rk_index *idx, hipStream_t stream);
+constexpr uint32_t kTileCopyAfter = 2;
 int rk_index_ensure_slices(rk_ctx *ctx, rk_index *idx, hipStream_t stream);
 int rk_index_ensure_dir(rk_ctx *ctx, rk_index *idx, hipStream_t stream);
 int rk_distq_launch(rk_ctx *ctx, const rk_index *idx, const rk_sketches *queries, const rk_dist_opts *opts, bool dense_mode,
diff --git a/rabbitkssd_amd/csrc/rk_tile_copy.h b/rabbitkssd_amd/csrc/rk_tile_copy.h
--- /dev/null
+++ b/rabbitkssd_amd/csrc/rk_tile_copy.h
@@ -0,0 +1,170 @@
+
+constexpr uint32_t kCopyStage = 512;
+constexpr uint32_t kCopyWaves = 8;
+constexpr uint32_t kCopyLoads = 8;
+constexpr uint32_t kCopySteps = 4;
+constexpr unsigned kCopyMaxGrid = 8192;
+
+struct TileCopyArgs {
+    const uint2 *recs;
+    const unsigned long long *tile_start;
+    const uint4 *proto;
+    const unsigned long long *copy_slot;
+    unsigned long long n_tiles;
+    const unsigned long long *n_tiles_dev;
+    const unsigned long long *n_slots_dev;
+    unsigned long long cap;
+    uint2 *sorted;
+    uint32_t *rows, *cols, *occ;
+    unsigned wave_blocks;
+};
+
+__device__ inline uint32_t octet_signature(uint32_t m)
+{
+    return ((m & 0xFFu) ? 1u : 0u) | ((m & 0xFF00u) ? 2u : 0u) | ((m & 0xFF0000u) ? 4u : 0u) | ((m >> 24) ? 8u : 0u);
+}
+
+__device__ inline uint32_t transpose_32x32(uint32_t x, uint32_t lane)
+{
+    uint32_t m = 0x0000FFFFu;
+#pragma unroll
+    for (uint32_t j = 16; j != 0; j >>= 1) {
+        const uint32_t t = (uint32_t)__shfl_xor((int)x, (int)j);
+        x = (lane & j) ? ((t >> j) & m) | (x & ~m) : (x & m) | ((t & m) << j);
+        m ^= m << (j >> 1);
+    }
+    return x;
+}
+
+__device__ inline void copy_wave_sync()
+{
+    __builtin_amdgcn_fence(__ATOMIC_RELEASE, "wavefront");
+    __builtin_amdgcn_wave_barrier();
+}
+
+__device__ inline void copy_histogram(const uint2 *recs, uint32_t n, uint32_t tid, uint32_t threads, uint32_t *hist)
+{
+    for (uint32_t i0 = tid; i0 < n; i0 += threads * kCopyLoads) {
+        uint32_t x[kCopyLoads];
+#pragma unroll
+        for (uint32_t d = 0; d < kCopyLoads; d++) x[d] = i0 + threads * d < n ? recs[i0 + threads * d].x : 0u;
+#pragma unroll
+        for (uint32_t d = 0; d < kCopyLoads; d++)
+            if (i0 + threads * d < n) atomicAdd(&hist[octet_signature(x[d])], 1u);
+    }
+}
+
+__device__ inline void copy_scan(uint32_t lane, uint32_t *hist)
+{
+    const uint32_t mine = lane < 16 ? hist[lane] : 0u;
+    uint32_t incl = mine;
+#pragma unroll
+    for (int o = 1; o < 16; o <<= 1) {
+        const uint32_t up = (uint32_t)__shfl_up((int)incl, o);
+        if ((int)lane >= o) incl += up;
+    }
+    copy_wave_sync();
+    if (lane < 16) hist[lane] = incl - mine;
+}
+
+__device__ inline void copy_place(const uint2 *recs, uint32_t n, uint32_t tid, uint32_t threads, uint32_t *hist, uint2 *sorted)
+{
+    for (uint32_t i0 = tid; i0 < n; i0 += threads * kCopyLoads) {
+        uint2 r[kCopyLoads];
+#pragma unroll
+        for (uint32_t d = 0; d < kCopyLoads; d++) r[d] = i0 + threads * d < n ? recs[i0 + threads * d] : make_uint2(0, 0);
+#pragma unroll
+        for (uint32_t d = 0; d < kCopyLoads; d++)
+            if (i0 + threads * d < n) sorted[atomicAdd(&hist[octet_signature(r[d].x)], 1u)] = r[d];
+    }
+}
+
+__device__ inline void copy_transpose(const TileCopyArgs &a, const uint2 *src, uint32_t n, uint32_t n_pad, unsigned long long c0, uint32_t j_first,
+                                      uint32_t j_stride, uint32_t lane)
+{
+    for (uint32_t j0 = j_first; j0 < n_pad; j0 += j_stride) {
+        uint2 rr[kCopySteps];
+#pragma unroll
+        for (uint32_t d = 0; d < kCopySteps; d++) {
+            const uint32_t i = j0 + 64 * d + lane;
+            rr[d] = i < n ? src[i] : make_uint2(0, 0);
+        }
+#pragma unroll
+        for (uint32_t d = 0; d < kCopySteps; d++) {
+            const uint32_t i0 = j0 + 64 * d, i = i0 + lane;
+            if (i0 >= n_pad) break;
+            const uint2 r = rr[d];
+            const uint32_t sig = octet_signature(r.x);
+            const uint32_t occ = (__ballot(sig & 1u) ? 1u : 0u) | (__ballot(sig & 2u) ? 2u : 0u) | (__ballot(sig & 4u) ? 4u : 0u) | (__ballot(sig & 8u) ? 8u : 0u);
+            a.rows[c0 + i] = transpose_32x32(r.x, lane & 31u);
+            a.cols[c0 + i] = transpose_32x32(r.y, lane & 31u);
+            if (lane == 0) a.occ[(c0 + i0) >> 6] = occ;
+        }
+    }
+}
+
+__global__ __launch_bounds__(64 * kCopyWaves) void k_tile_copy(TileCopyArgs a)
+{
+    __shared__ uint32_t s_hist[kCopyWaves][16];
+    __shared__ uint2 s_stage[kCopyWaves][kCopyStage];
+    if (a.n_slots_dev && *a.n_slots_dev > a.cap) return;
+    const unsigned long long n_tiles = a.n_tiles_dev ? *a.n_tiles_dev : a.n_tiles;
+    const uint32_t lane = threadIdx.x & 63, wave = threadIdx.x >> 6;
+    const bool by_wave = blockIdx.x < a.wave_blocks;
+    unsigned long long t = by_wave ? (unsigned long long)blockIdx.x * kCopyWaves + wave : (unsigned long long)(blockIdx.x - a.wave_blocks);
+    const unsigned long long t_step = by_wave ? (unsigned long long)a.wave_blocks * kCopyWaves : (unsigned long long)(gridDim.x - a.wave_blocks);
+    for (; t < n_tiles; t += t_step) {
+        unsigned long long s0, n64;
+        if (a.proto) {
+            const uint4 e0 = a.proto[2 * t];
+            s0 = (unsigned long long)e0.z | ((unsigned long long)e0.w << 32);
+            n64 = a.proto[2 * t + 1].x;
+        } else {
+            s0 = a.tile_start[t];
+            n64 = a.tile_start[t + 1] - s0;
+        }
+        if (by_wave != (n64 <= kCopyStage)) continue;
+        const unsigned long long c0 = a.copy_slot[t];
+        const unsigned long long n_pad = (n64 + 63ULL) & ~63ULL;
+        if (n64 > 0xFFFFFFFFULL || c0 + n_pad > a.cap) continue;
+        const uint32_t n = (uint32_t)n64;
+        const uint2 *recs = a.recs + s0;
+        if (by_wave) {
+            uint32_t *hist = s_hist[wave];
+            uint2 *stage = s_stage[wave];
+            if (n > 64) {
+                copy_wave_sync();
+                if (lane < 16) hist[lane] = 0;
+                copy_wave_sync();
+                copy_histogram(recs, n, lane, 64, hist);
+                copy_wave_sync();
+                copy_scan(lane, hist);
+                copy_wave_sync();
+                copy_place(recs, n, lane, 64, hist, stage);
+                copy_wave_sync();
+            }
+            copy_transpose(a, n > 64 ? stage : recs, n, (uint32_t)n_pad, c0, 0, 64 * kCopySteps, lane);
+        } else {
+            uint32_t *hist = s_hist[0];
+            uint2 *sorted = n <= kCopyWaves * kCopyStage ? &s_stage[0][0] : a.sorted + s0;
+            __syncthreads();
+            if (threadIdx.x < 16) hist[threadIdx.x] = 0;
+            __syncthreads();
+            copy_histogram(recs, n, threadIdx.x, 64 * kCopyWaves, hist);
+            __syncthreads();
+            if (wave == 0) copy_scan(lane, hist);
+            __syncthreads();
+            copy_place(recs, n, threadIdx.x, 64 * kCopyWaves, hist, sorted);
+            __syncthreads();
+            copy_transpose(a, sorted, n, (uint32_t)n_pad, c0, wave * 64 * kCopySteps, kCopyWaves * 64 * kCopySteps, lane);
+        }
+    }
+}
+
+inline void launch_tile_copy(TileCopyArgs a, unsigned long long n_tiles, hipStream_t st)
+{
+    const unsigned long long by_wave = (n_tiles + kCopyWaves - 1) / kCopyWaves;
+    a.wave_blocks = (unsigned)(by_wave < 1 ? 1 : (by_wave > kCopyMaxGrid ? kCopyMaxGrid : by_wave));
+    const unsigned by_group = (unsigned)(n_tiles < 1 ? 1 : (n_tiles > kCopyMaxGrid ? kCopyMaxGrid : n_tiles));
+    hipLaunchKernelGGL(k_tile_copy, dim3(a.wave_blocks + by_group), dim3(64 * kCopyWaves), 0, st, a);
+}
diff --git a/rabbitkssd_amd/csrc/rk_tiles.hip b/rabbitkssd_amd/csrc/rk_tiles.hip
--- a/rabbitkssd_amd/csrc/rk_tiles.hip
+++ b/rabbitkssd_amd/csrc/rk_tiles.hip
@@ -10,6 +10,8 @@
 #include "rk_internal.h"
 
 namespace {
+
+#include "rk_tile_copy.h"
 
 
 __global__ void k_list_starts(const uint32_t *upos, uint64_t U, uint8_t *starts)
@@ -127,7 +129,7 @@
     const unsigned long long i = (unsigned long long)blockIdx.x * blockDim.x + threadIdx.x;
     if (i >= n_tiles) return;
     const uint32_t t = order[i];
-    const unsigned long long key = tile_key[t], s0 = tile_start[t], n = tile_start[t + 1] - s0, d0 = slot_start[t];
+    const unsigned long long key = tile_key[t], s0 = tile_start[t], n = tile_start[t + 1] - s0, d0 = slot_start ? slot_start[t] : 0ULL;
     const uint32_t b = (uint32_t)(key >> 32), w = (uint32_t)key;
     const uint32_t mb = blk_min[b], mw = blk_min[w];
     out[2 * i] = make_uint4(b, w, (uint32_t)s0, (uint32_t)(s0 >> 32));
@@ -144,20 +146,7 @@
 __global__ void k_tile_padded_counts(const unsigned long long *tile_start, unsigned long long n_tiles, unsigned long long *padded)
 {
     const unsigned long long t = (unsigned long long)blockIdx.x * blockDim.x + threadIdx.x;
-    if (t < n_tiles) padded[t] = (tile_start[t + 1] - tile_start[t] + 1ULL) & ~1ULL;
-}
-__global__ void k_tile_split(const uint2 *recs, const unsigned long long *tile_start, const unsigned long long *slot_start, unsigned long long n_tiles,
-                             uint32_t *rows, uint32_t *cols)
-{
-    const unsigned long long t = (unsigned long long)blockIdx.x * (blockDim.x >> 6) + (threadIdx.x >> 6);
-    if (t >= n_tiles) return;
-    const uint32_t lane = threadIdx.x & 63;
-    const unsigned long long s0 = tile_start[t], n = tile_start[t + 1] - s0, d0 = slot_start[t];
-    for (unsigned long long i = lane; i < n; i += 64) {
-        const uint2 r = recs[s0 + i];
-        rows[d0 + i] = r.x;
-        cols[d0 + i] = r.y;
-    }
+    if (t < n_tiles) padded[t] = (tile_start[t + 1] - tile_start[t] + 63ULL) & ~63ULL;
 }
 
 #define RK_TILE_TRY(call) do { int rc__ = (call); if (rc__) return rc__; } while (0)
@@ -206,8 +195,8 @@
     DevBuf<uint2> vals_out(ctx);
     DevBuf<uint32_t> order_j(ctx), order_c(ctx);
     DevBuf<uint4> dir_j(ctx), dir_c(ctx);
-    DevBuf<uint32_t> t_rows(ctx), t_cols(ctx);
-    unsigned long long n_slots = 0;
+    DevBuf<uint32_t> t_rows(ctx), t_cols(ctx), t_occ(ctx);
+    unsigned long long n_copy_slots = 0;
     unsigned long long n_c = 0, n_t = 0;
     if (H && U) {
         DevBuf<uint32_t> bm(ctx), rank(ctx);
@@ -311,19 +300,34 @@
             RK_HIP(ctx, rocprim::radix_sort_pairs(tmp3.p, tb3, key_c.p, key_out.p, ids.p, order_c.p, (size_t)n_t, 0, 32, st));
             hipLaunchKernelGGL(k_tile_prefix_table, dim3(1), dim3(kTileTable), 0, st, key_out.p, n_t, table.p + kTileTable);
             DevBuf<unsigned long long> slot_start(ctx);
-            RK_HIP(ctx, slot_start.alloc(n_t + 1));
-            hipLaunchKernelGGL(k_tile_padded_counts, nb(n_t), dim3(tpb), 0, st, tile_start.p, n_t, slot_start.p);
-            RK_HIP(ctx, hipGetLastError());
-            RK_TILE_TRY(tile_scan_u64(ctx, slot_start.p, n_t, &n_slots, st));
-            RK_HIP(ctx, t_rows.alloc(n_slots + 256));
-            RK_HIP(ctx, t_cols.alloc(n_slots + 256));
-            RK_HIP(ctx, hipMemsetAsync(t_rows.p, 0, (n_slots + 256) * 4, st));
-            RK_HIP(ctx, hipMemsetAsync(t_cols.p, 0, (n_slots + 256) * 4, st));
-            hipLaunchKernelGGL(k_tile_split, dim3((unsigned)((n_t + 3) / 4)), dim3(256), 0, st, vals_out.p, tile_start.p, slot_start.p, n_t, t_rows.p, t_cols.p);
+            DevBuf<uint2> copy_scratch(ctx);
+            const bool with_copy = n_blocks <= ctx->sw_tile_copy_blocks;
+            if (with_copy) {
+                RK_HIP(ctx, slot_start.alloc(n_t + 1));
+                hipLaunchKernelGGL(k_tile_padded_counts, nb(n_t), dim3(tpb), 0, st, tile_start.p, n_t, slot_start.p);
+                RK_HIP(ctx, hipGetLastError());
+                RK_TILE_TRY(tile_scan_u64(ctx, slot_start.p, n_t, &n_copy_slots, st));
+                RK_HIP(ctx, t_rows.alloc(n_copy_slots));
+                RK_HIP(ctx, t_cols.alloc(n_copy_slots));
+                RK_HIP(ctx, t_occ.alloc(n_copy_slots / 64));
+                RK_HIP(ctx, copy_scratch.alloc(n_c));
+                TileCopyArgs ca;
+                memset(&ca, 0, sizeof ca);
+                ca.recs = vals_out.p;
+                ca.tile_start = tile_start.p;
+                ca.copy_slot = slot_start.p;
+                ca.n_tiles = n_t;
+                ca.cap = n_copy_slots;
+                ca.sorted = copy_scratch.p;
+                ca.rows = t_rows.p;
+                ca.cols = t_cols.p;
+                ca.occ = t_occ.p;
+                launch_tile_copy(ca, n_t, st);
+            }
             RK_HIP(ctx, dir_j.alloc(2 * n_t));
             RK_HIP(ctx, dir_c.alloc(2 * n_t));
-            hipLaunchKernelGGL(k_tile_dir, nb(n_t), dim3(tpb), 0, st, order_j.p, tile_key.p, tile_start.p, slot_start.p, blk_min.p, n_t, 0, dir_j.p);
-            hipLaunchKernelGGL(k_tile_dir, nb(n_t), dim3(tpb), 0, st, order_c.p, tile_key.p, tile_start.p, slot_start.p, blk_min.p, n_t, 1, dir_c.p);
+            hipLaunchKernelGGL(k_tile_dir, nb(n_t), dim3(tpb), 0, st, order_j.p, tile_key.p, tile_start.p, with_copy ? slot_start.p : nullptr, blk_min.p, n_t, 0, dir_j.p);
+            hipLaunchKernelGGL(k_tile_dir, nb(n_t), dim3(tpb), 0, st, order_c.p, tile_key.p, tile_start.p, with_copy ? slot_start.p : nullptr, blk_min.p, n_t, 1, dir_c.p);
             RK_HIP(ctx, hipGetLastError());
             RK_HIP(ctx, hipStreamSynchronize(st));
             RK_HIP(ctx, hipGetLastError());
@@ -336,7 +340,9 @@
     idx->d_tile_contrib = vals_out.release();
     idx->d_tile_rows = t_rows.release();
     idx->d_tile_cols = t_cols.release();
-    idx->n_tile_slots = n_slots;
+    idx->d_tile_occ = t_occ.release();
+    idx->n_tile_copy_slots = n_copy_slots;
+    idx->n_tile_slots = n_c;
     idx->d_tile_key = tile_key.release();
     idx->d_tile_start = tile_start.release();
     idx->d_blk_min = blk_min.release();
```

Measured after the change: 4049 billion genome-pairs/s (median of 6 runs). 37.8% higher.
